# TaceoLabs/co-snarks

Hardware: AMD Instinct MI355X
Metric: BN254 G1 MSM points/sec (higher is better)
Workload: dtype i32x9 29-bit-limb lazy Montgomery, i64 accumulate (BN254 Fq 254-bit); 1 GPU; BN254 G1 Pippenger MSM, uniform scalars / known-dlog points, 2^20 points per GPU (BASELINE config 2); points_total=1048576, points_per_gpu=1048576, split=single GPU, exchange_mode=none, rccl_ranks_seen=0, spinup_steps=190

## Files before the change

### co-snarks_amd/csrc/host_fp64.hpp

```cpp
#pragma once
#include <stdint.h>
#include <string.h>

#include "field.hpp"

#if defined(__clang__)
#define CSH_HOST_UNROLL _Pragma("unroll")
#elif defined(__GNUC__)
#define CSH_HOST_UNROLL _Pragma("GCC unroll 16")
#else
#define CSH_HOST_UNROLL
#endif

namespace csh {

template <int N>
struct Fp64Consts {
  uint64_t mod[N], one[N], pm2[N];
  uint64_t inv;
};
template <class P>
constexpr Fp64Consts<P::N / 2> fp64_consts() {
  Fp64Consts<P::N / 2> k{};
  for (int i = 0; i < P::N / 2; ++i) {
    k.mod[i] = (uint64_t)P::MOD[2 * i] | ((uint64_t)P::MOD[2 * i + 1] << 32);
    k.one[i] = (uint64_t)P::R1[2 * i] | ((uint64_t)P::R1[2 * i + 1] << 32);
    k.pm2[i] = (uint64_t)P::PM2[2 * i] | ((uint64_t)P::PM2[2 * i + 1] << 32);
  }
  uint64_t y = k.mod[0];
  for (int i = 0; i < 6; ++i) y *= 2 - k.mod[0] * y;
  k.inv = (uint64_t)0 - y;
  return k;
}

template <class P>
struct Fp64 {
  static_assert(P::N % 2 == 0, "limb count must be even");
  static constexpr int N = P::N / 2;
  using Params = P;
  using u128 = unsigned __int128;
  uint64_t l[N];

  static constexpr Fp64Consts<N> K = fp64_consts<P>();
  static_assert((K.mod[N - 1] >> 63) == 0 && K.mod[N - 1] != 0x7fffffffffffffffull, "the modulus must leave its top bit free");
  static_assert((uint64_t)(K.mod[0] * K.inv) == ~(uint64_t)0, "inv must be -p^-1 mod 2^64");

  static uint64_t word(const uint32_t* w, int i) { return (uint64_t)w[2 * i] | ((uint64_t)w[2 * i + 1] << 32); }
  static constexpr uint64_t inv64() { return K.inv; }
  static Fp64 zero() {
    Fp64 r;
    for (int i = 0; i < N; ++i) r.l[i] = 0;
    return r;
  }
  static Fp64 one() {
    Fp64 r;
    for (int i = 0; i < N; ++i) r.l[i] = K.one[i];
    return r;
  }
  bool is_zero() const {
    uint64_t a = 0;
    for (int i = 0; i < N; ++i) a |= l[i];
    return a == 0;
  }
  bool operator==(const Fp64& b) const { return memcmp(l, b.l, sizeof l) == 0; }
  bool operator!=(const Fp64& b) const { return !(*this == b); }

  static bool geq_mod(const uint64_t* a) {
    CSH_HOST_UNROLL
    for (int i = N - 1; i >= 0; --i) {
      if (a[i] > K.mod[i]) return true;
      if (a[i] < K.mod[i]) return false;
    }
    return true;
  }
  static void sub_mod(uint64_t* a) {
    u128 br = 0;
    CSH_HOST_UNROLL
    for (int i = 0; i < N; ++i) {
      const u128 d = (u128)a[i] - K.mod[i] - (uint64_t)br;
      a[i] = (uint64_t)d;
      br = (d >> 64) & 1;
    }
  }
  static Fp64 add(const Fp64& a, const Fp64& b) {
    Fp64 r;
    u128 c = 0;
    CSH_HOST_UNROLL
    for (int i = 0; i < N; ++i) {
      c += (u128)a.l[i] + b.l[i];
      r.l[i] = (uint64_t)c;
      c >>= 64;
    }
    if (geq_mod(r.l)) sub_mod(r.l);
    return r;
  }
  static Fp64 sub(const Fp64& a, const Fp64& b) {
    Fp64 r;
    uint64_t br = 0;
    CSH_HOST_UNROLL
    for (int i = 0; i < N; ++i) {
      const u128 d = (u128)a.l[i] - b.l[i] - br;
      r.l[i] = (uint64_t)d;
      br = (uint64_t)(d >> 64) & 1;
    }
    if (br) {
      u128 c = 0;
      CSH_HOST_UNROLL
      for (int i = 0; i < N; ++i) {
        c += (u128)r.l[i] + K.mod[i];
        r.l[i] = (uint64_t)c;
        c >>= 64;
      }
    }
    return r;
  }
  static Fp64 neg(const Fp64& a) { return a.is_zero() ? a : sub(zero(), a); }

  static Fp64 mul(const Fp64& a, const Fp64& b) {
    uint64_t t[N];
    CSH_HOST_UNROLL
    for (int j = 0; j < N; ++j) t[j] = 0;
    CSH_HOST_UNROLL
    for (int i = 0; i < N; ++i) {
      u128 A = (u128)a.l[i] * b.l[0] + t[0];
      const uint64_t m = (uint64_t)A * K.inv;
      u128 C = (u128)m * K.mod[0] + (uint64_t)A;
      CSH_HOST_UNROLL
      for (int j = 1; j < N; ++j) {
        A = (u128)a.l[i] * b.l[j] + t[j] + (uint64_t)(A >> 64);
        C = (u128)m * K.mod[j] + (uint64_t)A + (uint64_t)(C >> 64);
        t[j - 1] = (uint64_t)C;
      }
      t[N - 1] = (uint64_t)(A >> 64) + (uint64_t)(C >> 64);
    }
    Fp64 r;
    CSH_HOST_UNROLL
    for (int i = 0; i < N; ++i) r.l[i] = t[i];
    if (geq_mod(r.l)) sub_mod(r.l);
    return r;
  }
  static Fp64 sqr(const Fp64& a) {
    uint64_t t[2 * N];
    CSH_HOST_UNROLL
    for (int j = 0; j < 2 * N; ++j) t[j] = 0;
    CSH_HOST_UNROLL
    for (int i = 0; i < N - 1; ++i) {
      uint64_t c = 0;
      CSH_HOST_UNROLL
      for (int j = i + 1; j < N; ++j) {
        const u128 v = (u128)a.l[i] * a.l[j] + t[i + j] + c;
        t[i + j] = (uint64_t)v;
        c = (uint64_t)(v >> 64);
      }
      t[i + N] = c;
    }
    CSH_HOST_UNROLL
    for (int j = 2 * N - 1; j > 0; --j) t[j] = (t[j] << 1) | (t[j - 1] >> 63);
    t[0] = 0;
    {
      uint64_t c = 0;
      CSH_HOST_UNROLL
      for (int i = 0; i < N; ++i) {
        const u128 d = (u128)a.l[i] * a.l[i];
        const u128 lo = (u128)t[2 * i] + (uint64_t)d + c;
        t[2 * i] = (uint64_t)lo;
        const u128 hi = (u128)t[2 * i + 1] + (uint64_t)(d >> 64) + (uint64_t)(lo >> 64);
        t[2 * i + 1] = (uint64_t)hi;
        c = (uint64_t)(hi >> 64);
      }
    }
    uint64_t top = 0;
    CSH_HOST_UNROLL
    for (int i = 0; i < N; ++i) {
      const uint64_t m = t[i] * K.inv;
      u128 C = (u128)m * K.mod[0] + t[i];
      CSH_HOST_UNROLL
      for (int j = 1; j < N; ++j) {
        C = (u128)m * K.mod[j] + t[i + j] + (uint64_t)(C >> 64);
        t[i + j] = (uint64_t)C;
      }
      const u128 s = (u128)t[i + N] + (uint64_t)(C >> 64) + top;
      t[i + N] = (uint64_t)s;
      top = (uint64_t)(s >> 64);
    }
    Fp64 r;
    CSH_HOST_UNROLL
    for (int i = 0; i < N; ++i) r.l[i] = t[i + N];
    if (geq_mod(r.l)) sub_mod(r.l);
    return r;
  }
  static Fp64 mul2(const Fp64& a) { return add(a, a); }
  static Fp64 mul3(const Fp64& a) { return add(add(a, a), a); }
  static Fp64 mul4(const Fp64& a) { return mul2(mul2(a)); }
  static Fp64 mul8(const Fp64& a) { return mul2(mul4(a)); }
  static Fp64 inv(const Fp64& a) {
    Fp64 pw[16];
    pw[0] = one();
    pw[1] = a;
    for (int i = 2; i < 16; ++i) pw[i] = (i & 1) ? mul(pw[i - 1], a) : sqr(pw[i / 2]);
    Fp64 r = one();
    bool started = false;
    for (int i = 16 * N - 1; i >= 0; --i) {
      const unsigned d = (unsigned)(K.pm2[i >> 4] >> (4 * (i & 15))) & 15u;
      if (started) r = sqr(sqr(sqr(sqr(r))));
      if (d) {
        r = started ? mul(r, pw[d]) : pw[d];
        started = true;
      }
    }
    return r;
  }

  static Fp64 mul_looped(const Fp64& a, const Fp64& b) {
    uint64_t t[N + 2];
    for (int i = 0; i < N + 2; ++i) t[i] = 0;
    const uint64_t inv = K.inv;
    for (int i = 0; i < N; ++i) {
      u128 c = 0;
      for (int j = 0; j < N; ++j) {
        c += (u128)a.l[j] * b.l[i] + t[j];
        t[j] = (uint64_t)c;
        c >>= 64;
      }
      c += t[N];
      t[N] = (uint64_t)c;
      t[N + 1] = (uint64_t)(c >> 64);
      const uint64_t m = t[0] * inv;
      c = (u128)m * K.mod[0] + t[0];
      c >>= 64;
      for (int j = 1; j < N; ++j) {
        c += (u128)m * K.mod[j] + t[j];
        t[j - 1] = (uint64_t)c;
        c >>= 64;
      }
      c += t[N];
      t[N - 1] = (uint64_t)c;
      t[N] = t[N + 1] + (uint64_t)(c >> 64);
    }
    Fp64 r;
    for (int i = 0; i < N; ++i) r.l[i] = t[i];
    if (t[N] || geq_mod(r.l)) sub_mod(r.l);
    return r;
  }
  static Fp64 inv_looped(const Fp64& a) {
    Fp64 r = one();
    for (int i = P::N * 32 - 1; i >= 0; --i) {
      r = mul_looped(r, r);
      if ((P::PM2[i >> 5] >> (i & 31)) & 1) r = mul_looped(r, a);
    }
    return r;
  }
};

template <class F>
struct Host64;
template <class P>
struct Host64<Fp<P>> {
  using type = Fp64<P>;
};
template <class P, int NR>
struct Host64<Fp2T<Fp<P>, NR>> {
  using type = Fp2T<Fp64<P>, NR>;
};

}
```

### co-snarks_amd/csrc/msm.hip

```cpp
#include <algorithm>
#include <condition_variable>
#include <memory>
#include <mutex>
#include <string>
#include <vector>

#include "msm_impl.hpp"

namespace csh {

thread_local float tl_msm_timing[6] = {0, 0, 0, 0, 0, 0};
thread_local uint32_t tl_msm_params[4] = {0, 0, 0, 0};

CSH_MSM_INSTANTIATE(extern, Bn254G1Cfg)
CSH_MSM_INSTANTIATE(extern, Bn254G2Cfg)
CSH_MSM_INSTANTIATE(extern, Bls381G1Cfg)
CSH_MSM_INSTANTIATE(extern, Bls381G2Cfg)
CSH_MSM_INSTANTIATE(extern, GrumpkinG1Cfg)
CSH_MSM_INSTANTIATE(extern, Bls377G1Cfg)
CSH_MSM_INSTANTIATE(extern, Bls377G2Cfg)
CSH_MSM_ACCUM_INSTANTIATE(extern, Bn254G1Cfg)
CSH_MSM_ACCUM_INSTANTIATE(extern, Bn254G2Cfg)
CSH_MSM_ACCUM_INSTANTIATE(extern, Bls381G1Cfg)
CSH_MSM_ACCUM_INSTANTIATE(extern, Bls381G2Cfg)
CSH_MSM_ACCUM_INSTANTIATE(extern, GrumpkinG1Cfg)
CSH_MSM_ACCUM_INSTANTIATE(extern, Bls377G1Cfg)
CSH_MSM_ACCUM_INSTANTIATE(extern, Bls377G2Cfg)
CSH_MSM_ACCUM_PAIR_INSTANTIATE(extern, Bn254G2Cfg)
CSH_MSM_ACCUM_PAIR_INSTANTIATE(extern, Bls381G2Cfg)
CSH_MSM_ACCUM_PAIR_INSTANTIATE(extern, Bls377G2Cfg)

static int repack_bases(Bases* B, hipStream_t st);

template <class Cfg>
static GroupOps group_ops_of(csh_curve_t curve, csh_group_t group) {
  using Fq = typename Cfg::Fq;
  return GroupOps{curve, group, Cfg::Fr::Params::BITS, sizeof(Affine<Fq>), sizeof(XYZZ<Fq>), msm_sort_stage<typename Cfg::Fr>,
                  msm_bucket_bytes<Cfg>, msm_bucket_stage<Cfg>, fold_windows_erased<Cfg>, accum_occupancy<Cfg>};
}
const GroupOps* group_ops(csh_curve_t curve, csh_group_t group) {
  static const GroupOps table[] = {
      group_ops_of<Bn254G1Cfg>(CSH_BN254, CSH_G1),       group_ops_of<Bn254G2Cfg>(CSH_BN254, CSH_G2),       group_ops_of<Bls381G1Cfg>(CSH_BLS12_381, CSH_G1),
      group_ops_of<Bls381G2Cfg>(CSH_BLS12_381, CSH_G2),  group_ops_of<GrumpkinG1Cfg>(CSH_GRUMPKIN, CSH_G1), group_ops_of<Bls377G1Cfg>(CSH_BLS12_377, CSH_G1),
      group_ops_of<Bls377G2Cfg>(CSH_BLS12_377, CSH_G2)};
  for (const GroupOps& o : table)
    if (o.curve == curve && o.group == group) return &o;
  set_error("unknown curve/group %d/%d", (int)curve, (int)group);
  return nullptr;
}

struct BasesFree {
  void operator()(Bases* B) const {
    if (B->points) (void)hipFree(B->points);
    if (B->table) (void)hipFree(B->table);
    delete B;
  }
};
using BasesPtr = std::unique_ptr<Bases, BasesFree>;

static int on_callers_device(const Bases* B) {
  int cur = -1;
  if (hipGetDevice(&cur) == hipSuccess && cur != B->device) {
    set_error("bases were uploaded on device %d but the calling thread is bound to device %d (csh_init): upload a copy per device", B->device, cur);
    return CSH_ERR_INVALID;
  }
  return CSH_OK;
}

}

using namespace csh;

namespace {
struct SharedUpload {
  int device = 0;
  const void* host = nullptr;
  size_t bytes = 0, cap = 0;
  void* dev = nullptr;
  hipEvent_t ready = nullptr;
  int refs = 0;
  std::mutex m;
  std::condition_variable cv;
  int state = 0;
  struct Req {
    csh_bases_t bases = nullptr;
    size_t offset = 0;
    void* out = nullptr;
    int rc = CSH_OK;
    std::string err;
  };
  std::vector<Req*> batch;
  bool sealed = false;
  bool batch_done = false;
  int curve = -1, mont = -1;
};
std::mutex g_up_mu;
std::vector<SharedUpload*> g_up_live;
struct PooledBuffer {
  int device;
  size_t cap;
  void* dev;
};
std::vector<PooledBuffer> g_up_pool;
constexpr size_t UP_POOL_MAX = 8;
constexpr size_t UP_POOL_MAX_BYTES = size_t(1) << 30;

struct SharedUploadRef {
  SharedUpload* e = nullptr;
  hipStream_t stream = nullptr;
  const void* dev() const { return e->dev; }
  bool is_owner = false;
  int acquire(int device, const void* host, size_t bytes, hipStream_t st, SharedUpload::Req* req = nullptr, int curve = -1, int mont = -1, bool* joined = nullptr) {
    stream = st;
    bool owner = false;
    {
      std::lock_guard<std::mutex> g(g_up_mu);
      for (SharedUpload* x : g_up_live)
        if (x->device == device && x->host == host && x->bytes == bytes) {
          bool failed;
          {
            std::lock_guard<std::mutex> gs(x->m);
            failed = x->state < 0;
          }
          if (failed) continue;
          e = x;
          break;
        }
      if (e) {
        ++e->refs;
      } else {
        e = new SharedUpload();
        e->device = device, e->host = host, e->bytes = bytes, e->refs = 1;
        e->curve = curve, e->mont = mont;
        size_t best = (size_t)-1;
        for (size_t i = 0; i < g_up_pool.size(); ++i)
          if (g_up_pool[i].device == device && g_up_pool[i].cap >= bytes && (best == (size_t)-1 || g_up_pool[i].cap < g_up_pool[best].cap)) best = i;
        if (best != (size_t)-1) {
          e->cap = g_up_pool[best].cap;
          e->dev = g_up_pool[best].dev;
          g_up_pool.erase(g_up_pool.begin() + (ptrdiff_t)best);
        }
        g_up_live.push_back(e);
        owner = true;
      }
    }
    is_owner = owner;
    if (owner) {
      hipError_t rc = hipSuccess;
      if (!e->dev) {
        e->cap = (bytes + (size_t(1) << 20) - 1) & ~((size_t(1) << 20) - 1);
        rc = hipMalloc(&e->dev, e->cap);
        if (rc != hipSuccess) e->dev = nullptr;
      }
      if (rc == hipSuccess) rc = hipEventCreateWithFlags(&e->ready, hipEventDisableTiming);
      if (rc == hipSuccess && upload_h2d(e->dev, host, bytes, st, 3) != CSH_OK) rc = hipErrorUnknown;
      if (rc == hipSuccess) rc = hipEventRecord(e->ready, st);
      {
        std::lock_guard<std::mutex> g(e->m);
        e->state = rc == hipSuccess ? 1 : -1;
      }
      e->cv.notify_all();
      if (rc != hipSuccess) {
        set_error("csh_msm: uploading the scalars failed: %s", hipGetErrorString(rc));
        return rc == hipErrorOutOfMemory ? CSH_ERR_OOM : CSH_ERR_HIP;
      }
      return CSH_OK;
    }
    {
      std::unique_lock<std::mutex> g(e->m);
      if (req && joined && !e->sealed && e->curve == curve && e->mont == mont && curve >= 0 && e->batch.size() < 15) {
        e->batch.push_back(req);
        *joined = true;
        e->cv.wait(g, [&] { return e->batch_done || e->state < 0; });
        if (!e->batch_done) {
          e->batch.erase(std::find(e->batch.begin(), e->batch.end(), req));
          set_error("csh_msm: the concurrent call that was uploading this scalar slice failed");
          return CSH_ERR_HIP;
        }
        tune().stat_uploads_shared.fetch_add(1, std::memory_order_relaxed);
        return CSH_OK;
      }
      e->cv.wait(g, [&] { return e->state != 0; });
      if (e->state < 0) {
        set_error("csh_msm: the concurrent call that was uploading this scalar slice failed");
        return CSH_ERR_HIP;
      }
    }
    CSH_HIP(hipStreamWaitEvent(st, e->ready, 0));
    tune().stat_uploads_shared.fetch_add(1, std::memory_order_relaxed);
    return CSH_OK;
  }
  std::vector<SharedUpload::Req*> seal() {
    std::lock_guard<std::mutex> g(e->m);
    e->sealed = true;
    return e->batch;
  }
  void finish_batch() {
    {
      std::lock_guard<std::mutex> g(e->m);
      e->batch_done = true;
    }
    e->cv.notify_all();
  }
  ~SharedUploadRef() {
    if (!e) return;
    if (is_owner) {
      bool wake = false;
      {
        std::lock_guard<std::mutex> g(e->m);
        if (!e->batch_done) {
          e->sealed = true;
          for (SharedUpload::Req* r : e->batch)
            if (r->rc == CSH_OK && r->err.empty()) {
              r->rc = CSH_ERR_HIP;
              r->err = "csh_msm: the concurrent call that ran this batch failed before it reached this request";
            }
          e->batch_done = true;
          wake = true;
        }
      }
      if (wake) e->cv.notify_all();
    }
    (void)hipStreamSynchronize(stream);
    SharedUpload* dead = nullptr;
    {
      std::lock_guard<std::mutex> g(g_up_mu);
      if (--e->refs == 0) {
        g_up_live.erase(std::find(g_up_live.begin(), g_up_live.end(), e));
        dead = e;
        size_t pooled = 0;
        for (const PooledBuffer& b : g_up_pool) pooled += b.cap;
        if (dead->dev && g_up_pool.size() < UP_POOL_MAX && pooled + dead->cap <= UP_POOL_MAX_BYTES) {
          g_up_pool.push_back({dead->device, dead->cap, dead->dev});
          dead->dev = nullptr;
        }
      }
    }
    if (dead) {
      if (dead->ready) (void)hipEventDestroy(dead->ready);
      if (dead->dev) (void)hipFree(dead->dev);
      delete dead;
    }
  }
};
}

static int csh::repack_bases(Bases* B, hipStream_t st) {
  CURVE_DISPATCH(B->curve, B->group, (repack_bases_t<Cfg>(B, st)));
}

extern "C" {

static int bases_upload_common(csh_curve_t curve, csh_group_t group, const void* pts, size_t n, size_t stride, bool src_dev, void* stream,
                               csh_bases_t* out) {
  CSH_REQUIRE(out, "out is NULL");
  const GroupOps* G = group_ops(curve, group);
  if (!G) return CSH_ERR_INVALID;
  CSH_REQUIRE(n < (size_t(1) << 31), "at most 2^31-1 bases per handle");
  CSH_REQUIRE(pts || n == 0, "points is NULL");
  CSH_TRY(ensure_device());
  const size_t pb = G->point_bytes;
  if (stride == 0) stride = pb;
  CSH_REQUIRE(stride >= pb, "stride_bytes smaller than a packed affine point");
  BasesPtr B(new Bases());
  B->curve = curve;
  B->group = group;
  B->n = n;
  B->point_bytes = pb;
  B->points = nullptr;
  if (hipGetDevice(&B->device) != hipSuccess) B->device = 0;
  hipError_t e = hipMalloc(&B->points, n ? n * pb : 1);
  if (e != hipSuccess) {
    B->points = nullptr;
    set_error("hipMalloc(%zu bytes) for bases failed: %s", n * pb, hipGetErrorString(e));
    return CSH_ERR_OOM;
  }
  if (n) {
    hipStream_t st = resolve_stream(stream);
    const hipMemcpyKind kind = src_dev ? hipMemcpyDeviceToDevice : hipMemcpyHostToDevice;
    if (!src_dev && stride == pb) {
      if (upload_h2d(B->points, pts, n * pb, st, 0) != CSH_OK) e = hipErrorUnknown;
    } else {
      e = stride == pb ? hipMemcpyAsync(B->points, pts, n * pb, kind, st) : hipMemcpy2DAsync(B->points, pb, pts, stride, pb, n, kind, st);
    }
    if (e == hipSuccess) e = hipStreamSynchronize(st);
    if (e != hipSuccess) {
      set_error("bases upload failed: %s", hipGetErrorString(e));
      return CSH_ERR_HIP;
    }
    CSH_TRY(repack_bases(B.get(), st));
  }
  *out = reinterpret_cast<csh_bases_t>(B.release());
  return CSH_OK;
}

int csh_bases_upload(csh_curve_t curve, csh_group_t group, const void* pts, size_t n, size_t stride, csh_bases_t* out) {
  return bases_upload_common(curve, group, pts, n, stride, false, nullptr, out);
}
int csh_bases_upload_dev(csh_curve_t curve, csh_group_t group, const void* pts, size_t n, size_t stride, void* stream, csh_bases_t* out) {
  return bases_upload_common(curve, group, pts, n, stride, true, stream, out);
}
int csh_bases_len(csh_bases_t bases, size_t* n) {
  CSH_REQUIRE(bases && n, "NULL argument");
  *n = reinterpret_cast<Bases*>(bases)->n;
  return CSH_OK;
}
int csh_bases_clone_range(csh_bases_t src, size_t offset, size_t n, int device, csh_bases_t* out) {
  CSH_REQUIRE(src && out, "NULL argument");
  const Bases* S = reinterpret_cast<const Bases*>(src);
  CSH_REQUIRE(offset <= S->n && n <= S->n - offset, "csh_bases_clone_range: offset + n exceeds the number of bases");
  int ndev = 0, cur = 0;
  CSH_HIP(hipGetDeviceCount(&ndev));
  CSH_REQUIRE(device >= 0 && device < ndev, "device out of range");
  CSH_HIP(hipGetDevice(&cur));
  BasesPtr B(new Bases(*S));
  B->points = nullptr;
  B->table = nullptr;
  B->device = device;
  B->n = n;
  const size_t pb = S->point_bytes, pbytes = n * pb, rows = S->table ? (size_t)S->table_W : 0;
  if (!rows) B->table_c = B->table_W = 0;
  hipError_t e = hipSetDevice(device);
  if (e == hipSuccess && pbytes) e = hipMalloc(&B->points, pbytes);
  if (e == hipSuccess && pbytes && rows) e = hipMalloc(&B->table, pbytes * rows);
  if (e == hipSuccess && pbytes) e = hipMemcpyPeer(B->points, device, static_cast<const char*>(S->points) + offset * pb, S->device, pbytes);
  for (size_t k = 0; e == hipSuccess && pbytes && k < rows; ++k)
    e = hipMemcpyPeer(static_cast<char*>(B->table) + k * pbytes, device, static_cast<const char*>(S->table) + (k * S->n + offset) * pb, S->device, pbytes);
  if (e == hipSuccess) e = hipDeviceSynchronize();
  if (e == hipSuccess && S->device != device) {
    e = hipSetDevice(S->device);
    if (e == hipSuccess) e = hipDeviceSynchronize();
  }
  (void)hipSetDevice(cur);
  if (e != hipSuccess) {
    set_error("csh_bases_clone_range to device %d failed: %s", device, hipGetErrorString(e));
    return e == hipErrorOutOfMemory ? CSH_ERR_OOM : CSH_ERR_HIP;
  }
  *out = reinterpret_cast<csh_bases_t>(B.release());
  return CSH_OK;
}
int csh_bases_clone(csh_bases_t src, int device, csh_bases_t* out) {
  CSH_REQUIRE(src && out, "NULL argument");
  return csh_bases_clone_range(src, 0, reinterpret_cast<const Bases*>(src)->n, device, out);
}
int csh_bases_free(csh_bases_t bases) {
  const BasesPtr freed(reinterpret_cast<Bases*>(bases));
  return CSH_OK;
}

static int bases_precompute(csh_bases_t bases, int c, int groups);
int csh_bases_table_policy(size_t key_points, int* c_out, int* rows_out) {
  CSH_REQUIRE(c_out && rows_out, "c_out / rows_out is NULL");
  *c_out = 0;
  *rows_out = 0;
  if (key_points < (size_t(1) << 14) || key_points > (size_t(1) << 26)) return CSH_OK;
  if (key_points < (size_t(1) << 15)) {
    int c = 16;
    while (c > 10 && (size_t(1) << (c + 1)) > key_points) --c;
    *c_out = c;
    *rows_out = 16;
    return CSH_OK;
  }
  if (key_points <= (size_t(3) << 20)) {
    *c_out = 17;
    *rows_out = 16;
  } else {
    *c_out = 20;
    *rows_out = 13;
  }
  return CSH_OK;
}
int csh_bases_drop_tables(csh_bases_t bases) {
  CSH_REQUIRE(bases, "bases is NULL");
  Bases* B = reinterpret_cast<Bases*>(bases);
  if (B->table) {
    (void)hipFree(B->table);
    B->table = nullptr;
    B->table_c = B->table_W = 0;
  }
  return CSH_OK;
}
int csh_bases_precompute(csh_bases_t bases, int c) { return bases_precompute(bases, c, 0); }
int csh_bases_precompute_grouped(csh_bases_t bases, int c, int groups) {
  CSH_REQUIRE(groups >= 2 && groups <= MAX_WINDOWS, "groups must be in [2, 128]");
  return bases_precompute(bases, c, groups);
}
static int bases_precompute(csh_bases_t bases, int c, int groups) {
  CSH_REQUIRE(bases, "bases is NULL");
  CSH_TRY(ensure_device());
  Bases* B = reinterpret_cast<Bases*>(bases);
  CSH_REQUIRE(c == 0 || (c >= 4 && c <= 22), "window width must be 0 (auto) or in [4, 22]");
  if (B->table) {
    (void)hipFree(B->table);
    B->table = nullptr;
  }
  if (B->n < 1024) return CSH_OK;
  if (c == 0) {
    c = 16;
    while (c > 10 && (size_t(1) << (c + 1)) > B->n) --c;
  }
  CSH_TRY(on_callers_device(B));
  hipStream_t st = resolve_stream(nullptr);
  CURVE_DISPATCH(B->curve, B->group, (precompute_table_t<Cfg>(B, c, groups, st)));
}

static int msm_args(csh_bases_t bases, size_t offset, size_t n, const void* scalars, const void* out) {
  CSH_REQUIRE(bases, "bases is NULL");
  CSH_REQUIRE(out, "out is NULL");
  Bases* B = reinterpret_cast<Bases*>(bases);
  CSH_REQUIRE(offset <= B->n && n <= B->n - offset, "offset + n exceeds the uploaded bases");
  CSH_REQUIRE(scalars || n == 0, "scalars is NULL");
  return on_callers_device(B);
}

int csh_msm_dev(csh_bases_t bases, size_t offset, size_t n, const uint64_t* scalars_dev, int mont, void* out_host, void* stream) {
  CSH_TRY(msm_args(bases, offset, n, scalars_dev, out_host));
  CSH_TRY(ensure_device());
  Bases* B = reinterpret_cast<Bases*>(bases);
  hipStream_t st = resolve_stream(stream);
  CURVE_DISPATCH(B->curve, B->group, (msm_t<Cfg>(B, offset, n, scalars_dev, mont, out_host, st)));
}

static int run_owned_batch(SharedUploadRef& up, SharedUpload::Req& own, size_t n, const uint64_t* dsc, int mont, hipStream_t st) {
  const std::vector<SharedUpload::Req*> others = up.seal();
  if (others.empty()) {
    up.finish_batch();
    return csh_msm_dev(own.bases, own.offset, n, dsc, mont, own.out, st);
  }
  std::vector<SharedUpload::Req*> all;
  all.push_back(&own);
  for (SharedUpload::Req* r : others) all.push_back(r);
  std::stable_sort(all.begin(), all.end(), [](const SharedUpload::Req* a, const SharedUpload::Req* b) {
    return reinterpret_cast<const Bases*>(a->bases)->group > reinterpret_cast<const Bases*>(b->bases)->group;
  });
  std::vector<csh_bases_t> hs;
  std::vector<size_t> offs;
  std::vector<void*> outs;
  for (SharedUpload::Req* r : all) hs.push_back(r->bases), offs.push_back(r->offset), outs.push_back(r->out);
  const int rc = csh_msm_multi_dev(hs.data(), offs.data(), all.size(), n, dsc, mont, outs.data(), st);
  const std::string err = rc == CSH_OK ? std::string() : std::string(csh_last_error());
  for (SharedUpload::Req* r : others) r->rc = rc, r->err = err;
  up.finish_batch();
  return rc;
}

int csh_msm(csh_bases_t bases, size_t offset, size_t n, const uint64_t* scalars, int mont, void* out) {
  CSH_TRY(msm_args(bases, offset, n, scalars, out));
  const size_t bytes = 32 * n;
  if (bytes >= (size_t(1) << 20) && tune().msm_share_uploads.load(std::memory_order_relaxed) != 0) {
    CSH_TRY(ensure_device());
    hipStream_t st = resolve_stream(nullptr);
    int device = 0;
    (void)hipGetDevice(&device);
    const bool batching = tune().msm_share_uploads.load(std::memory_order_relaxed) >= 2;
    const Bases* B = reinterpret_cast<const Bases*>(bases);
    SharedUpload::Req req;
    req.bases = bases, req.offset = offset, req.out = out;
    bool joined = false;
    SharedUploadRef up;
    CSH_TRY(up.acquire(device, scalars, bytes, st, batching ? &req : nullptr, batching ? (int)B->curve : -1, mont != 0, &joined));
    if (joined) {
      if (req.rc != CSH_OK) set_error("%s", req.err.c_str());
      return req.rc;
    }
    const uint64_t* dsc = reinterpret_cast<const uint64_t*>(up.dev());
    if (!up.is_owner || !batching) return csh_msm_dev(bases, offset, n, dsc, mont, out, st);
    return run_owned_batch(up, req, n, dsc, mont, st);
  }
  HostStage h;
  CSH_TRY(h.begin(Arena::padded(bytes)));
  uint64_t* ds;
  CSH_TRY(h.up(ds, scalars, bytes));
  return csh_msm_dev(bases, offset, n, ds, mont, out, h.st);
}

int csh_msm_shares(csh_bases_t bases, size_t offset, size_t n, const uint64_t* shares, uint32_t ncomp, int mont, void* const* outs) {
  CSH_REQUIRE(ncomp >= 1 && ncomp <= 2 && outs, "msm_shares: ncomp must be 1 or 2 and outs non-NULL");
  for (uint32_t c = 0; c < ncomp; ++c) CSH_REQUIRE(outs[c], "msm_shares: NULL output");
  CSH_TRY(msm_args(bases, offset, n, shares, outs[0]));
  if (ncomp == 1) return csh_msm(bases, offset, n, shares, mont, outs[0]);
  HostStage h;
  CSH_TRY(h.begin(Arena::padded(32 * (size_t)ncomp * n) + Arena::padded(32 * n)));
  uint64_t *dsh, *dcomp;
  CSH_TRY(h.up(dsh, shares, 32 * (size_t)ncomp * n));
  CSH_TRY(h.up(dcomp, nullptr, 32 * n));
  for (uint32_t c = 0; c < ncomp; ++c) {
    CSH_TRY(csh_extract_component_dev(dsh, ncomp, c, n, dcomp, h.st));
    CSH_TRY(csh_msm_dev(bases, offset, n, dcomp, mont, outs[c], h.st));
  }
  return CSH_OK;
}

int csh_msm_partial_bytes(csh_curve_t curve, csh_group_t group, size_t* bytes) {
  CSH_REQUIRE(bytes, "bytes is NULL");
  if (!group_ops(curve, group)) return CSH_ERR_INVALID;
  *bytes = partial_bytes_of(curve, group);
  return CSH_OK;
}

int csh_msm_partial_dev(csh_bases_t bases, size_t offset, size_t n, const uint64_t* scalars_dev, int mont, void* out_dev, void* stream) {
  CSH_TRY(msm_args(bases, offset, n, scalars_dev, out_dev));
  CSH_TRY(ensure_device());
  Bases* B = reinterpret_cast<Bases*>(bases);
  hipStream_t st = resolve_stream(stream);
  CURVE_DISPATCH(B->curve, B->group, (msm_partial_t<Cfg>(B, offset, n, scalars_dev, mont, out_dev, st, true)));
}

int csh_msm_fold_partials(csh_curve_t curve, csh_group_t group, const void* partials_host, size_t nparts, void* out_jacobian) {
  CSH_REQUIRE(partials_host && out_jacobian, "NULL argument");
  CURVE_DISPATCH(curve, group, (fold_partials_t<Cfg>(partials_host, nparts, out_jacobian)));
}

int csh_msm_multi_dev(const csh_bases_t* bases, const size_t* offsets, size_t k, size_t n, const uint64_t* scalars_dev, int mont,
                      void* const* outs_host, void* stream) {
  CSH_REQUIRE(bases && offsets && outs_host && k >= 1 && k <= 16, "msm_multi: bad arguments");
  CSH_REQUIRE(scalars_dev || n == 0, "scalars is NULL");
  CSH_REQUIRE(n < (size_t(1) << 31), "n too large");
  CSH_TRY(ensure_device());
  const auto handle = [&](size_t i) { return reinterpret_cast<const Bases*>(bases[i]); };
  const Bases* B0 = handle(0);
  CSH_REQUIRE(B0, "bases[0] is NULL");
  for (size_t i = 0; i < k; ++i) {
    const Bases* B = handle(i);
    CSH_REQUIRE(B && outs_host[i], "msm_multi: NULL handle or output");
    CSH_REQUIRE(B->curve == B0->curve, "msm_multi: all bases must belong to one curve");
    CSH_REQUIRE(offsets[i] <= B->n && n <= B->n - offsets[i], "msm_multi: offset + n exceeds the number of bases");
    CSH_REQUIRE(B->device == B0->device, "msm_multi: bases live on different devices");
  }
  CSH_TRY(on_callers_device(B0));
  hipStream_t st = resolve_stream(stream);
  std::vector<const GroupOps*> ops(k);
  for (size_t i = 0; i < k; ++i)
    if (!(ops[i] = group_ops(handle(i)->curve, handle(i)->group))) return CSH_ERR_INVALID;
  if (n == 0) {
    for (size_t i = 0; i < k; ++i) ops[i]->fold(nullptr, 0, 2, 0, outs_host[i]);
    return CSH_OK;
  }
  bool merged = true;
  for (size_t i = 0; i < k; ++i) merged = merged && msm_use_table(handle(i), n) && handle(i)->table_c == B0->table_c && handle(i)->table_W == B0->table_W;
  int occ = 8;
  for (const GroupOps* o : ops) occ = std::min(occ, o->occ());
  const MsmTable table{B0->table_c, B0->table_W, B0->n, 0};
  MsmPlan plan = msm_plan(n, ops[0]->scalar_bits, mont, occ, merged ? &table : nullptr);
  msm_record_params(plan.srt);
  const MsmParams& pdig = plan.dig;
  MsmParams& p = plan.srt;
  size_t bucket_max = 0, win_bytes = 0, slice = 0;
  for (const GroupOps* o : ops) {
    bucket_max = std::max(bucket_max, o->bucket_bytes(&p));
    win_bytes += Arena::padded(o->xyzz_bytes * MAX_WINDOWS);
    slice = std::max(slice, Arena::padded(o->xyzz_bytes * MAX_WINDOWS));
  }
  Arena& ar = arena_for(st);
  CSH_TRY(ar.reserve(msm_sort_bytes(p, pdig) + 2 * Arena::padded(bucket_max)));
  Arena& wa = arena_for((hipStream_t)((uintptr_t)st ^ 0x2));
  CSH_TRY(wa.reserve(win_bytes));
  hipStream_t aux = nullptr;
  if (tune().msm_multi_overlap.load(std::memory_order_relaxed) != 0 && k > 1) aux = resolve_aux_stream();
  const bool two = aux != nullptr;
  Events evs;
  CSH_TRY(evs.create(k + (two ? 2 : 0), hipEventDisableTiming));
  const hipEvent_t sorted_ev = two ? evs[k] : nullptr, aux_done = two ? evs[k + 1] : nullptr;
  auto body = [&]() -> int {
    SortOut so;
    std::vector<char*> win_dev(k);
    std::vector<hipStream_t> stage_stream(k, st);
    size_t mark = 0, sorted_stride = (size_t)-1, sorted_off = (size_t)-1;
    bool aux_used = false;
    for (size_t i = 0; i < k; ++i) {
      const Bases* B = handle(i);
      const bool resort = merged ? (B->n != sorted_stride || offsets[i] != sorted_off) : i == 0;
      if (resort) {
        if (two && aux_used) {
          CSH_HIP(hipEventRecord(aux_done, aux));
          CSH_HIP(hipStreamWaitEvent(st, aux_done, 0));
        }
        ar.off = 0;
        if (merged) {
          p.remap_stride = (uint32_t)(sorted_stride = B->n);
          p.remap_off = (uint32_t)(sorted_off = offsets[i]);
        }
        CSH_TRY(ops[0]->sort(p, pdig, scalars_dev, st, ar, &so, nullptr));
        mark = ar.off;
        if (two) {
          CSH_HIP(hipEventRecord(sorted_ev, st));
          CSH_HIP(hipStreamWaitEvent(aux, sorted_ev, 0));
        }
      }
      const bool on_aux = two && (i & 1);
      stage_stream[i] = on_aux ? aux : st;
      aux_used = aux_used || on_aux;
      ar.off = mark + (on_aux ? Arena::padded(bucket_max) : 0);
      win_dev[i] = wa.take<char>(ops[i]->xyzz_bytes * MAX_WINDOWS);
      const void* src = merged ? B->table : static_cast<const char*>(B->points) + offsets[i] * B->point_bytes;
      CSH_TRY(ops[i]->bucket(src, &p, &so, stage_stream[i], &ar, win_dev[i], nullptr));
    }
    void *pin_host = nullptr, *pin_dev = nullptr;
    std::vector<char> pageable;
    char* wins = nullptr;
    if (pinned_for((hipStream_t)((uintptr_t)st ^ 0x4), slice * k, &pin_host, &pin_dev)) {
      wins = static_cast<char*>(pin_host);
    } else {
      pageable.resize(slice * k);
      wins = pageable.data();
    }
    for (size_t i = 0; i < k; ++i) {
      hipError_t e = hipMemcpyAsync(wins + slice * i, win_dev[i], ops[i]->xyzz_bytes * p.W, hipMemcpyDeviceToHost, stage_stream[i]);
      if (e == hipSuccess) e = hipEventRecord(evs[i], stage_stream[i]);
      if (e != hipSuccess) {
        set_error("msm_multi: queuing the window sums of result %zu failed: %s", i, hipGetErrorString(e));
        return CSH_ERR_HIP;
      }
    }
    for (size_t i = 0; i < k; ++i) {
      const hipError_t e = hipEventSynchronize(evs[i]);
      if (e != hipSuccess) {
        set_error("msm_multi: result %zu failed on the device: %s", i, hipGetErrorString(e));
        return CSH_ERR_HIP;
      }
      ops[i]->fold(wins + slice * i, p.W, p.c, p.wide, outs_host[i]);
    }
    CSH_HIP(hipStreamSynchronize(st));
    if (aux) CSH_HIP(hipStreamSynchronize(aux));
    return CSH_OK;
  };
  const int rc = body();
  if (rc != CSH_OK) {
    (void)hipStreamSynchronize(st);
    if (aux) (void)hipStreamSynchronize(aux);
  }
  return rc;
}

int csh_msm_plan(csh_curve_t curve, size_t n, uint32_t out[6]) {
  CSH_REQUIRE(out, "out is NULL");
  const GroupOps* G = group_ops(curve, CSH_G1);
  if (!G) return CSH_ERR_INVALID;
  CSH_REQUIRE(n >= 1 && n < (size_t(1) << 31), "n out of range");
  const MsmParams p = msm_plan(n, G->scalar_bits, 1, 1).srt;
  const uint64_t lanes = (n + p.L - 1) / p.L;
  out[0] = (uint32_t)p.c;
  out[1] = (uint32_t)p.W;
  out[2] = p.L;
  out[3] = p.S;
  out[4] = (uint32_t)((uint64_t)p.W * ((lanes + ACC_BLK - 1) / ACC_BLK) * (ACC_BLK / 64));
  out[5] = (uint32_t)device_simds();
  return CSH_OK;
}

int csh_msm_last_params(uint32_t out[4]) {
  CSH_REQUIRE(out, "out is NULL");
  for (int i = 0; i < 4; ++i) out[i] = tl_msm_params[i];
  return CSH_OK;
}

int csh_msm_last_timing(float out_ms[6]) {
  CSH_REQUIRE(out_ms, "out_ms is NULL");
  for (int i = 0; i < 6; ++i) out_ms[i] = tl_msm_timing[i];
  return CSH_OK;
}

}
```

### co-snarks_amd/csrc/msm_impl.hpp

```cpp
#pragma once
#include <stdlib.h>
#include <string.h>

#include <algorithm>
#include <type_traits>
#include <vector>

#include "common.hpp"
#include "curve.hpp"
#include "curve_lazy.hpp"
#include "curve_quad.hpp"
#include "curve_pair.hpp"
#include "host_fp64.hpp"
#include "msm_digits.hpp"
#include "msm_plan.hpp"
#include "msm_sort.hpp"
#include "msm_sort_wide.hpp"


namespace csh {

struct Bn254G1Cfg { using Fq = Bn254Fq;   using Fr = Bn254Fr; static constexpr bool LAZY = true;  using L = Fq29s; static constexpr bool INLINE_ADD = true; static constexpr bool PAIR = false; };
struct Bn254G2Cfg { using Fq = Bn254Fq2;  using Fr = Bn254Fr; static constexpr bool LAZY = true;  using L = Fq29s2; static constexpr bool INLINE_ADD = true; static constexpr bool PAIR = true; static constexpr bool PAIR_ACC_DEFAULT = false; using LP = Fp2Pair<Fq29s>; };
struct Bls381G1Cfg { using Fq = Bls381Fq;  using Fr = Bls381Fr; static constexpr bool LAZY = true;  using L = Fq28s; static constexpr bool INLINE_ADD = true; static constexpr bool PAIR = false; };
struct GrumpkinG1Cfg { using Fq = Bn254Fr;   using Fr = Bn254Fq; static constexpr bool LAZY = true;  using L = Fr29s; static constexpr bool INLINE_ADD = true; static constexpr bool PAIR = false; };
struct Bls377G1Cfg { using Fq = Bls377Fq;  using Fr = Bls377Fr; static constexpr bool LAZY = true;  using L = Fq28s377; static constexpr bool INLINE_ADD = true; static constexpr bool PAIR = false; };
struct Bls377G2Cfg { using Fq = Bls377Fq2; using Fr = Bls377Fr; static constexpr bool LAZY = true;  using L = Fq28s377x2; static constexpr bool INLINE_ADD = true; static constexpr bool PAIR = true; static constexpr bool PAIR_ACC_DEFAULT = true; using LP = Fp2Pair<Fq28s377, 5>; };
struct Bls381G2Cfg { using Fq = Bls381Fq2; using Fr = Bls381Fr; static constexpr bool LAZY = true;  using L = Fq28s2; static constexpr bool INLINE_ADD = true; static constexpr bool PAIR = true; static constexpr bool PAIR_ACC_DEFAULT = true; using LP = Fp2Pair<Fq28s>; };

struct Bases {
  csh_curve_t curve;
  csh_group_t group;
  int device;
  size_t n;
  size_t point_bytes;
  void* points;
  void* table = nullptr;
  int table_c = 0, table_W = 0;
};


constexpr int MSM_BLK = 256;

template <class Fr>
__device__ __forceinline__ void load_scalar(const Fr* __restrict__ scalars, size_t i, int mont, uint32_t* s) {
  Fr v = scalars[i];
  if (mont) v = v.from_mont();
#pragma unroll
  for (int k = 0; k < Fr::N; ++k) s[k] = v.l[k];
}


template <class Fr>
__global__ __launch_bounds__(MSM_BLK) void k_msm_digits(const Fr* __restrict__ scalars, MsmParams p, uint16_t* __restrict__ dig) {
  const uint32_t g = p.dig_g > 1 ? p.dig_g : 1u, wp = p.dig_g > 1 ? p.dig_wp : (uint32_t)p.W;
  const uint32_t rows = g * wp;
  const uint32_t W = (uint32_t)p.W, wide = (uint32_t)p.wide;
  for (size_t i = blockIdx.x * (size_t)MSM_BLK + threadIdx.x; i < p.n; i += (size_t)gridDim.x * MSM_BLK) {
    uint32_t s[Fr::N];
    load_scalar<Fr>(scalars, i, p.mont, s);
    uint32_t carry = 0, rq = 0, rr = 0;
    for (uint32_t w = 0; w < rows; ++w) {
      uint32_t code = DIG_ZERO;
      if (w < W) {
        const uint32_t c = (uint32_t)p.c - (w >= wide ? 1u : 0u);
        const uint32_t mask = (1u << c) - 1, half = 1u << (c - 1);
        const uint32_t v = (s[0] & mask) + carry;
#pragma unroll
        for (int k = 0; k + 1 < Fr::N; ++k) s[k] = (s[k] >> c) | (s[k + 1] << (32 - c));
        s[Fr::N - 1] >>= c;
        const uint32_t neg = v > half ? 1u : 0u;
        const uint32_t mag = neg ? (1u << c) - v : v;
        carry = neg;
        code = mag ? ((mag - 1) | (neg << 15)) : (uint32_t)DIG_ZERO;
      }
      dig[(size_t)(rr * g + rq) * p.n + i] = (uint16_t)code;
      if (++rr == wp) {
        rr = 0;
        ++rq;
      }
    }
  }
}

template <class P>
__device__ __forceinline__ uint32_t top_word(const Fp<P>& f) { return f.l[Fp<P>::N - 1]; }
template <class F, int NR>
__device__ __forceinline__ uint32_t top_word(const Fp2T<F, NR>& f) { return top_word(f.c0) | top_word(f.c1); }
template <class Fq>
__device__ __forceinline__ bool stored_is_inf(const Affine<Fq>& pt) {
  return (top_word(pt.x) | top_word(pt.y)) == 0 && pt.is_inf();
}

__device__ __forceinline__ uint32_t upper_bound_u32(const uint32_t* __restrict__ a, uint32_t lo, uint32_t hi, uint32_t v) {
  while (lo < hi) {
    const uint32_t mid = (lo + hi) >> 1;
    if (a[mid] > v) hi = mid; else lo = mid + 1;
  }
  return lo;
}

template <class Cfg>
using LazyPt = XYZZLazy<typename Cfg::L>;

template <class Cfg>
__global__ __launch_bounds__(ACC_BLK) void k_msm_accum(const Affine<typename Cfg::Fq>* __restrict__ bases, MsmParams p,
                                                       const uint32_t* __restrict__ start, const uint32_t* __restrict__ nlanes,
                                                       const uint32_t* __restrict__ sorted, LazyPt<Cfg>* partial, uint32_t* giant_count) {
  using Fq = typename Cfg::Fq;
  static_assert(Cfg::LAZY, "the bucket pipeline runs in the signed lazy field");
  const int w = blockIdx.y;
  const uint32_t k = blockIdx.x * blockDim.x + threadIdx.x;
  if (k == 0 && w == 0) {
    giant_count[0] = 0;
    giant_count[1] = 0;
  }
  if (k >= nlanes[w]) return;
  const uint32_t* st = start + (size_t)w * (p.NB + 2);
  const uint32_t total = st[p.NB + 1];
  const uint32_t Lw = lane_len(p, w);
  const uint32_t lo = k * Lw;
  uint32_t hi = lo + Lw;
  if (hi > total) hi = total;
  uint32_t b = upper_bound_u32(st, 1, p.NB + 1, lo) - 1;
  uint32_t next = st[b + 1];
  const uint32_t* so = sorted + (size_t)w * p.n;
  LazyPt<Cfg>* pw = partial + (size_t)w * p.tmax;
  {
    using L = typename Cfg::L;
    XYZZLazy<L> acc = XYZZLazy<L>::inf();
    uint32_t e_next = so[lo];
    Affine<Fq> pt_next = bases[e_next & 0x7fffffffu];
    constexpr bool INDEX_AHEAD = !Cfg::PAIR;
    uint32_t e_next2 = (INDEX_AHEAD && lo + 1 < hi) ? so[lo + 1] : 0;
    for (uint32_t pos = lo; pos < hi; ++pos) {
      const uint32_t e = e_next;
      const Affine<Fq> pt = pt_next;
      if (pos + 1 < hi) {
        if constexpr (INDEX_AHEAD) {
          e_next = e_next2;
          pt_next = bases[e_next & 0x7fffffffu];
          if (pos + 2 < hi) e_next2 = so[pos + 2];
        } else {
          e_next = so[pos + 1];
          pt_next = bases[e_next & 0x7fffffffu];
        }
      }
      const bool inf = stored_is_inf(pt);
      const L x = L::unpack(pt.x);
      const L y = L::unpack(pt.y).cneg_unpacked(e >> 31);
      if (pos == next) {
        pw[b + k] = acc;
        do { ++b; next = st[b + 1]; } while (next <= pos);
        acc.x = x;
        acc.y = y;
        acc.zz = L::one();
        acc.zzz = L::one();
        acc.empty = inf;
        continue;
      }
      if (inf) continue;
      lazy_madd<L, Affine<Fq>>(acc, x, y, bases + (e & 0x7fffffffu), e >> 31);
    }
    pw[b + k] = acc;
  }
}

template <class Cfg>
__global__ __launch_bounds__(ACC_BLK) void k_msm_accum_pair(const Affine<typename Cfg::Fq>* __restrict__ bases, MsmParams p,
                                                            const uint32_t* __restrict__ start, const uint32_t* __restrict__ nlanes,
                                                            const uint32_t* __restrict__ sorted, LazyPt<Cfg>* partial, uint32_t* giant_count) {
  using Fq = typename Cfg::Fq;
  using L = typename Cfg::LP;
  using LF = typename L::Base;
  using F32 = decltype(bases->x.c0);
  const int w = blockIdx.y;
  const int role = pair_role();
  const uint32_t k = (blockIdx.x * blockDim.x + threadIdx.x) >> 1;
  if (blockIdx.x == 0 && threadIdx.x == 0 && w == 0) {
    giant_count[0] = 0;
    giant_count[1] = 0;
  }
  if (k >= nlanes[w]) return;
  const uint32_t* st = start + (size_t)w * (p.NB + 2);
  const uint32_t total = st[p.NB + 1];
  const uint32_t Lw = lane_len(p, w);
  const uint32_t lo = k * Lw;
  uint32_t hi = lo + Lw;
  if (hi > total) hi = total;
  uint32_t b = upper_bound_u32(st, 1, p.NB + 1, lo) - 1;
  uint32_t next = st[b + 1];
  const uint32_t* so = sorted + (size_t)w * p.n;
  LazyPt<Cfg>* pw = partial + (size_t)w * p.tmax;
  const F32* half = reinterpret_cast<const F32*>(bases) + role;
  XYZZLazy<L> acc = XYZZLazy<L>::inf();
  uint32_t e_next = so[lo];
  F32 x_next = half[4 * (size_t)(e_next & 0x7fffffffu)], y_next = half[4 * (size_t)(e_next & 0x7fffffffu) + 2];
  for (uint32_t pos = lo; pos < hi; ++pos) {
    const uint32_t e = e_next;
    const F32 xs = x_next, ys = y_next;
    if (pos + 1 < hi) {
      e_next = so[pos + 1];
      x_next = half[4 * (size_t)(e_next & 0x7fffffffu)];
      y_next = half[4 * (size_t)(e_next & 0x7fffffffu) + 2];
    }
    const bool inf = pair_all((top_word(xs) | top_word(ys)) == 0 && xs.is_zero() && ys.is_zero());
    const L x{LF::unpack(xs)};
    const L y{LF::unpack(ys).cneg_unpacked(e >> 31)};
    if (pos == next) {
      pair_store(&pw[b + k], role, acc);
      do { ++b; next = st[b + 1]; } while (next <= pos);
      acc.x = x;
      acc.y = y;
      acc.zz = L::one();
      acc.zzz = L::one();
      acc.empty = inf;
      continue;
    }
    if (inf) continue;
    lazy_madd<L, Affine<Fq>>(acc, x, y, bases + (e & 0x7fffffffu), e >> 31);
  }
  pair_store(&pw[b + k], role, acc);
}

constexpr int MERGE_BLK = 256;
constexpr int MERGE_Q = MERGE_BLK / 4;

constexpr uint32_t MERGE_CAP = 16;
constexpr uint32_t GIANT_BIG = 256, GIANT_SLICES = 16, GIANT_BIG_CAP = 128, GIANT_ROWS = 32, GIANT_SLICED_FLAG = 0x80000000u;
__device__ __forceinline__ void giant_enqueue(uint32_t* giant_count, uint32_t* giant_list, uint32_t* big_list, uint32_t w, uint32_t b, uint32_t nparts) {
  uint32_t tag = w;
  if (nparts >= GIANT_BIG) {
    const uint32_t q = atomicAdd(giant_count + 1, 1u);
    if (q < GIANT_BIG_CAP) {
      big_list[2 * q] = w;
      big_list[2 * q + 1] = b;
      tag |= GIANT_SLICED_FLAG;
    }
  }
  const uint32_t g = atomicAdd(giant_count, 1u);
  giant_list[2 * g] = tag;
  giant_list[2 * g + 1] = b;
}
template <class Cfg>
__global__ __launch_bounds__(MERGE_BLK) void k_msm_merge(MsmParams p, const uint32_t* __restrict__ start,
                                                         const LazyPt<Cfg>* __restrict__ partial, LazyPt<Cfg>* dense,
                                                         uint32_t* giant_count, uint32_t* giant_list, uint32_t* big_list) {
  using L = typename Cfg::L;
  __shared__ uint32_t list_n;
  __shared__ uint32_t list[MERGE_Q];
  const int w = blockIdx.y;
  const int role = threadIdx.x & 3;
  const uint32_t q = threadIdx.x >> 2;
  const uint32_t b0 = blockIdx.x * MERGE_Q + 1;
  const uint32_t* st = start + (size_t)w * (p.NB + 2);
  const uint32_t Lw = lane_len(p, w);
  const LazyPt<Cfg>* pw = partial + (size_t)w * p.tmax;
  LazyPt<Cfg>* dw = dense + (size_t)w * (p.NB + 1);
  if (threadIdx.x == 0) list_n = 0;
  __syncthreads();
  if (const uint32_t b = b0 + q; b <= p.NB) {
    const uint32_t lo = st[b], hi = st[b + 1];
    QPt<L> acc = qpt_inf<L>();
    if (hi > lo) {
      const uint32_t k0 = lo / Lw, k1 = (hi - 1) / Lw;
      if (k1 - k0 >= MERGE_CAP) {
        if (role == 0) giant_enqueue(giant_count, giant_list, big_list, (uint32_t)w, b, k1 - k0 + 1);
      } else {
        acc = qpt_load<L>(&pw[b + k0], role);
        if (k1 > k0) qadd<L>(acc, qpt_load<L>(&pw[b + k0 + 1], role), role);
        if (k1 - k0 >= 2 && role == 0) list[atomicAdd(&list_n, 1u)] = q;
      }
    }
    qpt_store<L>(&dw[b], role, acc);
  }
  __syncthreads();
  if (q < list_n) {
    const uint32_t b = b0 + list[q];
    const uint32_t k0 = st[b] / Lw, k1 = (st[b + 1] - 1) / Lw;
    QPt<L> acc = qpt_load<L>(&dw[b], role);
    for (uint32_t k = k0 + 2; k <= k1; ++k) qadd<L>(acc, qpt_load<L>(&pw[b + k], role), role);
    qpt_store<L>(&dw[b], role, acc);
  }
}

template <class L>
__device__ __forceinline__ void quad_block_tree(QPt<L>& x, XYZZLazy<L>* sh, int q, int nq, int role) {
  for (int half = nq >> 1; half >= 1; half >>= 1) {
    if (q >= half && q < 2 * half) qpt_store<L>(&sh[q - half], role, x);
    __syncthreads();
    if (q < half) qadd<L>(x, qpt_load<L>(&sh[q], role), role);
    __syncthreads();
  }
}

template <class Cfg>
__global__ __launch_bounds__(256) void k_msm_giant_slices(MsmParams p, const uint32_t* __restrict__ start, const LazyPt<Cfg>* __restrict__ partial,
                                                          const uint32_t* __restrict__ giant_count, const uint32_t* __restrict__ big_list,
                                                          LazyPt<Cfg>* gscratch) {
  using L = typename Cfg::L;
  __shared__ XYZZLazy<L> sh[32];
  const uint32_t sl = blockIdx.x;
  const uint32_t nbig = giant_count[1] < GIANT_BIG_CAP ? giant_count[1] : GIANT_BIG_CAP;
  const int role = threadIdx.x & 3, qd = threadIdx.x >> 2;
  for (uint32_t q = blockIdx.y; q < nbig; q += gridDim.y) {
    const uint32_t w = big_list[2 * q], b = big_list[2 * q + 1];
    const uint32_t* st = start + (size_t)w * (p.NB + 2);
    const uint32_t Lw = lane_len(p, (int)w);
    const uint32_t k0 = st[b] / Lw, k1 = (st[b + 1] - 1) / Lw;
    const uint32_t per = (k1 - k0 + GIANT_SLICES) / GIANT_SLICES;
    const uint32_t a = k0 + sl * per;
    uint32_t e = a + per;
    if (e > k1 + 1) e = k1 + 1;
    const LazyPt<Cfg>* pw = partial + (size_t)w * p.tmax + b;
    QPt<L> acc = qpt_inf<L>();
    for (uint32_t k = a + qd; k < e; k += 64) qadd<L>(acc, qpt_load<L>(&pw[k], role), role);
    quad_block_tree<L>(acc, sh, qd, 64, role);
    if (qd == 0) qpt_store<L>(&gscratch[(size_t)q * GIANT_SLICES + sl], role, acc);
  }
}

template <class Cfg>
__global__ __launch_bounds__(256) void k_msm_merge_giant(MsmParams p, const uint32_t* __restrict__ start,
                                                         const LazyPt<Cfg>* __restrict__ partial, LazyPt<Cfg>* dense,
                                                         const uint32_t* __restrict__ giant_count, const uint32_t* __restrict__ giant_list,
                                                         const uint32_t* __restrict__ big_list, const LazyPt<Cfg>* __restrict__ gscratch) {
  using L = typename Cfg::L;
  __shared__ XYZZLazy<L> sh[32];
  __shared__ uint32_t slot;
  const uint32_t count = giant_count[0];
  const uint32_t nbig = giant_count[1] < GIANT_BIG_CAP ? giant_count[1] : GIANT_BIG_CAP;
  const int role = threadIdx.x & 3, q = threadIdx.x >> 2;
  for (uint32_t g = blockIdx.x; g < count; g += gridDim.x) {
    const uint32_t tag = giant_list[2 * g], w = tag & ~GIANT_SLICED_FLAG, b = giant_list[2 * g + 1];
    QPt<L> acc = qpt_inf<L>();
    if (tag & GIANT_SLICED_FLAG) {
      __syncthreads();
      if (threadIdx.x == 0) slot = GIANT_BIG_CAP;
      __syncthreads();
      if (threadIdx.x < nbig && big_list[2 * threadIdx.x] == w && big_list[2 * threadIdx.x + 1] == b) slot = threadIdx.x;
      __syncthreads();
      if (slot < GIANT_BIG_CAP) {
        if ((uint32_t)q < GIANT_SLICES) acc = qpt_load<L>(&gscratch[(size_t)slot * GIANT_SLICES + q], role);
      } else {
        const uint32_t* st = start + (size_t)w * (p.NB + 2);
        const uint32_t Lw = lane_len(p, (int)w);
        const uint32_t k0 = st[b] / Lw, k1 = (st[b + 1] - 1) / Lw;
        const LazyPt<Cfg>* pw = partial + (size_t)w * p.tmax + b;
        for (uint32_t k = k0 + q; k <= k1; k += 64) qadd<L>(acc, qpt_load<L>(&pw[k], role), role);
      }
    } else {
      const uint32_t* st = start + (size_t)w * (p.NB + 2);
      const uint32_t Lw = lane_len(p, (int)w);
      const uint32_t k0 = st[b] / Lw, k1 = (st[b + 1] - 1) / Lw;
      const LazyPt<Cfg>* pw = partial + (size_t)w * p.tmax + b;
      for (uint32_t k = k0 + q; k <= k1; k += 64) qadd<L>(acc, qpt_load<L>(&pw[k], role), role);
    }
    quad_block_tree<L>(acc, sh, q, 64, role);
    if (q == 0) qpt_store<L>(&dense[(size_t)w * (p.NB + 1) + b], role, acc);
  }
}

template <class Cfg>
__global__ __launch_bounds__(256) void k_msm_mark_giant(MsmParams p, const uint32_t* __restrict__ start, uint32_t* giant_count, uint32_t* giant_list,
                                                        uint32_t* big_list) {
  const int w = blockIdx.y;
  const uint32_t b = blockIdx.x * 256 + threadIdx.x + 1;
  if (b > p.NB) return;
  const uint32_t* st = start + (size_t)w * (p.NB + 2);
  const uint32_t lo = st[b], hi = st[b + 1];
  const uint32_t Lw = lane_len(p, w);
  if (hi > lo && (hi - 1) / Lw - lo / Lw >= MERGE_CAP) giant_enqueue(giant_count, giant_list, big_list, (uint32_t)w, b, (hi - 1) / Lw - lo / Lw + 1);
}
template <class Cfg>
__device__ __forceinline__ QPt<typename Cfg::L> qbucket_merged(uint32_t Lw, const uint32_t* __restrict__ st, const LazyPt<Cfg>* __restrict__ pw,
                                                               const LazyPt<Cfg>* __restrict__ dw, uint32_t t, int role) {
  using L = typename Cfg::L;
  const uint32_t lo = st[t], hi = st[t + 1];
  if (hi <= lo) return qpt_inf<L>();
  const uint32_t k0 = lo / Lw, k1 = (hi - 1) / Lw;
  if (k1 - k0 >= MERGE_CAP) return qpt_load<L>(&dw[t], role);
  QPt<L> acc = qpt_load<L>(&pw[t + k0], role);
  for (uint32_t k = k0 + 1; k <= k1; ++k) qadd<L>(acc, qpt_load<L>(&pw[t + k], role), role);
  return acc;
}
template <class Cfg>
__device__ __forceinline__ XYZZLazy<typename Cfg::LP> pbucket_merged(uint32_t Lw, const uint32_t* __restrict__ st, const LazyPt<Cfg>* __restrict__ pw,
                                                                     const LazyPt<Cfg>* __restrict__ dw, uint32_t t, int role) {
  using L = typename Cfg::LP;
  const uint32_t lo = st[t], hi = st[t + 1];
  if (hi <= lo) return XYZZLazy<L>::inf();
  const uint32_t k0 = lo / Lw, k1 = (hi - 1) / Lw;
  if (k1 - k0 >= MERGE_CAP) return dw[t].empty ? XYZZLazy<L>::inf() : pair_load(&dw[t], role);
  XYZZLazy<L> acc = pw[t + k0].empty ? XYZZLazy<L>::inf() : pair_load(&pw[t + k0], role);
  for (uint32_t k = k0 + 1; k <= k1; ++k) {
    if (pw[t + k].empty) continue;
    const XYZZLazy<L> q = pair_load(&pw[t + k], role);
    lazy_add_inl<L>(acc, q);
  }
  return acc;
}

template <class Cfg, bool FUSED>
__global__ __launch_bounds__(256) void k_msm_reduce(MsmParams p, const LazyPt<Cfg>* __restrict__ dense,
                                                    LazyPt<Cfg>* segres, const uint32_t* __restrict__ start, const LazyPt<Cfg>* __restrict__ partial) {
  using L = typename Cfg::L;
  const int w = blockIdx.y;
  const int role = threadIdx.x & 3;
  const uint32_t k = blockIdx.x * 64 + (threadIdx.x >> 2);
  if (k >= p.S) return;
  const uint32_t per = (p.NB + p.S - 1) / p.S;
  const uint32_t t0 = 1 + k * per;
  uint32_t t1 = t0 + per;
  if (t1 > p.NB + 1) t1 = p.NB + 1;
  QPt<L> running = qpt_inf<L>(), acc = qpt_inf<L>();
  uint32_t prev_b = 0;
  if (t0 < t1) {
    const LazyPt<Cfg>* dw = dense + (size_t)w * (p.NB + 1);
    const uint32_t* st = FUSED ? start + (size_t)w * (p.NB + 2) : nullptr;
    const LazyPt<Cfg>* pw = FUSED ? partial + (size_t)w * p.tmax : nullptr;
    for (uint32_t t = t1; t-- > t0;) {
      QPt<L> pt;
      if constexpr (FUSED) pt = qbucket_merged<Cfg>(lane_len(p, w), st, pw, dw, t, role);
      else pt = qpt_load<L>(&dw[t], role);
      if (pt.empty) continue;
      uint32_t gap = prev_b ? prev_b - t : 0;
      if (gap) {
        if (gap <= 4) {
          while (gap--) qadd<L>(acc, running, role);
        } else {
          const QPt<L> m = qmul_small_w2<L>(running, gap, role);
          qadd<L>(acc, m, role);
        }
      }
      qadd<L>(running, pt, role);
      prev_b = t;
    }
    if (prev_b) {
      const QPt<L> m = qmul_small_w2<L>(running, prev_b, role);
      qadd<L>(acc, m, role);
    }
  }
  qpt_store<L>(&segres[(size_t)w * p.S + k], role, acc);
}

constexpr int RED_BLK = 256;

template <class Cfg>
__global__ __launch_bounds__(RED_BLK) void k_msm_reduce_serial(MsmParams p, const LazyPt<Cfg>* __restrict__ dense, LazyPt<Cfg>* segres) {
  using L = typename Cfg::L;
  const int w = blockIdx.y;
  const uint32_t k = blockIdx.x * RED_BLK + threadIdx.x;
  if (k >= p.S) return;
  const uint32_t per = (p.NB + p.S - 1) / p.S;
  const uint32_t t0 = 1 + k * per;
  uint32_t t1 = t0 + per;
  if (t1 > p.NB + 1) t1 = p.NB + 1;
  LazyPt<Cfg> running = LazyPt<Cfg>::inf(), acc = LazyPt<Cfg>::inf();
  uint32_t prev_b = 0;
  if (t0 < t1) {
    const LazyPt<Cfg>* dw = dense + (size_t)w * (p.NB + 1);
    for (uint32_t t = t1; t-- > t0;) {
      const LazyPt<Cfg> pt = dw[t];
      if (pt.empty) continue;
      uint32_t gap = prev_b ? prev_b - t : 0;
      if (gap) {
        if (gap <= 4) {
          while (gap--) lazy_add_inl<L>(acc, running);
        } else {
          const LazyPt<Cfg> m = lazy_mul_small<L, true>(running, gap);
          lazy_add_inl<L>(acc, m);
        }
      }
      lazy_add_inl<L>(running, pt);
      prev_b = t;
    }
    if (prev_b) {
      const LazyPt<Cfg> m = lazy_mul_small<L, true>(running, prev_b);
      lazy_add_inl<L>(acc, m);
    }
  }
  segres[(size_t)w * p.S + k] = acc;
}

template <class Cfg, bool FUSED>
__global__ __launch_bounds__(RED_BLK) void k_msm_reduce_pair(MsmParams p, const LazyPt<Cfg>* __restrict__ dense, LazyPt<Cfg>* segres,
                                                             const uint32_t* __restrict__ start, const LazyPt<Cfg>* __restrict__ partial) {
  using L = typename Cfg::LP;
  const int w = blockIdx.y;
  const int role = pair_role();
  const uint32_t k = blockIdx.x * (RED_BLK / 2) + (threadIdx.x >> 1);
  if (k >= p.S) return;
  const uint32_t per = (p.NB + p.S - 1) / p.S;
  const uint32_t t0 = 1 + k * per;
  uint32_t t1 = t0 + per;
  if (t1 > p.NB + 1) t1 = p.NB + 1;
  XYZZLazy<L> running = XYZZLazy<L>::inf(), acc = XYZZLazy<L>::inf();
  uint32_t prev_b = 0;
  if (t0 < t1) {
    const LazyPt<Cfg>* dw = dense + (size_t)w * (p.NB + 1);
    const uint32_t* st = FUSED ? start + (size_t)w * (p.NB + 2) : nullptr;
    const LazyPt<Cfg>* pw = FUSED ? partial + (size_t)w * p.tmax : nullptr;
    for (uint32_t t = t1; t-- > t0;) {
      XYZZLazy<L> pt;
      if constexpr (FUSED) {
        pt = pbucket_merged<Cfg>(lane_len(p, w), st, pw, dw, t, role);
        if (pt.empty) continue;
      } else {
        if (dw[t].empty) continue;
        pt = pair_load(&dw[t], role);
      }
      uint32_t gap = prev_b ? prev_b - t : 0;
      if (gap) {
        if (gap <= 4) {
          while (gap--) lazy_add_inl<L>(acc, running);
        } else {
          const XYZZLazy<L> m = lazy_mul_small<L, true>(running, gap);
          lazy_add_inl<L>(acc, m);
        }
      }
      lazy_add_inl<L>(running, pt);
      prev_b = t;
    }
    if (prev_b) {
      const XYZZLazy<L> m = lazy_mul_small<L, true>(running, prev_b);
      lazy_add_inl<L>(acc, m);
    }
  }
  pair_store(&segres[(size_t)w * p.S + k], role, acc);
}

template <class Cfg>
__global__ __launch_bounds__(256) void k_msm_fold_tree(const LazyPt<Cfg>* __restrict__ in, uint32_t stride_in, uint32_t count,
                                                       LazyPt<Cfg>* out, uint32_t stride_out, XYZZ<typename Cfg::Fq>* win_out) {
  using L = typename Cfg::L;
  using Fq = typename Cfg::Fq;
  __shared__ XYZZLazy<L> sh[32];
  const int w = blockIdx.y;
  const int role = threadIdx.x & 3, q = threadIdx.x >> 2;
  const LazyPt<Cfg>* a = in + (size_t)w * stride_in;
  const uint32_t i0 = blockIdx.x * 128 + q, i1 = i0 + 64;
  QPt<L> x = i0 < count ? qpt_load<L>(&a[i0], role) : qpt_inf<L>();
  if (i1 < count) qadd<L>(x, qpt_load<L>(&a[i1], role), role);
  quad_block_tree<L>(x, sh, q, 64, role);
  if (q == 0) {
    if (win_out) {
      static_assert(sizeof(XYZZ<Fq>) == 4 * sizeof(Fq), "XYZZ members must be contiguous");
      (&win_out[w].x)[role] = x.empty ? Fq::zero() : x.v.to_fp();
    } else {
      qpt_store<L>(&out[(size_t)w * stride_out + blockIdx.x], role, x);
    }
  }
}

template <class Cfg>
__global__ __launch_bounds__(256) void k_bases_repack(Affine<typename Cfg::Fq>* pts, size_t n) {
  if constexpr (Cfg::LAZY) {
    using L = typename Cfg::L;
    for (size_t i = blockIdx.x * (size_t)256 + threadIdx.x; i < n; i += (size_t)gridDim.x * 256) {
      Affine<typename Cfg::Fq> p = pts[i];
      if (p.is_inf()) continue;
      p.x = L::repack_for_storage(p.x);
      p.y = L::repack_for_storage(p.y);
      pts[i] = p;
    }
  }
}

template <class Cfg>
__global__ void k_msm_gather_windows(const LazyPt<Cfg>* segres, uint32_t stride, int W, XYZZ<typename Cfg::Fq>* out) {
  const int w = threadIdx.x;
  if (w < W) out[w] = lazy_to_xyzz<typename Cfg::L, typename Cfg::Fq>(segres[(size_t)w * stride]);
}

extern thread_local float tl_msm_timing[6];
extern thread_local uint32_t tl_msm_params[4];
inline void msm_record_params(const MsmParams& srt) {
  tl_msm_params[0] = (uint32_t)srt.c;
  tl_msm_params[1] = (uint32_t)srt.W;
  tl_msm_params[2] = srt.L;
  tl_msm_params[3] = srt.S;
}

struct Events {
  std::vector<hipEvent_t> ev;
  Events() = default;
  Events(const Events&) = delete;
  Events& operator=(const Events&) = delete;
  ~Events() {
    for (hipEvent_t e : ev) (void)hipEventDestroy(e);
  }
  int create(size_t count, unsigned flags) {
    ev.reserve(ev.size() + count);
    for (size_t i = 0; i < count; ++i) {
      hipEvent_t e;
      CSH_HIP(hipEventCreateWithFlags(&e, flags));
      ev.push_back(e);
    }
    return CSH_OK;
  }
  hipEvent_t operator[](size_t i) const { return ev[i]; }
};

struct PartialHeader {
  uint32_t magic, c, W, wide;
  uint32_t pad[4];
};
constexpr uint32_t PARTIAL_MAGIC = 0x4d534d50u;


struct SortOut {
  uint32_t *start, *nlanes, *sorted;
};

inline bool msm_sort_is_wide(const MsmParams& p) { return p.c > 16 && p.W == 1 && p.remap_n != 0; }
template <class Fr>
constexpr int fr_id_of() {
  return std::is_same<Fr, Bls381Fr>::value ? 1 : (std::is_same<Fr, Bn254Fq>::value ? 2 : (std::is_same<Fr, Bls377Fr>::value ? 3 : 0));
}

struct SortStageBufs {
  SortBuffers sb;
  bool two_level;
};
inline SortBuffers sort_group_view(const MsmParams& p, const SortBuffers& b, int w0) {
  const size_t len = (size_t)p.NB + 2, n = p.n;
  SortBuffers g = b;
  g.hist += len * w0;
  g.start += len * w0;
  g.nlanes += w0;
  g.sorted += n * w0;
  g.dig += n * w0;
  g.blkcnt += (size_t)p.NB * p.CH * w0;
  if (g.inter) g.inter += n * w0;
  if (g.part_cnt) g.part_cnt += (size_t)(p.NB / 256) * p.CH * w0;
  return g;
}
inline SortStageBufs sort_take(const MsmParams& p, Arena& ar) {
  const size_t len = (size_t)p.NB + 2, n = p.n;
  SortStageBufs s;
  s.sb.hist = ar.take<uint32_t>(len * p.W);
  s.sb.start = ar.take<uint32_t>(len * p.W);
  s.sb.nlanes = ar.take<uint32_t>(MAX_WINDOWS);
  s.sb.sorted = ar.take<uint32_t>(n * p.W);
  s.sb.dig = ar.take<uint16_t>(n * p.W);
  s.sb.blkcnt = ar.take<uint32_t>((size_t)p.NB * p.CH * p.W);
  s.two_level = msm_sort_two_level(p);
  s.sb.inter = s.two_level ? ar.take<uint64_t>(n * p.W) : nullptr;
  s.sb.part_cnt = s.two_level ? ar.take<uint32_t>((size_t)(p.NB / 256) * p.CH * p.W) : nullptr;
  return s;
}
inline size_t msm_sort_bytes(const MsmParams& p, const MsmParams& pdig) {
  if (msm_sort_is_wide(p)) return msm_sort_wide_bytes(p, pdig);
  Arena sizing;
  sort_take(p, sizing);
  return sizing.off;
}
template <class Fr>
int msm_sort_prepare(const MsmParams& p, const MsmParams& pdig, const uint64_t* scalars_dev, hipStream_t st, Arena& ar, SortStageBufs* out) {
  *out = sort_take(p, ar);
  const int g1 = grid_for(pdig.n, MSM_BLK, 65536);
  hipLaunchKernelGGL(k_msm_digits<Fr>, dim3(g1), dim3(MSM_BLK), 0, st, reinterpret_cast<const Fr*>(scalars_dev), pdig, const_cast<uint16_t*>(out->sb.dig));
  return CSH_OK;
}
template <class Fr>
int msm_sort_stage(const MsmParams& p, const MsmParams& pdig, const uint64_t* scalars_dev, hipStream_t st, Arena& ar, SortOut* out, hipEvent_t* ev) {
  if (msm_sort_is_wide(p)) return msm_sort_wide_launch(fr_id_of<Fr>(), p, pdig, scalars_dev, st, ar, &out->start, &out->nlanes, &out->sorted, ev);
  SortStageBufs ss;
  CSH_TRY(msm_sort_prepare<Fr>(p, pdig, scalars_dev, st, ar, &ss));
  CSH_TRY(msm_sort_launch(p, ss.sb, st, ev));
  *out = SortOut{ss.sb.start, ss.sb.nlanes, ss.sb.sorted};
  return CSH_OK;
}

template <class Cfg>
struct BucketBufs {
  LazyPt<Cfg>*partial, *segres, *dense, *fold_a, *fold_b;
  uint32_t* giant;
  uint32_t* big;
  LazyPt<Cfg>* gscratch;
  uint32_t fold_n1, max_lanes, max_giant, giant_blocks;
};
constexpr int MAX_GROUPS = 8;
template <class Cfg>
BucketBufs<Cfg> bucket_take(const MsmParams& p, Arena& ar) {
  BucketBufs<Cfg> b;
  b.max_lanes = (uint32_t)(((size_t)p.n + p.L - 1) / p.L);
  b.max_giant = (uint32_t)(((uint64_t)b.max_lanes * p.W) / MERGE_CAP + 1);
  b.giant_blocks = b.max_giant < 1024 ? b.max_giant : 1024;
  b.partial = ar.take<LazyPt<Cfg>>((size_t)p.tmax * p.W);
  b.segres = ar.take<LazyPt<Cfg>>((size_t)p.S * p.W);
  b.dense = ar.take<LazyPt<Cfg>>((size_t)(p.NB + 1) * p.W);
  b.giant = ar.take<uint32_t>((2 * (size_t)b.max_giant + 2) * MAX_GROUPS);
  b.big = ar.take<uint32_t>((size_t)2 * GIANT_BIG_CAP * MAX_GROUPS);
  b.gscratch = ar.take<LazyPt<Cfg>>((size_t)GIANT_BIG_CAP * GIANT_SLICES * MAX_GROUPS);
  b.fold_n1 = (p.S + 127) / 128;
  b.fold_a = ar.take<LazyPt<Cfg>>((size_t)b.fold_n1 * p.W);
  b.fold_b = ar.take<LazyPt<Cfg>>((size_t)b.fold_n1 * p.W);
  return b;
}
template <class Cfg>
size_t msm_bucket_bytes(const MsmParams* pp) {
  Arena sizing;
  bucket_take<Cfg>(*pp, sizing);
  return sizing.off;
}

template <class Cfg>
int bucket_group(const void* points, const MsmParams& p_all, const SortOut& so, const BucketBufs<Cfg>& bb, int w0, int nw, int group, hipStream_t st,
                 void* win_out_dev, hipEvent_t* ev) {
  using Fq = typename Cfg::Fq;
  MsmParams p = p_all;
  p.wide = p_all.wide > w0 ? p_all.wide - w0 : 0;
  const size_t len = (size_t)p.NB + 2;
  const uint32_t* start = so.start + len * w0;
  const uint32_t* nlanes = so.nlanes + w0;
  const uint32_t* sorted = so.sorted + (size_t)p.n * w0;
  LazyPt<Cfg>* partial = bb.partial + (size_t)p.tmax * w0;
  LazyPt<Cfg>* segres = bb.segres + (size_t)p.S * w0;
  LazyPt<Cfg>* dense = bb.dense + (size_t)(p.NB + 1) * w0;
  LazyPt<Cfg>* fold_a = bb.fold_a + (size_t)bb.fold_n1 * w0;
  LazyPt<Cfg>* fold_b = bb.fold_b + (size_t)bb.fold_n1 * w0;
  uint32_t* giant = bb.giant + (2 * (size_t)bb.max_giant + 2) * group;
  uint32_t* big = bb.big + (size_t)2 * GIANT_BIG_CAP * group;
  LazyPt<Cfg>* gscratch = bb.gscratch + (size_t)GIANT_BIG_CAP * GIANT_SLICES * group;
  const Affine<Fq>* bases = reinterpret_cast<const Affine<Fq>*>(points);
  {
    const int tb = tune().acc_blk.load(std::memory_order_relaxed);
    const int blk = (tb == 64 || tb == 128) ? tb : ACC_BLK;
    bool pair = false;
    if constexpr (Cfg::PAIR) pair = Cfg::PAIR_ACC_DEFAULT != ((tune().msm_variant.load(std::memory_order_relaxed) & 2) != 0);
    if constexpr (Cfg::PAIR) {
      if (pair) {
        const dim3 ag((2 * bb.max_lanes + blk - 1) / blk, nw), ab(blk);
        hipLaunchKernelGGL(k_msm_accum_pair<Cfg>, ag, ab, 0, st, bases, p, start, nlanes, sorted, partial, giant);
      }
    }
    if (!pair) {
      const dim3 ag((bb.max_lanes + blk - 1) / blk, nw), ab(blk);
      hipLaunchKernelGGL(k_msm_accum<Cfg>, ag, ab, 0, st, bases, p, start, nlanes, sorted, partial, giant);
    }
  }
  if (ev) CSH_HIP(hipEventRecord(ev[4], st));
  const int variant = tune().msm_variant.load(std::memory_order_relaxed);
  int form;
  if constexpr (Cfg::PAIR) form = (variant & 1) ? 1 : ((variant & 4) ? 0 : 2);
  else form = (variant & 1) ? 0 : 1;
  const bool fused = form != 0 && (variant & 16) != 0;
  if (fused)
    hipLaunchKernelGGL(k_msm_mark_giant<Cfg>, dim3((p.NB + 255) / 256, nw), dim3(256), 0, st, p, start, giant, giant + 2, big);
  else
    hipLaunchKernelGGL(k_msm_merge<Cfg>, dim3((p.NB + MERGE_Q - 1) / MERGE_Q, nw), dim3(MERGE_BLK), 0, st, p, start, partial, dense, giant, giant + 2, big);
  hipLaunchKernelGGL(k_msm_giant_slices<Cfg>, dim3(GIANT_SLICES, GIANT_ROWS), dim3(256), 0, st, p, start, partial, giant, big, gscratch);
  hipLaunchKernelGGL(k_msm_merge_giant<Cfg>, dim3(bb.giant_blocks), dim3(256), 0, st, p, start, partial, dense, giant, giant + 2, big, gscratch);
  MsmParams pr = p;
  if (form == 1) {
    pr.S = std::min(p.S, reduce_segments(p.NB, p.W, 4));
    if (fused) hipLaunchKernelGGL((k_msm_reduce<Cfg, true>), dim3((pr.S + 63) / 64, nw), dim3(256), 0, st, pr, dense, segres, start, partial);
    else hipLaunchKernelGGL((k_msm_reduce<Cfg, false>), dim3((pr.S + 63) / 64, nw), dim3(256), 0, st, pr, dense, segres, start, partial);
  } else if (form == 2) {
    pr.S = std::min(p.S, reduce_segments(p.NB, p.W, 2));
    if constexpr (Cfg::PAIR) {
      if (fused) hipLaunchKernelGGL((k_msm_reduce_pair<Cfg, true>), dim3((pr.S + RED_BLK / 2 - 1) / (RED_BLK / 2), nw), dim3(RED_BLK), 0, st, pr, dense, segres, start, partial);
      else hipLaunchKernelGGL((k_msm_reduce_pair<Cfg, false>), dim3((pr.S + RED_BLK / 2 - 1) / (RED_BLK / 2), nw), dim3(RED_BLK), 0, st, pr, dense, segres, start, partial);
    }
  } else {
    hipLaunchKernelGGL(k_msm_reduce_serial<Cfg>, dim3((pr.S + RED_BLK - 1) / RED_BLK, nw), dim3(RED_BLK), 0, st, pr, dense, segres);
  }
  const LazyPt<Cfg>* cur = segres;
  uint32_t cur_n = pr.S, cur_stride = pr.S;
  LazyPt<Cfg>* nxt = fold_a;
  XYZZ<Fq>* win_out = reinterpret_cast<XYZZ<Fq>*>(win_out_dev) + w0;
  bool exported = false;
  while (cur_n > 1) {
    const uint32_t out_n = (cur_n + 127) / 128;
    exported = out_n == 1;
    hipLaunchKernelGGL(k_msm_fold_tree<Cfg>, dim3(out_n, nw), dim3(256), 0, st, cur, cur_stride, cur_n, nxt, bb.fold_n1,
                       exported ? win_out : (XYZZ<Fq>*)nullptr);
    cur = nxt;
    cur_n = out_n;
    cur_stride = bb.fold_n1;
    nxt = nxt == fold_a ? fold_b : fold_a;
  }
  if (!exported)
    hipLaunchKernelGGL(k_msm_gather_windows<Cfg>, dim3(1), dim3(MAX_WINDOWS), 0, st, cur, cur_stride, nw, win_out);
  CSH_HIP(hipGetLastError());
  return CSH_OK;
}

template <class Cfg>
int msm_bucket_stage(const void* points, const MsmParams* pp, const SortOut* so, hipStream_t st, Arena* arp, void* win_out_dev, hipEvent_t* ev) {
  const MsmParams& p = *pp;
  const BucketBufs<Cfg> bb = bucket_take<Cfg>(p, *arp);
  CSH_TRY((bucket_group<Cfg>(points, p, *so, bb, 0, p.W, 0, st, win_out_dev, ev)));
  if (ev) CSH_HIP(hipEventRecord(ev[5], st));
  return CSH_OK;
}


inline bool msm_use_table(const Bases* B, size_t n) {
  if (!B->table || n == 0 || tune().msm_no_table.load(std::memory_order_relaxed)) return false;
  if ((uint64_t)n * (uint64_t)B->table_W >= (uint64_t(1) << 31) || (uint64_t)B->n * (uint64_t)B->table_W >= (uint64_t(1) << 31)) return false;
  return n * 8 >= B->n;
}

template <class Cfg>
int accum_occupancy() {
  static std::atomic<int> cache{0};
  int v = cache.load(std::memory_order_relaxed);
  if (v) return v;
  v = 1;
  if constexpr (!Cfg::PAIR) {
    int blocks = 0;
    if (hipOccupancyMaxActiveBlocksPerMultiprocessor(&blocks, k_msm_accum<Cfg>, ACC_BLK, 0) == hipSuccess && blocks > 0) {
      v = blocks * (ACC_BLK / 64) / 4;
      v = v < 1 ? 1 : (v > 8 ? 8 : v);
    }
  }
  cache.store(v, std::memory_order_relaxed);
  return v;
}

template <class Cfg>
int msm_windows_dev(const Bases* B, size_t offset, size_t n, const uint64_t* scalars_dev, int mont, hipStream_t st,
                    XYZZ<typename Cfg::Fq>* win_out_dev , MsmParams* p_out) {
  using Fr = typename Cfg::Fr;
  using Fq = typename Cfg::Fq;
  const MsmTable table{B->table_c, B->table_W, B->n, offset};
  const MsmPlan plan = msm_plan(n, Fr::Params::BITS, mont, accum_occupancy<Cfg>(), msm_use_table(B, n) ? &table : nullptr);
  const MsmParams &p = plan.srt, &pdig = plan.dig;
  const void* points = plan.merged ? B->table : reinterpret_cast<const Affine<Fq>*>(B->points) + offset;
  msm_record_params(p);
  *p_out = p;
  Arena& ar = arena_for(st);
  CSH_TRY(ar.reserve(msm_sort_bytes(p, pdig) + msm_bucket_bytes<Cfg>(&p)));
  const bool timing = tune().msm_timing.load(std::memory_order_relaxed) != 0;
  Events timed;
  if (timing) {
    CSH_TRY(timed.create(7, hipEventDefault));
    CSH_HIP(hipEventRecord(timed[0], st));
  }
  hipEvent_t* ev = timing ? timed.ev.data() : nullptr;
  SortOut so;
  CSH_TRY(msm_sort_stage<Fr>(p, pdig, scalars_dev, st, ar, &so, ev));
  CSH_TRY(msm_bucket_stage<Cfg>(points, &p, &so, st, &ar, win_out_dev, ev));
  if (timing) {
    CSH_HIP(hipEventSynchronize(ev[5]));
    for (int i = 0; i < 5; ++i) CSH_HIP(hipEventElapsedTime(&tl_msm_timing[i], ev[i], ev[i + 1]));
    CSH_HIP(hipEventElapsedTime(&tl_msm_timing[5], ev[0], ev[5]));
  }
  return CSH_OK;
}

template <class Cfg>
__global__ __launch_bounds__(128) void k_bases_precompute(const Affine<typename Cfg::Fq>* __restrict__ pts, size_t n, int c, int W,
                                                          Affine<typename Cfg::Fq>* __restrict__ table) {
  using Fq = typename Cfg::Fq;
  using L = typename Cfg::L;
  const size_t i = blockIdx.x * (size_t)128 + threadIdx.x;
  if (i >= n) return;
  const Affine<Fq> stored = pts[i];
  table[i] = stored;
  if (stored.is_inf()) {
    for (int w = 1; w < W; ++w) table[(size_t)w * n + i] = stored;
    return;
  }
  Affine<Fq> q{L::unpack(stored.x).to_fp(), L::unpack(stored.y).to_fp()};
  for (int w = 1; w < W; ++w) {
    XYZZ<Fq> acc = XYZZ<Fq>::from_affine(q);
    for (int k = 0; k < c; ++k) acc = xyzz_dbl(acc);
    q = xyzz_to_affine(acc);
    Affine<Fq> out = q;
    if (!q.is_inf()) {
      out.x = L::repack_for_storage(q.x);
      out.y = L::repack_for_storage(q.y);
    }
    table[(size_t)w * n + i] = out;
  }
}

template <class Cfg>
int precompute_table_t(Bases* B, int c, int groups, hipStream_t st) {
  using Fq = typename Cfg::Fq;
  using Fr = typename Cfg::Fr;
  const int windows = windows_for(Fr::Params::BITS, c);
  const int asked = groups <= 0 || groups > windows ? windows : groups;
  CSH_REQUIRE(c <= 16 || asked == windows, "windows wider than 16 bits need one table row per window (groups = 0 or >= the window count)");
  const int wp = (windows + asked - 1) / asked;
  const int W = (windows + wp - 1) / wp;
  const int step = c * wp;
  void* t = nullptr;
  hipError_t e = hipMalloc(&t, sizeof(Affine<Fq>) * B->n * (size_t)W);
  if (e != hipSuccess) {
    set_error("hipMalloc(%zu bytes) for the fixed-base tables failed: %s", sizeof(Affine<Fq>) * B->n * (size_t)W, hipGetErrorString(e));
    return CSH_ERR_OOM;
  }
  hipLaunchKernelGGL(k_bases_precompute<Cfg>, dim3((unsigned)((B->n + 127) / 128)), dim3(128), 0, st, reinterpret_cast<const Affine<Fq>*>(B->points),
                     B->n, step, W, reinterpret_cast<Affine<Fq>*>(t));
  e = hipGetLastError();
  if (e == hipSuccess) e = hipStreamSynchronize(st);
  if (e != hipSuccess) {
    (void)hipFree(t);
    set_error("fixed-base table kernel failed: %s", hipGetErrorString(e));
    return CSH_ERR_HIP;
  }
  B->table = t;
  B->table_c = c;
  B->table_W = W;
  return CSH_OK;
}

template <class Cfg>
void fold_windows_erased(const void* wins_host, int W, int c, int wide, void* out_jacobian);

template <class F>
XYZZ<F> horner_windows(const XYZZ<F>* wins, int W, int c, int wide);
template <class Fq>
void fold_windows_host(const XYZZ<Fq>* wins32, int W, int c, int wide, void* out_jacobian) {
  using F = typename Host64<Fq>::type;
  static_assert(sizeof(XYZZ<F>) == sizeof(XYZZ<Fq>) && sizeof(Jac<F>) == sizeof(Jac<Fq>), "64-bit view must alias the device encoding");
  std::vector<XYZZ<F>> wins(W);
  memcpy((void*)wins.data(), wins32, sizeof(XYZZ<F>) * W);
  Affine<F> a = xyzz_to_affine(horner_windows<F>(wins.data(), W, c, wide));
  Jac<F> j = a.is_inf() ? Jac<F>::inf() : Jac<F>{a.x, a.y, F::one()};
  memcpy(out_jacobian, &j, sizeof(j));
}

template <class Cfg>
void fold_windows_erased(const void* wins_host, int W, int c, int wide, void* out_jacobian) {
  fold_windows_host<typename Cfg::Fq>(reinterpret_cast<const XYZZ<typename Cfg::Fq>*>(wins_host), W, c, wide, out_jacobian);
}

template <class Cfg>
int msm_t(const Bases* B, size_t offset, size_t n, const uint64_t* scalars_dev, int mont, void* out_host, hipStream_t st) {
  using Fq = typename Cfg::Fq;
  if (n == 0) {
    Jac<Fq> j = Jac<Fq>::inf();
    memcpy(out_host, &j, sizeof(j));
    return CSH_OK;
  }
  Arena& wa = arena_for((hipStream_t)((uintptr_t)st ^ 0x2));
  CSH_TRY(wa.reserve(sizeof(XYZZ<Fq>) * MAX_WINDOWS));
  XYZZ<Fq>* win_dev = wa.take<XYZZ<Fq>>(MAX_WINDOWS);
  MsmParams p;
  CSH_TRY((msm_windows_dev<Cfg>(B, offset, n, scalars_dev, mont, st, win_dev, &p)));
  void *pin_host = nullptr, *pin_dev = nullptr;
  std::vector<XYZZ<Fq>> pageable;
  XYZZ<Fq>* wins = nullptr;
  if (pinned_for(st, sizeof(XYZZ<Fq>) * MAX_WINDOWS, &pin_host, &pin_dev)) {
    wins = reinterpret_cast<XYZZ<Fq>*>(pin_host);
  } else {
    pageable.resize(p.W);
    wins = pageable.data();
  }
  CSH_HIP(hipMemcpyAsync(wins, win_dev, sizeof(XYZZ<Fq>) * p.W, hipMemcpyDeviceToHost, st));
  CSH_HIP(hipStreamSynchronize(st));
  fold_windows_host<Fq>(wins, p.W, p.c, p.wide, out_host);
  return CSH_OK;
}

template <int UNUSED = 0>
__global__ void k_msm_partial_header(PartialHeader* out, uint32_t c, uint32_t W, uint32_t wide) {
  PartialHeader h;
  h.magic = PARTIAL_MAGIC;
  h.c = c;
  h.W = W;
  h.wide = wide;
  for (int i = 0; i < 4; ++i) h.pad[i] = 0;
  *out = h;
}

template <class Cfg>
int msm_partial_t(const Bases* B, size_t offset, size_t n, const uint64_t* scalars_dev, int mont, void* out_dev, hipStream_t st, bool sync) {
  using Fq = typename Cfg::Fq;
  XYZZ<Fq>* wins = reinterpret_cast<XYZZ<Fq>*>(static_cast<char*>(out_dev) + sizeof(PartialHeader));
  CSH_HIP(hipMemsetAsync(out_dev, 0, sizeof(PartialHeader) + sizeof(XYZZ<Fq>) * MAX_WINDOWS, st));
  uint32_t c = 0, W = 0, wide = 0;
  if (n > 0) {
    MsmParams p;
    CSH_TRY((msm_windows_dev<Cfg>(B, offset, n, scalars_dev, mont, st, wins, &p)));
    c = (uint32_t)p.c;
    W = (uint32_t)p.W;
    wide = (uint32_t)p.wide;
  }
  hipLaunchKernelGGL(k_msm_partial_header<0>, dim3(1), dim3(1), 0, st, reinterpret_cast<PartialHeader*>(out_dev), c, W, wide);
  CSH_HIP(hipGetLastError());
  if (sync) CSH_HIP(hipStreamSynchronize(st));
  return CSH_OK;
}

template <class F>
XYZZ<F> xyzz_dbl_many_host(const XYZZ<F>& p, int c) {
  if (p.is_inf() || c <= 0) return p;
  const F zz2 = F::sqr(p.zz);
  F X = F::mul(p.x, zz2), Y = F::mul(p.y, F::mul(zz2, p.zz)), Z = p.zzz;
  for (int k = 0; k < c; ++k) {
    if (Y.is_zero()) return XYZZ<F>::inf();
    const F A = F::sqr(X), B = F::sqr(Y), C = F::sqr(B);
    const F t = F::add(X, B);
    const F D = F::mul2(F::sub(F::sub(F::sqr(t), A), C));
    const F E = F::mul3(A);
    const F X3 = F::sub(F::sqr(E), F::mul2(D));
    const F Y3 = F::sub(F::mul(E, F::sub(D, X3)), F::mul8(C));
    Z = F::mul2(F::mul(Y, Z));
    X = X3;
    Y = Y3;
  }
  const F ZZ = F::sqr(Z);
  return {X, Y, ZZ, F::mul(Z, ZZ)};
}

template <class F>
XYZZ<F> horner_windows(const XYZZ<F>* wins, int W, int c, int wide) {
  XYZZ<F> acc = XYZZ<F>::inf();
  for (int w = W - 1; w >= 0; --w) {
    acc = xyzz_dbl_many_host(acc, window_bits(c, wide, w));
    acc = xyzz_add_inl(acc, wins[w]);
  }
  return acc;
}

template <class Cfg>
int fold_partials_t(const void* partials_host, size_t nparts, void* out_jacobian) {
  using Fq = typename Cfg::Fq;
  using F = typename Host64<Fq>::type;
  const size_t stride = sizeof(PartialHeader) + sizeof(XYZZ<Fq>) * MAX_WINDOWS;
  XYZZ<F> total = XYZZ<F>::inf();
  std::vector<XYZZ<F>> sum;
  uint32_t sum_c = 0, sum_W = 0, sum_wide = 0;
  for (size_t k = 0; k < nparts; ++k) {
    const char* base = static_cast<const char*>(partials_host) + k * stride;
    PartialHeader h;
    memcpy(&h, base, sizeof h);
    CSH_REQUIRE(h.magic == PARTIAL_MAGIC, "fold_partials: bad partial header");
    if (h.W == 0) continue;
    CSH_REQUIRE(h.W <= (uint32_t)MAX_WINDOWS && h.c >= 2 && h.c <= 22 && h.wide <= h.W, "fold_partials: bad window parameters");
    const uint32_t wide = h.wide ? h.wide : h.W;
    std::vector<XYZZ<F>> wins(h.W);
    memcpy((void*)wins.data(), base + sizeof h, sizeof(XYZZ<F>) * h.W);
    if (sum.empty()) {
      sum.swap(wins);
      sum_c = h.c;
      sum_W = h.W;
      sum_wide = wide;
    } else if (h.c == sum_c && h.W == sum_W && wide == sum_wide) {
      for (uint32_t w = 0; w < h.W; ++w) sum[w] = xyzz_add_inl(sum[w], wins[w]);
    } else {
      total = xyzz_add_inl(total, horner_windows<F>(wins.data(), (int)h.W, (int)h.c, (int)wide));
    }
  }
  if (!sum.empty()) total = xyzz_add_inl(total, horner_windows<F>(sum.data(), (int)sum_W, (int)sum_c, (int)sum_wide));
  Affine<F> a = xyzz_to_affine(total);
  Jac<F> j = a.is_inf() ? Jac<F>::inf() : Jac<F>{a.x, a.y, F::one()};
  memcpy(out_jacobian, &j, sizeof(j));
  return CSH_OK;
}

template <class Cfg>
int repack_bases_t(Bases* B, hipStream_t st) {
  if constexpr (Cfg::LAZY) {
    if (B->n) {
      hipLaunchKernelGGL(k_bases_repack<Cfg>, dim3(grid_for(B->n, 256)), dim3(256), 0, st, (Affine<typename Cfg::Fq>*)B->points, B->n);
      CSH_HIP(hipGetLastError());
      CSH_HIP(hipStreamSynchronize(st));
    }
  }
  return CSH_OK;
}

template <class Cfg>
int msm_tail_selftest_t(const void* dense_host, uint32_t NB, uint32_t S, int form, void* win_out_host) {
  using Fq = typename Cfg::Fq;
  CSH_REQUIRE(dense_host && win_out_host && NB >= 1 && S >= 1 && NB <= (1u << 21) && S <= (1u << 16), "msm_tail_selftest: bad arguments");
  CSH_REQUIRE(form == 0 || form == 1 || (form == 2 && Cfg::PAIR), "msm_tail_selftest: unknown form");
  CSH_TRY(ensure_device());
  MsmParams p{};
  p.NB = NB;
  p.S = S;
  p.W = 1;
  p.wide = 1;
  const uint32_t fold_n1 = (S + 127) / 128;
  struct Mem {
    void* p = nullptr;
    ~Mem() {
      if (p) (void)hipFree(p);
    }
  } m_dense, m_seg, m_fa, m_fb, m_win;
  CSH_HIP(hipMalloc(&m_dense.p, ((size_t)NB + 1) * sizeof(LazyPt<Cfg>)));
  CSH_HIP(hipMalloc(&m_seg.p, (size_t)S * sizeof(LazyPt<Cfg>)));
  CSH_HIP(hipMalloc(&m_fa.p, (size_t)fold_n1 * sizeof(LazyPt<Cfg>)));
  CSH_HIP(hipMalloc(&m_fb.p, (size_t)fold_n1 * sizeof(LazyPt<Cfg>)));
  CSH_HIP(hipMalloc(&m_win.p, sizeof(XYZZ<Fq>)));
  CSH_HIP(hipMemcpy(m_dense.p, dense_host, ((size_t)NB + 1) * sizeof(LazyPt<Cfg>), hipMemcpyHostToDevice));
  const LazyPt<Cfg>* dense = reinterpret_cast<const LazyPt<Cfg>*>(m_dense.p);
  LazyPt<Cfg>* segres = reinterpret_cast<LazyPt<Cfg>*>(m_seg.p);
  LazyPt<Cfg>* fold_a = reinterpret_cast<LazyPt<Cfg>*>(m_fa.p);
  LazyPt<Cfg>* fold_b = reinterpret_cast<LazyPt<Cfg>*>(m_fb.p);
  XYZZ<Fq>* win_out = reinterpret_cast<XYZZ<Fq>*>(m_win.p);
  const hipStream_t st = nullptr;
  const uint32_t* no_start = nullptr;
  const LazyPt<Cfg>* no_partial = nullptr;
  if (form == 1) {
    hipLaunchKernelGGL((k_msm_reduce<Cfg, false>), dim3((S + 63) / 64, 1), dim3(256), 0, st, p, dense, segres, no_start, no_partial);
  } else if (form == 2) {
    if constexpr (Cfg::PAIR)
      hipLaunchKernelGGL((k_msm_reduce_pair<Cfg, false>), dim3((S + RED_BLK / 2 - 1) / (RED_BLK / 2), 1), dim3(RED_BLK), 0, st, p, dense, segres, no_start, no_partial);
  } else {
    hipLaunchKernelGGL(k_msm_reduce_serial<Cfg>, dim3((S + RED_BLK - 1) / RED_BLK, 1), dim3(RED_BLK), 0, st, p, dense, segres);
  }
  CSH_HIP(hipGetLastError());
  const LazyPt<Cfg>* cur = segres;
  uint32_t cur_n = S, cur_stride = S;
  LazyPt<Cfg>* nxt = fold_a;
  bool exported = false;
  while (cur_n > 1) {
    const uint32_t out_n = (cur_n + 127) / 128;
    exported = out_n == 1;
    hipLaunchKernelGGL(k_msm_fold_tree<Cfg>, dim3(out_n, 1), dim3(256), 0, st, cur, cur_stride, cur_n, nxt, fold_n1, exported ? win_out : (XYZZ<Fq>*)nullptr);
    cur = nxt;
    cur_n = out_n;
    cur_stride = fold_n1;
    nxt = nxt == fold_a ? fold_b : fold_a;
  }
  if (!exported) hipLaunchKernelGGL(k_msm_gather_windows<Cfg>, dim3(1), dim3(MAX_WINDOWS), 0, st, cur, cur_stride, 1, win_out);
  CSH_HIP(hipGetLastError());
  CSH_HIP(hipDeviceSynchronize());
  CSH_HIP(hipMemcpy(win_out_host, win_out, sizeof(XYZZ<Fq>), hipMemcpyDeviceToHost));
  return CSH_OK;
}

#define CSH_MSM_ACCUM_INSTANTIATE(KW, CFG)                                                                                               \
  KW template __global__ void k_msm_accum<CFG>(const Affine<typename CFG::Fq>* __restrict__, MsmParams, const uint32_t* __restrict__,  \
                                               const uint32_t* __restrict__, const uint32_t* __restrict__, LazyPt<CFG>*, uint32_t*);
#define CSH_MSM_ACCUM_PAIR_INSTANTIATE(KW, CFG)                                                                                               \
  KW template __global__ void k_msm_accum_pair<CFG>(const Affine<typename CFG::Fq>* __restrict__, MsmParams, const uint32_t* __restrict__,  \
                                                    const uint32_t* __restrict__, const uint32_t* __restrict__, LazyPt<CFG>*, uint32_t*);

#define CSH_MSM_INSTANTIATE(KW, CFG)                                                                                            \
  KW template int msm_t<CFG>(const Bases*, size_t, size_t, const uint64_t*, int, void*, hipStream_t);                           \
  KW template int msm_partial_t<CFG>(const Bases*, size_t, size_t, const uint64_t*, int, void*, hipStream_t, bool);                 \
  KW template int fold_partials_t<CFG>(const void*, size_t, void*);                                                             \
  KW template int repack_bases_t<CFG>(Bases*, hipStream_t);                                                                     \
  KW template int msm_tail_selftest_t<CFG>(const void*, uint32_t, uint32_t, int, void*);                                        \
  KW template size_t msm_bucket_bytes<CFG>(const MsmParams*);                                                                   \
  KW template int msm_bucket_stage<CFG>(const void*, const MsmParams*, const SortOut*, hipStream_t, Arena*, void*, hipEvent_t*);          \
  KW template int precompute_table_t<CFG>(Bases*, int, int, hipStream_t);                                                            \
  KW template void fold_windows_erased<CFG>(const void*, int, int, int, void*);

#define CURVE_DISPATCH(curve, group, CALL)                                                      \
  do {                                                                                          \
    if ((curve) == CSH_BN254 && (group) == CSH_G1) { using Cfg = csh::Bn254G1Cfg; return CALL; }     \
    if ((curve) == CSH_BN254 && (group) == CSH_G2) { using Cfg = csh::Bn254G2Cfg; return CALL; }     \
    if ((curve) == CSH_BLS12_381 && (group) == CSH_G1) { using Cfg = csh::Bls381G1Cfg; return CALL; } \
    if ((curve) == CSH_BLS12_381 && (group) == CSH_G2) { using Cfg = csh::Bls381G2Cfg; return CALL; } \
    if ((curve) == CSH_GRUMPKIN && (group) == CSH_G1) { using Cfg = csh::GrumpkinG1Cfg; return CALL; }  \
    if ((curve) == CSH_BLS12_377 && (group) == CSH_G1) { using Cfg = csh::Bls377G1Cfg; return CALL; } \
    if ((curve) == CSH_BLS12_377 && (group) == CSH_G2) { using Cfg = csh::Bls377G2Cfg; return CALL; } \
    (void)csh::group_ops(curve, group);               \
    return CSH_ERR_INVALID;                                                                     \
  } while (0)

struct GroupOps {
  csh_curve_t curve;
  csh_group_t group;
  int scalar_bits;
  size_t point_bytes;
  size_t xyzz_bytes;
  int (*sort)(const MsmParams&, const MsmParams&, const uint64_t*, hipStream_t, Arena&, SortOut*, hipEvent_t*);
  size_t (*bucket_bytes)(const MsmParams*);
  int (*bucket)(const void*, const MsmParams*, const SortOut*, hipStream_t, Arena*, void*, hipEvent_t*);
  void (*fold)(const void*, int, int, int, void*);
  int (*occ)();
};
const GroupOps* group_ops(csh_curve_t curve, csh_group_t group);
inline size_t partial_bytes_of(csh_curve_t c, csh_group_t g) { return sizeof(PartialHeader) + 2 * group_ops(c, g)->point_bytes * MAX_WINDOWS; }

}
```

### co-snarks_amd/csrc/msm_sort.hip

```cpp
#include <stdlib.h>

#include "msm_sort.hpp"

namespace csh {

__device__ __forceinline__ uint32_t entry_id(const MsmParams& p, size_t i) {
  if (p.remap_n == 0) return (uint32_t)i;
  const uint32_t f = (uint32_t)i;
  const uint32_t w = f / p.remap_n;
  return w * p.remap_stride + p.remap_off + (f - w * p.remap_n);
}

__global__ __launch_bounds__(SORT_BLK) void k_msm_hist_lds(MsmParams p, const uint16_t* __restrict__ dig, uint32_t* __restrict__ blkcnt,
                                                            uint32_t* __restrict__ part_cnt ) {
  extern __shared__ uint32_t lds_cnt[];
  const uint32_t ch = blockIdx.x, w = blockIdx.y;
  for (uint32_t b = threadIdx.x; b < p.NB; b += SORT_BLK) lds_cnt[b] = 0;
  __syncthreads();
  const size_t lo = (size_t)ch * p.chunk_len;
  size_t hi = lo + p.chunk_len;
  if (hi > p.n) hi = p.n;
  const uint16_t* d = dig + (size_t)w * p.n;
  for (size_t i0 = lo; i0 < hi; i0 += 4 * SORT_BLK) {
    uint32_t code[4];
#pragma unroll
    for (int k = 0; k < 4; ++k) {
      const size_t i = i0 + (size_t)k * SORT_BLK + threadIdx.x;
      code[k] = i < hi ? (uint32_t)d[i] : DIG_ZERO;
    }
#pragma unroll
    for (int k = 0; k < 4; ++k) (void)lds_slot(lds_cnt, code[k] & 0x7fffu, code[k] != DIG_ZERO);
  }
  __syncthreads();
  uint32_t* out = blkcnt + ((size_t)w * p.CH + ch) * p.NB;
  for (uint32_t b = threadIdx.x; b < p.NB; b += SORT_BLK) out[b] = lds_cnt[b];
  if (part_cnt) {
    const uint32_t P = p.NB / 256;
    const int lane = threadIdx.x & 63;
    for (uint32_t part = threadIdx.x >> 6; part < P; part += SORT_BLK / 64) {
      const uint32_t* c = lds_cnt + part * 256;
      uint32_t v = c[lane] + c[lane + 64] + c[lane + 128] + c[lane + 192];
#pragma unroll
      for (int d = 32; d >= 1; d >>= 1) v += (uint32_t)__shfl_xor((int)v, d);
      if (lane == 0) part_cnt[((size_t)w * p.CH + ch) * P + part] = v;
    }
  }
}

__global__ __launch_bounds__(256) void k_msm_colscan(MsmParams p, uint32_t* __restrict__ blkcnt, uint32_t* __restrict__ hist) {
  const uint32_t w = blockIdx.y;
  const uint32_t b = blockIdx.x * 256 + threadIdx.x;
  if (b >= p.NB) return;
  uint32_t acc = 0;
  uint32_t* col = blkcnt + (size_t)w * p.CH * p.NB + b;
  for (uint32_t ch0 = 0; ch0 < p.CH; ch0 += 8) {
    uint32_t t[8];
#pragma unroll
    for (uint32_t j = 0; j < 8; ++j) t[j] = ch0 + j < p.CH ? col[(size_t)(ch0 + j) * p.NB] : 0u;
#pragma unroll
    for (uint32_t j = 0; j < 8; ++j) {
      if (ch0 + j < p.CH) col[(size_t)(ch0 + j) * p.NB] = acc;
      acc += t[j];
    }
  }
  hist[(size_t)w * (p.NB + 2) + b + 1] = acc;
  if (b == 0) {
    hist[(size_t)w * (p.NB + 2)] = 0;
    hist[(size_t)w * (p.NB + 2) + p.NB + 1] = 0;
  }
}

__global__ __launch_bounds__(1024) void k_msm_scan(MsmParams p, uint32_t* hist, uint32_t* start, uint32_t* nlanes) {
  extern __shared__ uint32_t sc_lds[];
  const int w = blockIdx.x;
  const uint32_t len = p.NB + 2;
  uint32_t* h = hist + (size_t)w * len;
  uint32_t* st = start + (size_t)w * len;
  uint32_t* wave_tot = sc_lds + len;
  for (uint32_t b = threadIdx.x; b < len; b += 1024) sc_lds[b] = h[b];
  __syncthreads();
  const uint32_t per = (len + 1023) / 1024;
  const uint32_t b0 = threadIdx.x * per;
  uint32_t cnt = 0;
  for (uint32_t k = 0; k < per; ++k) {
    const uint32_t b = b0 + k;
    if (b < len) cnt += sc_lds[b];
  }
  uint32_t total;
  uint32_t run_c = block_excl_scan<16>(cnt, wave_tot, &total);
  for (uint32_t k = 0; k < per; ++k) {
    const uint32_t b = b0 + k;
    if (b < len) {
      const uint32_t cv = sc_lds[b];
      sc_lds[b] = run_c;
      run_c += cv;
    }
  }
  __syncthreads();
  for (uint32_t b = threadIdx.x; b < len; b += 1024) {
    st[b] = sc_lds[b];
    h[b] = sc_lds[b];
  }
  if (threadIdx.x == 0) nlanes[w] = (total + lane_len(p, w) - 1) / lane_len(p, w);
}

__global__ __launch_bounds__(SORT_BLK) void k_msm_scatter_lds(MsmParams p, const uint16_t* __restrict__ dig,
                                                               const uint32_t* __restrict__ start, const uint32_t* __restrict__ blkcnt,
                                                               uint32_t* __restrict__ sorted) {
  extern __shared__ uint32_t lds_cur[];
  const uint32_t ch = blockIdx.x, w = blockIdx.y;
  const uint32_t* st = start + (size_t)w * (p.NB + 2) + 1;
  const uint32_t* pre = blkcnt + ((size_t)w * p.CH + ch) * p.NB;
  for (uint32_t b = threadIdx.x; b < p.NB; b += SORT_BLK) lds_cur[b] = st[b] + pre[b];
  __syncthreads();
  const size_t lo = (size_t)ch * p.chunk_len;
  size_t hi = lo + p.chunk_len;
  if (hi > p.n) hi = p.n;
  const uint16_t* d = dig + (size_t)w * p.n;
  uint32_t* so = sorted + (size_t)w * p.n;
  for (size_t i0 = lo; i0 < hi; i0 += SORT_BLK) {
    const size_t i = i0 + threadIdx.x;
    uint32_t code = DIG_ZERO;
    if (i < hi) code = d[i];
    const bool valid = code != DIG_ZERO;
    const uint32_t pos = lds_slot(lds_cur, code & 0x7fffu, valid);
    if (valid) so[pos] = entry_id(p, i) | ((code >> 15) << 31);
  }
}


constexpr uint32_t PART_BUCKETS = 256;
constexpr uint32_t PART_LB = 8;
static_assert(PART_BUCKETS == 1u << PART_LB, "the record format's low key must hold a partition's bucket index");

__global__ __launch_bounds__(256) void k_msm_part_offsets(MsmParams p, const uint32_t* __restrict__ start, uint32_t* part_cnt) {
  const uint32_t P = p.NB / PART_BUCKETS;
  const uint32_t part = blockIdx.x * 256 + threadIdx.x, w = blockIdx.y;
  if (part >= P) return;
  uint32_t run = start[(size_t)w * (p.NB + 2) + (size_t)part * PART_BUCKETS + 1];
  uint32_t* col = part_cnt + (size_t)w * p.CH * P + part;
  for (uint32_t ch0 = 0; ch0 < p.CH; ch0 += 8) {
    uint32_t c[8];
#pragma unroll
    for (uint32_t j = 0; j < 8; ++j) c[j] = ch0 + j < p.CH ? col[(size_t)(ch0 + j) * P] : 0u;
#pragma unroll
    for (uint32_t j = 0; j < 8; ++j) {
      if (ch0 + j < p.CH) col[(size_t)(ch0 + j) * P] = run;
      run += c[j];
    }
  }
}

#ifndef CSH_L1_WPE
#define CSH_L1_WPE 8
#endif
#if CSH_L1_WPE > 0
#define CSH_L1_OCC __attribute__((amdgpu_waves_per_eu(CSH_L1_WPE)))
#else
#define CSH_L1_OCC
#endif
constexpr int L1_EPT = 8;
constexpr int L1_TILE = L1_EPT * SORT_BLK;
constexpr uint32_t MAXP = 128;
template <int REC>
__global__ __launch_bounds__(SORT_BLK) CSH_L1_OCC void k_msm_scatter_l1(MsmParams p, const uint16_t* __restrict__ dig, const uint32_t* __restrict__ part_off,
                                                             void* __restrict__ inter) {
  __shared__ uint32_t gcur[MAXP];
  __shared__ uint32_t cnt[MAXP];
  __shared__ uint32_t toff[MAXP];
  __shared__ uint32_t wsum[2];
  __shared__ uint32_t pay[L1_TILE];
  __shared__ uint8_t slo[L1_TILE];
  __shared__ uint8_t sbin[L1_TILE];
  const uint32_t ch = blockIdx.x, w = blockIdx.y, tid = threadIdx.x;
  const uint32_t P = p.NB / PART_BUCKETS;
  if (tid < MAXP) {
    gcur[tid] = tid < P ? part_off[((size_t)w * p.CH + ch) * P + tid] : 0;
    cnt[tid] = 0;
  }
  __syncthreads();
  const size_t lo = (size_t)ch * p.chunk_len;
  size_t hi = lo + p.chunk_len;
  if (hi > p.n) hi = p.n;
  const uint16_t* d = dig + (size_t)w * p.n;
  SortRec<REC>* out = reinterpret_cast<SortRec<REC>*>(inter) + (size_t)w * p.n;
  for (size_t t0 = lo; t0 < hi; t0 += L1_TILE) {
    uint32_t code[L1_EPT], rank[L1_EPT];
#pragma unroll
    for (int k = 0; k < L1_EPT; ++k) {
      const size_t i = t0 + (size_t)k * SORT_BLK + tid;
      code[k] = i < hi ? (uint32_t)__builtin_nontemporal_load(d + i) : DIG_ZERO;
    }
#pragma unroll
    for (int k = 0; k < L1_EPT; ++k) rank[k] = lds_slot(cnt, (code[k] & 0x7fffu) / PART_BUCKETS, code[k] != DIG_ZERO);
    __syncthreads();
    const uint32_t v = tid < MAXP ? cnt[tid] : 0;
    uint32_t tile_n;
    const uint32_t excl = block_excl_scan<MAXP / 64, SORT_BLK / 64>(v, wsum, &tile_n);
    if (tid < MAXP) toff[tid] = excl;
    __syncthreads();
#pragma unroll
    for (int k = 0; k < L1_EPT; ++k) {
      if (code[k] != DIG_ZERO) {
        const uint32_t b0 = code[k] & 0x7fffu;
        const uint32_t slot = toff[b0 / PART_BUCKETS] + rank[k];
        pay[slot] = entry_id(p, t0 + (size_t)k * SORT_BLK + tid) | ((code[k] >> 15) << 31);
        slo[slot] = (uint8_t)(b0 % PART_BUCKETS);
        sbin[slot] = (uint8_t)(b0 / PART_BUCKETS);
      }
    }
    __syncthreads();
#pragma unroll
    for (int k = 0; k < L1_EPT; ++k) {
      const uint32_t sl = k * SORT_BLK + tid;
      if (sl < tile_n) {
        const uint32_t bin = sbin[sl];
        out[gcur[bin] + (sl - toff[bin])] = rec_pack<REC>(pay[sl], slo[sl], PART_LB);
      }
    }
    __syncthreads();
    if (tid < MAXP) {
      gcur[tid] += v;
      cnt[tid] = 0;
    }
    __syncthreads();
  }
}

struct L2Lds {
  uint32_t obase[PART_BUCKETS];
  uint32_t cnt[PART_BUCKETS];
  uint32_t toff[PART_BUCKETS];
  uint32_t wsum[4];
  uint32_t pay[L2_TILE];
  uint8_t sbin[L2_TILE];
};
struct L2OwnRuns {
  __device__ void reserve(uint32_t*, uint32_t, uint32_t) const {}
  __device__ void advance(uint32_t* obase, uint32_t b, uint32_t v) const { obase[b] += v; }
};
struct L2SharedRuns {
  uint32_t* cur;
  __device__ void reserve(uint32_t* obase, uint32_t b, uint32_t v) const { obase[b] = v ? atomicAdd(&cur[b], v) : 0u; }
  __device__ void advance(uint32_t*, uint32_t, uint32_t) const {}
};
template <int REC, class Runs>
__device__ __forceinline__ void l2_sort_slice(L2Lds& s, const Runs runs, const SortRec<REC>* __restrict__ in, uint32_t lo, uint32_t hi,
                                              uint32_t* __restrict__ so) {
  const uint32_t tid = threadIdx.x;
  for (uint32_t t0 = lo; t0 < hi; t0 += L2_TILE) {
    SortRec<REC> e[L2_EPT];
    uint32_t rank[L2_EPT];
    l2_load_rank<REC>(in, t0, hi, PART_LB, s.cnt, e, rank);
    __syncthreads();
    uint32_t v = 0, total;
    if (tid < PART_BUCKETS) {
      v = s.cnt[tid];
      runs.reserve(s.obase, tid, v);
    }
    const uint32_t excl = block_excl_scan<PART_BUCKETS / 64, SORT_BLK / 64>(v, s.wsum, &total);
    if (tid < PART_BUCKETS) s.toff[tid] = excl;
    __syncthreads();
#pragma unroll
    for (int k = 0; k < L2_EPT; ++k) {
      if (t0 + k * SORT_BLK + tid < hi) {
        const uint32_t bin = rec_low<REC>(e[k], PART_LB);
        const uint32_t slot = s.toff[bin] + rank[k];
        s.pay[slot] = rec_entry<REC>(e[k], PART_LB);
        s.sbin[slot] = (uint8_t)bin;
      }
    }
    __syncthreads();
    const uint32_t tile_n = hi - t0 < (uint32_t)L2_TILE ? hi - t0 : (uint32_t)L2_TILE;
#pragma unroll
    for (int k = 0; k < L2_EPT; ++k) {
      const uint32_t sl = k * SORT_BLK + tid;
      if (sl < tile_n) {
        const uint32_t bin = s.sbin[sl];
        so[s.obase[bin] + (sl - s.toff[bin])] = s.pay[sl];
      }
    }
    __syncthreads();
    if (tid < PART_BUCKETS) {
      runs.advance(s.obase, tid, v);
      s.cnt[tid] = 0;
    }
    __syncthreads();
  }
}

template <int REC>
__global__ __launch_bounds__(SORT_BLK) void k_msm_scatter_l2(MsmParams p, const uint32_t* __restrict__ start, const void* __restrict__ inter,
                                                             uint32_t* __restrict__ sorted) {
  __shared__ L2Lds s;
  const uint32_t part = blockIdx.x, w = blockIdx.y, tid = threadIdx.x;
  const uint32_t* st = start + (size_t)w * (p.NB + 2) + (size_t)part * PART_BUCKETS + 1;
  if (tid < PART_BUCKETS) {
    s.obase[tid] = st[tid];
    s.cnt[tid] = 0;
  }
  __syncthreads();
  l2_sort_slice<REC>(s, L2OwnRuns{}, reinterpret_cast<const SortRec<REC>*>(inter) + (size_t)w * p.n, st[0], st[PART_BUCKETS],
                     sorted + (size_t)w * p.n);
}

template <int REC>
__global__ __launch_bounds__(SORT_BLK) void k_msm_scatter_l2t(MsmParams p, const uint32_t* __restrict__ start, uint32_t* __restrict__ cursor,
                                                              const void* __restrict__ inter, uint32_t* __restrict__ sorted) {
  __shared__ L2Lds s;
  __shared__ uint32_t job[3];
  const uint32_t x = blockIdx.x, w = blockIdx.y, tid = threadIdx.x;
  const uint32_t P = p.NB / PART_BUCKETS;
  const uint32_t* stw = start + (size_t)w * (p.NB + 2);
  {
    uint32_t lo_p = 0, hi_p = 0, nb = 0, total;
    if (tid < P) {
      lo_p = stw[(size_t)tid * PART_BUCKETS + 1];
      hi_p = stw[(size_t)(tid + 1) * PART_BUCKETS + 1];
      const uint32_t c = hi_p - lo_p;
      nb = c ? (c + L2_TILE / 2) / L2_TILE : 0;
      if (c && nb == 0) nb = 1;
    }
    if (tid == 0) job[0] = 0xffffffffu;
    const uint32_t pre = block_excl_scan<MAXP / 64, SORT_BLK / 64>(nb, s.wsum, &total);
    if (nb && x >= pre && x < pre + nb) {
      const uint32_t c = hi_p - lo_p, slice = (c + nb - 1) / nb, j = x - pre;
      uint32_t a = lo_p + j * slice, b = a + slice;
      if (b > hi_p) b = hi_p;
      if (a > hi_p) a = hi_p;
      job[0] = tid;
      job[1] = a;
      job[2] = b;
    }
    __syncthreads();
  }
  const uint32_t part = job[0];
  if (part == 0xffffffffu) return;
  if (tid < PART_BUCKETS) s.cnt[tid] = 0;
  __syncthreads();
  l2_sort_slice<REC>(s, L2SharedRuns{cursor + (size_t)w * (p.NB + 2) + (size_t)part * PART_BUCKETS + 1},
                     reinterpret_cast<const SortRec<REC>*>(inter) + (size_t)w * p.n, job[1], job[2], sorted + (size_t)w * p.n);
}

bool msm_sort_two_level(const MsmParams& p) {
  if (p.NB < 4 * PART_BUCKETS) return false;
  if (const int f = tune().sort_two_level.load(std::memory_order_relaxed); f >= 0) return f != 0;
  return p.n >= (1u << 20);
}

SortPath msm_sort_path(const MsmParams& p) {
  SortPath s{msm_sort_two_level(p), false, false};
  if (!s.two_level) return s;
  const uint64_t max_id = p.remap_n ? (uint64_t)(p.n / p.remap_n) * p.remap_stride : (uint64_t)p.n;
  const int variant = tune().msm_variant.load(std::memory_order_relaxed);
  s.rec4 = (variant & 8) == 0 && max_id <= (1u << (31 - PART_LB));
  s.per_partition = (variant & 32) != 0;
  return s;
}

template <int REC>
static void launch_two_level(const MsmParams& p, const SortBuffers& b, bool per_partition, hipStream_t st) {
  const uint32_t nparts = p.NB / PART_BUCKETS;
  hipLaunchKernelGGL(k_msm_scatter_l1<REC>, dim3(p.CH, p.W), dim3(SORT_BLK), 0, st, p, b.dig, b.part_cnt, (void*)b.inter);
  if (per_partition) {
    hipLaunchKernelGGL(k_msm_scatter_l2<REC>, dim3(nparts, p.W), dim3(SORT_BLK), 0, st, p, b.start, (const void*)b.inter, b.sorted);
  } else {
    const uint32_t l2_blocks = (uint32_t)(p.n / L2_TILE) + nparts + 1;
    hipLaunchKernelGGL(k_msm_scatter_l2t<REC>, dim3(l2_blocks, p.W), dim3(SORT_BLK), 0, st, p, b.start, b.hist, (const void*)b.inter, b.sorted);
  }
}

int msm_sort_launch(const MsmParams& p, const SortBuffers& b, hipStream_t st, hipEvent_t* ev) {
  const SortPath path = msm_sort_path(p);
  const bool two_level = path.two_level;
  const size_t sort_lds = sizeof(uint32_t) * p.NB;
  if (sort_lds > 48 * 1024) {
    CSH_TRY(raise_lds_limit((const void*)k_msm_hist_lds, 128 * 1024));
    CSH_TRY(raise_lds_limit((const void*)k_msm_scatter_lds, 128 * 1024));
  }
  hipLaunchKernelGGL(k_msm_hist_lds, dim3(p.CH, p.W), dim3(SORT_BLK), sort_lds, st, p, b.dig, b.blkcnt, two_level ? b.part_cnt : nullptr);
  hipLaunchKernelGGL(k_msm_colscan, dim3((p.NB + 255) / 256, p.W), dim3(256), 0, st, p, b.blkcnt, b.hist);
  if (ev) CSH_HIP(hipEventRecord(ev[1], st));
  {
    const size_t scan_lds = sizeof(uint32_t) * ((size_t)p.NB + 2 + 16);
    if (scan_lds > 48 * 1024) CSH_TRY(raise_lds_limit((const void*)k_msm_scan, 136 * 1024));
    hipLaunchKernelGGL(k_msm_scan, dim3(p.W), dim3(1024), scan_lds, st, p, b.hist, b.start, b.nlanes);
  }
  if (ev) CSH_HIP(hipEventRecord(ev[2], st));
  if (two_level) {
    hipLaunchKernelGGL(k_msm_part_offsets, dim3((p.NB / PART_BUCKETS + 255) / 256, p.W), dim3(256), 0, st, p, b.start, b.part_cnt);
    path.rec4 ? launch_two_level<1>(p, b, path.per_partition, st) : launch_two_level<0>(p, b, path.per_partition, st);
  } else {
    hipLaunchKernelGGL(k_msm_scatter_lds, dim3(p.CH, p.W), dim3(SORT_BLK), sort_lds, st, p, b.dig, b.start, b.blkcnt, b.sorted);
  }
  if (ev) CSH_HIP(hipEventRecord(ev[3], st));
  return CSH_OK;
}

}
```

### co-snarks_amd/csrc/msm_sort.hpp

```cpp
#pragma once
#include <type_traits>

#include "common.hpp"

namespace csh {

struct MsmParams {
  uint32_t n;
  int c;
  int W;
  uint32_t NB;
  uint32_t L;
  uint32_t tmax;
  uint32_t S;
  int mont;
  uint32_t CH;
  uint32_t chunk_len;
  uint32_t remap_n, remap_stride, remap_off;
  uint32_t dig_g, dig_wp;
  int wide;
  uint32_t Ln;
};
__host__ __device__ inline uint32_t lane_len(const MsmParams& p, int w) { return w >= p.wide ? p.Ln : p.L; }

constexpr uint32_t DIG_ZERO = 0xFFFFu;
constexpr int MAX_WINDOWS = 128;

struct SortBuffers {
  uint32_t* hist;
  uint32_t* start;
  uint32_t* nlanes;
  uint32_t* sorted;
  const uint16_t* dig;
  uint32_t* blkcnt;
  uint64_t* inter;
  uint32_t* part_cnt;
};

#if defined(__HIPCC__)
__device__ __forceinline__ uint32_t lds_slot(uint32_t* counter, uint32_t b, bool valid) {
  uint32_t slot = 0;
  bool todo = valid;
  for (int round = 0; round < 4; ++round) {
    const unsigned long long act = __ballot(todo);
    if (!act) return slot;
    const int leader = __ffsll((long long)act) - 1;
    const uint32_t lb = (uint32_t)__shfl((int)b, leader);
    const unsigned long long grp = __ballot(todo && b == lb);
    const int cnt = __popcll(grp);
    if (cnt < 8) break;
    uint32_t base = 0;
    const int lane = threadIdx.x & 63;
    if (lane == leader) base = atomicAdd(&counter[lb], (uint32_t)cnt);
    base = (uint32_t)__shfl((int)base, leader);
    if (todo && b == lb) {
      slot = base + (uint32_t)__popcll(grp & ((1ull << lane) - 1ull));
      todo = false;
    }
  }
  if (todo) slot = atomicAdd(&counter[b], 1u);
  return slot;
}

__device__ __forceinline__ uint32_t wave_incl_scan(uint32_t v) {
  const int lane = threadIdx.x & 63;
#pragma unroll
  for (int d = 1; d < 64; d <<= 1) {
    const uint32_t up = (uint32_t)__shfl_up((int)v, d);
    if (lane >= d) v += up;
  }
  return v;
}

template <int NW, int BLOCK_WAVES = NW>
__device__ __forceinline__ uint32_t block_excl_scan(uint32_t v, uint32_t* wsum, uint32_t* total) {
  const int lane = threadIdx.x & 63, wv = threadIdx.x >> 6;
  uint32_t incl = 0;
  if (BLOCK_WAVES == NW || wv < NW) {
    incl = wave_incl_scan(v);
    if (lane == 63) wsum[wv] = incl;
  }
  __syncthreads();
  uint32_t base = 0, tot = 0;
#pragma unroll
  for (int i = 0; i < NW; ++i) {
    const uint32_t t = wsum[i];
    if (i < wv) base += t;
    tot += t;
  }
  *total = tot;
  return base + incl - v;
}

template <int REC>
using SortRec = typename std::conditional<REC != 0, uint32_t, uint64_t>::type;
template <int REC>
__device__ __forceinline__ SortRec<REC> rec_pack(uint32_t entry, uint32_t low, uint32_t lb) {
  if constexpr (REC == 1) {
    const uint32_t idb = 31 - lb;
    return (entry & ((1u << idb) - 1)) | ((entry >> 31) << idb) | (low << (idb + 1));
  } else {
    return (uint64_t)entry | ((uint64_t)low << 32);
  }
}
template <int REC>
__device__ __forceinline__ uint32_t rec_low(SortRec<REC> e, uint32_t lb) {
  if constexpr (REC == 1) return e >> (32 - lb);
  else return (uint32_t)(e >> 32);
}
template <int REC>
__device__ __forceinline__ uint32_t rec_entry(SortRec<REC> e, uint32_t lb) {
  if constexpr (REC == 1) {
    const uint32_t idb = 31 - lb;
    return (e & ((1u << idb) - 1)) | (((e >> idb) & 1u) << 31);
  } else {
    return (uint32_t)e;
  }
}

constexpr int SORT_BLK = 1024;
constexpr int L2_EPT = 8;
constexpr int L2_TILE = L2_EPT * SORT_BLK;
template <int REC>
__device__ __forceinline__ void l2_load_rank(const SortRec<REC>* __restrict__ in, uint32_t t0, uint32_t hi, uint32_t lb, uint32_t* cnt,
                                             SortRec<REC>* e, uint32_t* rank) {
#pragma unroll
  for (int k = 0; k < L2_EPT; ++k) {
    const uint32_t i = t0 + k * SORT_BLK + threadIdx.x;
    e[k] = i < hi ? __builtin_nontemporal_load(in + i) : 0;
  }
#pragma unroll
  for (int k = 0; k < L2_EPT; ++k) rank[k] = lds_slot(cnt, rec_low<REC>(e[k], lb), t0 + k * SORT_BLK + threadIdx.x < hi);
}
#endif

bool msm_sort_two_level(const MsmParams& p);
struct SortPath {
  bool two_level;
  bool rec4;
  bool per_partition;
};
SortPath msm_sort_path(const MsmParams& p);
int msm_sort_launch(const MsmParams& p, const SortBuffers& b, hipStream_t st, hipEvent_t* ev);

}
```

### co-snarks_amd/csrc/selftest_dev.hip

```cpp
#define CSH_CHECK_BOUNDS_DEVICE 1
#include <string.h>

#include <vector>

#include "msm_impl.hpp"

using namespace csh;

namespace csh {
#define CSH_ST_TAIL_DECL(CFG) extern template int msm_tail_selftest_t<CFG>(const void*, uint32_t, uint32_t, int, void*);
CSH_ST_TAIL_DECL(Bn254G1Cfg)
CSH_ST_TAIL_DECL(Bn254G2Cfg)
CSH_ST_TAIL_DECL(Bls381G1Cfg)
CSH_ST_TAIL_DECL(Bls381G2Cfg)
CSH_ST_TAIL_DECL(GrumpkinG1Cfg)
CSH_ST_TAIL_DECL(Bls377G1Cfg)
CSH_ST_TAIL_DECL(Bls377G2Cfg)
}

namespace {

struct DevMem {
  void* p = nullptr;
  ~DevMem() {
    if (p) (void)hipFree(p);
  }
  int alloc(size_t bytes) {
    CSH_HIP(hipMalloc(&p, bytes ? bytes : 1));
    return CSH_OK;
  }
  template <class T>
  T* as() { return reinterpret_cast<T*>(p); }
};

int bound_record_clear() {
  const unsigned long long z[2] = {0, 0};
  CSH_HIP(hipMemcpyToSymbol(HIP_SYMBOL(g_bound_record), z, sizeof z));
  return CSH_OK;
}
int bound_record_take(uint64_t rec[3]) {
  unsigned long long r[2];
  CSH_HIP(hipDeviceSynchronize());
  CSH_HIP(hipMemcpyFromSymbol(r, HIP_SYMBOL(g_bound_record), sizeof r));
  rec[0] = r[0];
  rec[1] = r[1] >> 16;
  rec[2] = r[1] & 0xffff;
  return bound_record_clear();
}

template <class LF>
__global__ void k_st_bound_control(int64_t* sink) {
  LF a, b;
  for (int i = 0; i < LF::NL; ++i) {
    a.l[i] = (int32_t)(1u << (LF::B + 2));
    b.l[i] = 3;
  }
  const typename LF::Wide w = LF::mul_wide(a, b);
  int64_t s = 0;
  for (int k = 0; k < 2 * LF::NL; ++k) s += w.t[k];
  sink[threadIdx.x] = s;
}
template <class LF>
int bound_control_t(uint64_t rec[3]) {
  DevMem sink;
  CSH_TRY(sink.alloc(64 * sizeof(int64_t)));
  CSH_TRY(bound_record_clear());
  hipLaunchKernelGGL(k_st_bound_control<LF>, dim3(1), dim3(64), 0, 0, sink.as<int64_t>());
  CSH_HIP(hipGetLastError());
  return bound_record_take(rec);
}

template <class LP, class F32>
__global__ __launch_bounds__(256) void k_st_fp2pair_raw(int op, const int32_t* __restrict__ limbs, uint32_t npairs, F32* out) {
  constexpr int NL = LP::NL;
  const uint32_t t = blockIdx.x * 256 + threadIdx.x, j = t >> 1;
  const int role = pair_role();
  if (j >= npairs) return;
  LP v[4];
  for (int e = 0; e < 4; ++e)
    for (int i = 0; i < NL; ++i) v[e].v.l[i] = limbs[(((size_t)j * 4 + e) * 2 + role) * NL + i];
  LP r;
  if (op == 0) r = LP::mul(v[0], v[1]);
  else if (op == 1) r = LP::sqr(v[0]);
  else if (op == 2) r = LP::sqr_sub(v[0], v[1]);
  else r = LP::mul_sub(v[0], v[1], v[2], v[3]);
  out[2 * (size_t)j + role] = r.v.to_fp();
}
template <class LP, class F32>
int fp2pair_raw_t(int op, const int32_t* limbs, size_t npairs, uint64_t* out, uint64_t rec[3]) {
  const size_t in_bytes = npairs * 8 * LP::NL * sizeof(int32_t), out_bytes = npairs * 2 * sizeof(F32);
  DevMem din, dout;
  CSH_TRY(din.alloc(in_bytes));
  CSH_TRY(dout.alloc(out_bytes));
  CSH_HIP(hipMemcpy(din.p, limbs, in_bytes, hipMemcpyHostToDevice));
  CSH_TRY(bound_record_clear());
  hipLaunchKernelGGL((k_st_fp2pair_raw<LP, F32>), dim3((unsigned)((2 * npairs + 255) / 256)), dim3(256), 0, 0, op, din.as<int32_t>(), (uint32_t)npairs,
                     dout.as<F32>());
  CSH_HIP(hipGetLastError());
  CSH_TRY(bound_record_take(rec));
  CSH_HIP(hipMemcpy(out, dout.p, out_bytes, hipMemcpyDeviceToHost));
  return CSH_OK;
}

template <class LP>
__global__ __launch_bounds__(256) void k_st_fp2pair_zero(const int32_t* __restrict__ limbs, uint32_t npairs, uint8_t* flags) {
  constexpr int NL = LP::NL;
  const uint32_t t = blockIdx.x * 256 + threadIdx.x, j = t >> 1;
  const int role = pair_role();
  if (j >= npairs) return;
  LP v;
  for (int i = 0; i < NL; ++i) v.v.l[i] = limbs[((size_t)j * 2 + role) * NL + i];
  const bool m = v.maybe_zero(), s = v.is_zero_slow(), z = v.is_zero();
  if (role == 0) flags[j] = (uint8_t)((m ? 1 : 0) | (s ? 2 : 0) | (z ? 4 : 0));
}
template <class LP>
int fp2pair_zero_t(const int32_t* limbs, size_t npairs, uint8_t* flags, uint64_t rec[3]) {
  const size_t in_bytes = npairs * 2 * LP::NL * sizeof(int32_t);
  DevMem din, dout;
  CSH_TRY(din.alloc(in_bytes));
  CSH_TRY(dout.alloc(npairs));
  CSH_HIP(hipMemcpy(din.p, limbs, in_bytes, hipMemcpyHostToDevice));
  CSH_TRY(bound_record_clear());
  hipLaunchKernelGGL(k_st_fp2pair_zero<LP>, dim3((unsigned)((2 * npairs + 255) / 256)), dim3(256), 0, 0, din.as<int32_t>(), (uint32_t)npairs, dout.as<uint8_t>());
  CSH_HIP(hipGetLastError());
  CSH_TRY(bound_record_take(rec));
  CSH_HIP(hipMemcpy(flags, dout.p, npairs, hipMemcpyDeviceToHost));
  return CSH_OK;
}

template <class L, class Fq>
void build_slots(const Affine<Fq>* pts, const uint8_t* neg, const uint32_t* off, size_t nslots, XYZZLazy<L>* out) {
  for (size_t s = 0; s < nslots; ++s) {
    XYZZLazy<L> acc = XYZZLazy<L>::inf();
    for (uint32_t i = off[s]; i < off[s + 1]; ++i) {
      Affine<Fq> p;
      memcpy(&p, pts + i, sizeof p);
      if (p.is_inf()) continue;
      L x = L::unpack(L::repack_for_storage(p.x)), y = L::unpack(L::repack_for_storage(p.y));
      if (neg && neg[i]) y = y.neg_unpacked();
      lazy_madd(acc, x, y);
    }
    memset(&out[s], 0, sizeof out[s]);
    out[s].x = acc.x;
    out[s].y = acc.y;
    out[s].zz = acc.zz;
    out[s].zzz = acc.zzz;
    out[s].empty = acc.empty;
  }
}

struct StOp {
  uint32_t code, reg, arg, k;
};
enum : uint32_t {
  ST_LOAD = 0,
  ST_ADDP = 1,
  ST_ADDR = 2,
  ST_ADDS = 3,
  ST_DBL = 4,
  ST_MULK = 5,
  ST_MADD = 6,
  ST_ADDK = 7,
  ST_NOPS = 8
};

template <class T>
__device__ __forceinline__ void st_swap(T& a, T& b) {
  const T t = a;
  a = b;
  b = t;
}

template <class L>
__global__ __launch_bounds__(256) void k_st_quad_ops(const XYZZLazy<L>* __restrict__ slots, const StOp* __restrict__ ops, const uint32_t* __restrict__ unit_off,
                                                     uint32_t nunits, XYZZLazy<L>* out) {
  const int role = threadIdx.x & 3;
  const uint32_t u = (blockIdx.x * 256 + threadIdx.x) >> 2;
  if (u >= nunits) return;
  QPt<L> d = qpt_inf<L>(), o = qpt_inf<L>();
  for (uint32_t i = unit_off[u]; i < unit_off[u + 1]; ++i) {
    const StOp op = ops[i];
    if (op.reg & 1) st_swap(d, o);
    QPt<L> p = qpt_inf<L>();
    bool add = false;
    if (op.code == ST_LOAD || op.code == ST_ADDP) {
      p = qpt_load<L>(&slots[op.arg], role);
      if (op.code == ST_LOAD) d = p;
      else add = true;
    } else if (op.code == ST_ADDR) {
      p = o;
      add = true;
    } else if (op.code == ST_ADDS) {
      p = d;
      add = true;
    } else if (op.code == ST_MULK || op.code == ST_ADDK) {
      p = qmul_small<L>(op.code == ST_ADDK ? o : d, op.k, role);
      if (op.code == ST_MULK) d = p;
      else add = true;
    }
    if (add) qadd<L>(d, p, role);
    if (op.code == ST_DBL) qdbl<L>(d, role);
    if (op.reg & 1) st_swap(d, o);
  }
  qpt_store<L>(&out[2 * (size_t)u], role, d);
  qpt_store<L>(&out[2 * (size_t)u + 1], role, o);
}

template <class LS, class LP, class Fq>
__global__ __launch_bounds__(256) void k_st_pair_ops(const XYZZLazy<LS>* __restrict__ slots, const Affine<Fq>* __restrict__ aff, const StOp* __restrict__ ops,
                                                     const uint32_t* __restrict__ unit_off, uint32_t nunits, XYZZLazy<LS>* out) {
  const int role = pair_role();
  const uint32_t u = (blockIdx.x * 256 + threadIdx.x) >> 1;
  if (u >= nunits) return;
  XYZZLazy<LP> d = XYZZLazy<LP>::inf(), o = XYZZLazy<LP>::inf();
  for (uint32_t i = unit_off[u]; i < unit_off[u + 1]; ++i) {
    const StOp op = ops[i];
    if (op.reg & 1) st_swap(d, o);
    XYZZLazy<LP> p = XYZZLazy<LP>::inf();
    bool add = false;
    if (op.code == ST_LOAD || op.code == ST_ADDP) {
      p = pair_load(&slots[op.arg], role);
      if (op.code == ST_LOAD) d = p;
      else add = true;
    } else if (op.code == ST_ADDR) {
      p = o;
      add = true;
    } else if (op.code == ST_ADDS) {
      p = d;
      add = true;
    } else if (op.code == ST_MULK || op.code == ST_ADDK) {
      p = lazy_mul_small<LP, true>(op.code == ST_ADDK ? o : d, op.k);
      if (op.code == ST_MULK) d = p;
      else add = true;
    } else if (op.code == ST_MADD) {
      LP x, y;
      pair_unpack_affine<LP, Affine<Fq>>(aff + op.arg, &x, &y);
      y = y.cneg_unpacked(op.k & 1u);
      lazy_madd<LP, Affine<Fq>>(d, x, y, aff + op.arg, op.k & 1u);
    }
    if (add) lazy_add_inl<LP>(d, p);
    if (op.code == ST_DBL) d = lazy_dbl_inl<LP>(d);
    if (op.reg & 1) st_swap(d, o);
  }
  pair_store(&out[2 * (size_t)u], role, d);
  pair_store(&out[2 * (size_t)u + 1], role, o);
}

template <class L, class Fq>
__global__ __launch_bounds__(128) void k_st_export(const XYZZLazy<L>* __restrict__ in, uint32_t n, XYZZ<Fq>* out) {
  const uint32_t i = blockIdx.x * 128 + threadIdx.x;
  if (i < n) out[i] = lazy_to_xyzz<L, Fq>(in[i]);
}

template <class L, class LP, class Fq>
int point_ops_t(int form, const void* affine_pts, const uint8_t* neg, size_t npts, const uint32_t* slot_off, size_t nslots, const uint32_t* ops_words,
                const uint32_t* unit_off, size_t nunits, void* out_xyzz, uint64_t rec[3]) {
  constexpr bool HAS_PAIR = !std::is_void<LP>::value;
  if (form != 1 && !(form == 2 && HAS_PAIR)) return CSH_ERR_INVALID;
  if (!nunits || !nslots || nunits > (1u << 20) || nslots > (1u << 20)) return CSH_ERR_INVALID;
  const Affine<Fq>* pts = reinterpret_cast<const Affine<Fq>*>(affine_pts);
  for (size_t s = 0; s < nslots; ++s)
    if (slot_off[s] > slot_off[s + 1] || slot_off[s + 1] > npts) return CSH_ERR_INVALID;
  const size_t nops = unit_off[nunits];
  const StOp* ops = reinterpret_cast<const StOp*>(ops_words);
  for (size_t u = 0; u < nunits; ++u)
    if (unit_off[u] > unit_off[u + 1]) return CSH_ERR_INVALID;
  for (size_t i = 0; i < nops; ++i) {
    const StOp& o = ops[i];
    if (o.code >= ST_NOPS || o.reg > 1) return CSH_ERR_INVALID;
    if ((o.code == ST_LOAD || o.code == ST_ADDP) && o.arg >= nslots) return CSH_ERR_INVALID;
    if (o.code == ST_MADD) {
      if (form != 2 || o.arg >= npts) return CSH_ERR_INVALID;
      Affine<Fq> p;
      memcpy(&p, pts + o.arg, sizeof p);
      if (p.is_inf()) return CSH_ERR_INVALID;
    }
  }
  std::vector<XYZZLazy<L>> slots(nslots);
  build_slots<L, Fq>(pts, neg, slot_off, nslots, slots.data());
  std::vector<Affine<Fq>> stored(npts ? npts : 1);
  for (size_t i = 0; i < npts; ++i) {
    memcpy(&stored[i], pts + i, sizeof(Affine<Fq>));
    if (!stored[i].is_inf()) stored[i] = {L::repack_for_storage(stored[i].x), L::repack_for_storage(stored[i].y)};
  }
  DevMem dslots, daff, dops, doff, dout, dx;
  CSH_TRY(dslots.alloc(nslots * sizeof(XYZZLazy<L>)));
  CSH_TRY(daff.alloc(stored.size() * sizeof(Affine<Fq>)));
  CSH_TRY(dops.alloc(nops * sizeof(StOp)));
  CSH_TRY(doff.alloc((nunits + 1) * sizeof(uint32_t)));
  CSH_TRY(dout.alloc(2 * nunits * sizeof(XYZZLazy<L>)));
  CSH_TRY(dx.alloc(2 * nunits * sizeof(XYZZ<Fq>)));
  CSH_HIP(hipMemcpy(dslots.p, slots.data(), nslots * sizeof(XYZZLazy<L>), hipMemcpyHostToDevice));
  CSH_HIP(hipMemcpy(daff.p, stored.data(), stored.size() * sizeof(Affine<Fq>), hipMemcpyHostToDevice));
  if (nops) CSH_HIP(hipMemcpy(dops.p, ops, nops * sizeof(StOp), hipMemcpyHostToDevice));
  CSH_HIP(hipMemcpy(doff.p, unit_off, (nunits + 1) * sizeof(uint32_t), hipMemcpyHostToDevice));
  CSH_HIP(hipMemset(dout.p, 0, 2 * nunits * sizeof(XYZZLazy<L>)));
  CSH_TRY(bound_record_clear());
  if (form == 1) {
    hipLaunchKernelGGL(k_st_quad_ops<L>, dim3((unsigned)((4 * nunits + 255) / 256)), dim3(256), 0, 0, dslots.as<XYZZLazy<L>>(), dops.as<StOp>(),
                       doff.as<uint32_t>(), (uint32_t)nunits, dout.as<XYZZLazy<L>>());
  } else {
    if constexpr (HAS_PAIR)
      hipLaunchKernelGGL((k_st_pair_ops<L, LP, Fq>), dim3((unsigned)((2 * nunits + 255) / 256)), dim3(256), 0, 0, dslots.as<XYZZLazy<L>>(),
                         daff.as<Affine<Fq>>(), dops.as<StOp>(), doff.as<uint32_t>(), (uint32_t)nunits, dout.as<XYZZLazy<L>>());
  }
  CSH_HIP(hipGetLastError());
  hipLaunchKernelGGL((k_st_export<L, Fq>), dim3((unsigned)((2 * nunits + 127) / 128)), dim3(128), 0, 0, dout.as<XYZZLazy<L>>(), (uint32_t)(2 * nunits),
                     dx.as<XYZZ<Fq>>());
  CSH_HIP(hipGetLastError());
  CSH_TRY(bound_record_take(rec));
  CSH_HIP(hipMemcpy(out_xyzz, dx.p, 2 * nunits * sizeof(XYZZ<Fq>), hipMemcpyDeviceToHost));
  return CSH_OK;
}

template <class Cfg>
int msm_tail_t(int form, const void* affine_pts, const uint8_t* neg, size_t npts, const uint32_t* ids, const uint32_t* off, size_t nocc, uint32_t NB, uint32_t S,
               void* out_xyzz) {
  using L = typename Cfg::L;
  using Fq = typename Cfg::Fq;
  if (NB < 1 || NB > (1u << 16) || S < 1 || S > (1u << 16) || nocc > NB) return CSH_ERR_INVALID;
  for (size_t i = 0; i < nocc; ++i)
    if (ids[i] < 1 || ids[i] > NB || off[i] > off[i + 1] || off[i + 1] > npts) return CSH_ERR_INVALID;
  std::vector<XYZZLazy<L>> occ(nocc ? nocc : 1);
  build_slots<L, Fq>(reinterpret_cast<const Affine<Fq>*>(affine_pts), neg, off, nocc, occ.data());
  std::vector<XYZZLazy<L>> dense((size_t)NB + 1);
  memset((void*)dense.data(), 0, dense.size() * sizeof(XYZZLazy<L>));
  for (auto& d : dense) d.empty = true;
  for (size_t i = 0; i < nocc; ++i) dense[ids[i]] = occ[i];
  return msm_tail_selftest_t<Cfg>(dense.data(), NB, S, form, out_xyzz);
}

enum : int {
  SI_C = 0, SI_W, SI_WIDE, SI_NB, SI_L, SI_LN, SI_DIG_G, SI_DIG_WP, SI_REMAP_N, SI_REMAP_STRIDE, SI_REMAP_OFF,
  SI_SRT_N, SI_SRT_W, SI_SRT_WIDE,
  SI_PATH,
  SI_REC_BYTES,
  SI_PER_PARTITION,
  SI_WIDE_LB,
  SI_CH, SI_CHUNK_LEN,
  SI_WORDS = 24
};
int msm_sort_selftest(csh_curve_t curve, const uint64_t* scalars, size_t n, int mont, const uint64_t* table, uint32_t* info, uint32_t* start, size_t start_words,
                      uint32_t* nlanes, uint32_t* sorted, size_t sorted_words) {
  const GroupOps* G = group_ops(curve, CSH_G1);
  if (!G) return CSH_ERR_INVALID;
  CSH_REQUIRE(scalars && info, "selftest_msm_sort: NULL argument");
  CSH_REQUIRE(n >= 1 && n <= (size_t(1) << 24), "selftest_msm_sort: n out of range");
  CSH_TRY(ensure_device());
  MsmTable tb{};
  if (table) {
    CSH_REQUIRE(table[0] >= 2 && table[0] <= 22 && table[1] >= 1, "selftest_msm_sort: table window width or rows out of range");
    tb = MsmTable{(int)table[0], 0, (size_t)table[2], (size_t)table[3]};
    CSH_REQUIRE(table[1] <= (uint64_t)windows_for(G->scalar_bits, tb.c), "selftest_msm_sort: more table rows than windows");
    tb.rows = (int)table[1];
    CSH_REQUIRE(table[3] <= table[2] && n <= table[2] - table[3], "selftest_msm_sort: offset + n exceeds the table's stride");
    CSH_REQUIRE((uint64_t)tb.stride * tb.rows < (uint64_t(1) << 31) && (uint64_t)n * tb.rows < (uint64_t(1) << 31), "selftest_msm_sort: table ids exceed 31 bits");
  }
  const MsmPlan plan = msm_plan(n, G->scalar_bits, mont ? 1 : 0, 1, table ? &tb : nullptr);
  const MsmParams &p = plan.srt, &pd = plan.dig;
  const bool wide = msm_sort_is_wide(p);
  CSH_REQUIRE(p.c <= 16 || wide, "selftest_msm_sort: windows wider than 16 bits need one table row per window");
  memset(info, 0, SI_WORDS * sizeof(uint32_t));
  info[SI_C] = (uint32_t)pd.c, info[SI_W] = (uint32_t)pd.W, info[SI_WIDE] = (uint32_t)pd.wide, info[SI_NB] = p.NB, info[SI_L] = p.L, info[SI_LN] = p.Ln;
  info[SI_DIG_G] = pd.dig_g, info[SI_DIG_WP] = pd.dig_wp, info[SI_REMAP_N] = p.remap_n, info[SI_REMAP_STRIDE] = p.remap_stride, info[SI_REMAP_OFF] = p.remap_off;
  info[SI_SRT_N] = p.n, info[SI_SRT_W] = (uint32_t)p.W, info[SI_SRT_WIDE] = (uint32_t)p.wide;
  if (wide) {
    const WidePlan wp = msm_wide_plan(p, pd);
    info[SI_PATH] = 2, info[SI_REC_BYTES] = wp.rec4 ? 4 : 8, info[SI_WIDE_LB] = wp.lb, info[SI_CH] = wp.CH, info[SI_CHUNK_LEN] = wp.chunk_tiles * 512;
  } else {
    const SortPath sp = msm_sort_path(p);
    info[SI_PATH] = sp.two_level ? 1 : 0, info[SI_REC_BYTES] = sp.two_level ? (sp.rec4 ? 4 : 8) : 0, info[SI_PER_PARTITION] = sp.per_partition ? 1 : 0;
    info[SI_CH] = p.CH, info[SI_CHUNK_LEN] = p.chunk_len;
  }
  if (!start && !nlanes && !sorted) return CSH_OK;
  const size_t nstart = ((size_t)p.NB + 2) * p.W, nsorted = (size_t)p.n * p.W;
  CSH_REQUIRE(start && nlanes && sorted && start_words >= nstart && sorted_words >= nsorted, "selftest_msm_sort: output buffers too small");
  DevMem dsc;
  CSH_TRY(dsc.alloc(32 * n));
  CSH_HIP(hipMemcpy(dsc.p, scalars, 32 * n, hipMemcpyHostToDevice));
  hipStream_t st = resolve_stream(nullptr);
  Arena& ar = arena_for(st);
  const size_t bytes = msm_sort_bytes(p, pd);
  CSH_TRY(ar.reserve(bytes));
  CSH_HIP(hipMemset(ar.base, 0xFF, bytes));
  CSH_HIP(hipDeviceSynchronize());
  SortOut so{};
  CSH_TRY(G->sort(p, pd, dsc.as<uint64_t>(), st, ar, &so, nullptr));
  CSH_HIP(hipGetLastError());
  CSH_HIP(hipStreamSynchronize(st));
  CSH_HIP(hipMemcpy(start, so.start, nstart * sizeof(uint32_t), hipMemcpyDeviceToHost));
  CSH_HIP(hipMemcpy(nlanes, so.nlanes, (size_t)p.W * sizeof(uint32_t), hipMemcpyDeviceToHost));
  CSH_HIP(hipMemcpy(sorted, so.sorted, nsorted * sizeof(uint32_t), hipMemcpyDeviceToHost));
  return CSH_OK;
}

template <class Launch>
int fused_form(const uint64_t* subtrahend, uint64_t* out, size_t n, int alias, Launch launch) {
  if (n == 0) return CSH_OK;
  const size_t eb = 32 * n;
  DevMem dsub, dout;
  CSH_TRY(dout.alloc(eb));
  if (alias) {
    CSH_HIP(hipMemcpy(dout.p, subtrahend, eb, hipMemcpyHostToDevice));
  } else {
    CSH_HIP(hipMemset(dout.p, 0xFF, eb));
    if (subtrahend) {
      CSH_TRY(dsub.alloc(eb));
      CSH_HIP(hipMemcpy(dsub.p, subtrahend, eb, hipMemcpyHostToDevice));
    }
  }
  CSH_HIP(hipDeviceSynchronize());
  hipStream_t st = resolve_stream(nullptr);
  CSH_TRY(launch(alias ? dout.as<uint64_t>() : dsub.as<uint64_t>(), dout.as<uint64_t>(), st));
  CSH_HIP(hipStreamSynchronize(st));
  CSH_HIP(hipMemcpy(out, dout.p, eb, hipMemcpyDeviceToHost));
  return CSH_OK;
}
int upload_operand(DevMem& d, const uint64_t* host, size_t bytes) {
  CSH_TRY(d.alloc(bytes));
  CSH_HIP(hipMemcpy(d.p, host, bytes, hipMemcpyHostToDevice));
  return CSH_OK;
}

}

#define ST_GROUP_DISPATCH(curve, group, CALL)                                                                                                   \
  do {                                                                                                                                          \
    if ((curve) == CSH_BN254 && (group) == CSH_G1) { using Cfg = Bn254G1Cfg; using L = Fq29s; using LP = void; using Fq = Bn254Fq; return CALL; }           \
    if ((curve) == CSH_BN254 && (group) == CSH_G2) { using Cfg = Bn254G2Cfg; using L = Fq29s2; using LP = Bn254G2Cfg::LP; using Fq = Bn254Fq2; return CALL; } \
    if ((curve) == CSH_BLS12_381 && (group) == CSH_G1) { using Cfg = Bls381G1Cfg; using L = Fq28s; using LP = void; using Fq = Bls381Fq; return CALL; }     \
    if ((curve) == CSH_BLS12_381 && (group) == CSH_G2) { using Cfg = Bls381G2Cfg; using L = Fq28s2; using LP = Bls381G2Cfg::LP; using Fq = Bls381Fq2; return CALL; } \
    if ((curve) == CSH_GRUMPKIN && (group) == CSH_G1) { using Cfg = GrumpkinG1Cfg; using L = Fr29s; using LP = void; using Fq = Bn254Fr; return CALL; }      \
    if ((curve) == CSH_BLS12_377 && (group) == CSH_G1) { using Cfg = Bls377G1Cfg; using L = Fq28s377; using LP = void; using Fq = Bls377Fq; return CALL; }  \
    if ((curve) == CSH_BLS12_377 && (group) == CSH_G2) { using Cfg = Bls377G2Cfg; using L = Fq28s377x2; using LP = Bls377G2Cfg::LP; using Fq = Bls377Fq2; return CALL; } \
    return CSH_ERR_INVALID;                                                                                                                     \
  } while (0)

extern "C" {

int csh_selftest_bound_control_dev(int type, uint64_t rec[3]) {
  CSH_TRY(ensure_device());
  switch (type) {
    case 0: return bound_control_t<Fq29s>(rec);
    case 1: return bound_control_t<Fq28s>(rec);
    case 2: return bound_control_t<Fr29s>(rec);
    case 3: return bound_control_t<Fq28s377>(rec);
    default: return CSH_ERR_INVALID;
  }
}

int csh_selftest_fp2pair_raw_dev(int curve, int op, const int32_t* limbs, size_t npairs, uint64_t* out, uint64_t rec[3]) {
  CSH_TRY(ensure_device());
  if (op < 0 || op > 3 || !npairs || npairs > (1u << 20)) return CSH_ERR_INVALID;
  if (curve == CSH_BN254) return fp2pair_raw_t<Bn254G2Cfg::LP, Bn254Fq>(op, limbs, npairs, out, rec);
  if (curve == CSH_BLS12_381) return fp2pair_raw_t<Bls381G2Cfg::LP, Bls381Fq>(op, limbs, npairs, out, rec);
  if (curve == CSH_BLS12_377) return fp2pair_raw_t<Bls377G2Cfg::LP, Bls377Fq>(op, limbs, npairs, out, rec);
  return CSH_ERR_INVALID;
}

int csh_selftest_fp2pair_zero_dev(int curve, const int32_t* limbs, size_t npairs, uint8_t* flags, uint64_t rec[3]) {
  CSH_TRY(ensure_device());
  if (!npairs || npairs > (1u << 20)) return CSH_ERR_INVALID;
  if (curve == CSH_BN254) return fp2pair_zero_t<Bn254G2Cfg::LP>(limbs, npairs, flags, rec);
  if (curve == CSH_BLS12_381) return fp2pair_zero_t<Bls381G2Cfg::LP>(limbs, npairs, flags, rec);
  if (curve == CSH_BLS12_377) return fp2pair_zero_t<Bls377G2Cfg::LP>(limbs, npairs, flags, rec);
  return CSH_ERR_INVALID;
}

int csh_selftest_point_ops_dev(int curve, int group, int form, const void* affine_pts, const uint8_t* neg, size_t npts, const uint32_t* slot_off, size_t nslots,
                               const uint32_t* ops, const uint32_t* unit_off, size_t nunits, void* out_xyzz, uint64_t rec[3]) {
  CSH_TRY(ensure_device());
  ST_GROUP_DISPATCH(curve, group, (point_ops_t<L, LP, Fq>(form, affine_pts, neg, npts, slot_off, nslots, ops, unit_off, nunits, out_xyzz, rec)));
}

int csh_selftest_msm_tail_dev(int curve, int group, int form, const void* affine_pts, const uint8_t* neg, size_t npts, const uint32_t* bucket_ids,
                              const uint32_t* bucket_off, size_t nocc, uint32_t NB, uint32_t S, void* out_xyzz) {
  CSH_TRY(ensure_device());
  ST_GROUP_DISPATCH(curve, group, (msm_tail_t<Cfg>(form, affine_pts, neg, npts, bucket_ids, bucket_off, nocc, NB, S, out_xyzz)));
}

int csh_selftest_msm_sort_dev(int curve, const uint64_t* scalars, size_t n, int mont, const uint64_t* table, uint32_t* info, uint32_t* start, size_t start_words,
                              uint32_t* nlanes, uint32_t* sorted, size_t sorted_words) {
  return msm_sort_selftest((csh_curve_t)curve, scalars, n, mont, table, info, start, start_words, nlanes, sorted, sorted_words);
}

int csh_selftest_vec_mul_sub_dev(int curve, const uint64_t* a, const uint64_t* b, const uint64_t* c, uint64_t* out, size_t n, int c_aliases_out) {
  CSH_REQUIRE((a && b && c && out) || n == 0, "selftest_vec_mul_sub: NULL argument");
  CSH_TRY(ensure_device());
  DevMem da, db;
  if (n) {
    CSH_TRY(upload_operand(da, a, 32 * n));
    CSH_TRY(upload_operand(db, b, 32 * n));
  }
  return fused_form(c, out, n, c_aliases_out, [&](const uint64_t* dc, uint64_t* dout, hipStream_t st) {
    return vec_mul_sub_dev((csh_curve_t)curve, da.as<uint64_t>(), db.as<uint64_t>(), dc, dout, n, st);
  });
}

int csh_selftest_rep3_local_mul_sub_dev(int curve, const uint64_t* lhs, const uint64_t* rhs, const uint64_t* mask, const uint64_t* sub, uint64_t* out, size_t n,
                                        int sub_aliases_out) {
  CSH_REQUIRE((lhs && rhs && out) || n == 0, "selftest_rep3_local_mul_sub: NULL argument");
  CSH_REQUIRE(sub || !sub_aliases_out, "selftest_rep3_local_mul_sub: no sub operand to put into the output buffer");
  CSH_TRY(ensure_device());
  DevMem dl, dr, dm;
  if (n) {
    CSH_TRY(upload_operand(dl, lhs, 64 * n));
    CSH_TRY(upload_operand(dr, rhs, 64 * n));
    if (mask) CSH_TRY(upload_operand(dm, mask, 32 * n));
  }
  return fused_form(sub, out, n, sub_aliases_out, [&](const uint64_t* ds, uint64_t* dout, hipStream_t st) {
    return rep3_local_mul_sub_dev((csh_curve_t)curve, dl.as<uint64_t>(), dr.as<uint64_t>(), dm.as<uint64_t>(), ds, dout, n, st);
  });
}

}
```

Baseline: 658.9 million points/s.

## Fork bucket scans onto aux stream, gate giant kernels, use binary-GCD host inverse

The two-level sort now runs the column scan and bucket-start scan on an auxiliary stream, concurrently with the partition-offset and level-1 scatter kernels, and joins before level 2. Partition offsets are computed independently with a block scan, and colscan can skip its write-back. A small kernel counts oversized buckets into pinned memory so the host can skip the giant slice/merge kernels when none exist, at the cost of a host sync mid-pipeline. The host field inverse switches from exponentiation to binary extended GCD.

```diff
diff --git a/co-snarks_amd/csrc/host_fp64.hpp b/co-snarks_amd/csrc/host_fp64.hpp
--- a/co-snarks_amd/csrc/host_fp64.hpp
+++ b/co-snarks_amd/csrc/host_fp64.hpp
@@ -16,7 +16,7 @@
 
 template <int N>
 struct Fp64Consts {
-  uint64_t mod[N], one[N], pm2[N];
+  uint64_t mod[N], one[N], pm2[N], r2[N];
   uint64_t inv;
 };
 template <class P>
@@ -26,6 +26,7 @@
     k.mod[i] = (uint64_t)P::MOD[2 * i] | ((uint64_t)P::MOD[2 * i + 1] << 32);
     k.one[i] = (uint64_t)P::R1[2 * i] | ((uint64_t)P::R1[2 * i + 1] << 32);
     k.pm2[i] = (uint64_t)P::PM2[2 * i] | ((uint64_t)P::PM2[2 * i + 1] << 32);
+    k.r2[i] = (uint64_t)P::R2[2 * i] | ((uint64_t)P::R2[2 * i + 1] << 32);
   }
   uint64_t y = k.mod[0];
   for (int i = 0; i < 6; ++i) y *= 2 - k.mod[0] * y;
@@ -193,22 +194,92 @@
   static Fp64 mul3(const Fp64& a) { return add(add(a, a), a); }
   static Fp64 mul4(const Fp64& a) { return mul2(mul2(a)); }
   static Fp64 mul8(const Fp64& a) { return mul2(mul4(a)); }
+  static void shr1(uint64_t* x) {
+    CSH_HOST_UNROLL
+    for (int i = 0; i + 1 < N; ++i) x[i] = (x[i] >> 1) | (x[i + 1] << 63);
+    x[N - 1] >>= 1;
+  }
+  static void halve_mod(uint64_t* x) {
+    if (x[0] & 1) {
+      u128 c = 0;
+      CSH_HOST_UNROLL
+      for (int i = 0; i < N; ++i) {
+        c += (u128)x[i] + K.mod[i];
+        x[i] = (uint64_t)c;
+        c >>= 64;
+      }
+    }
+    shr1(x);
+  }
+  static bool sub_words(uint64_t* x, const uint64_t* y) {
+    uint64_t br = 0;
+    CSH_HOST_UNROLL
+    for (int i = 0; i < N; ++i) {
+      const u128 d = (u128)x[i] - y[i] - br;
+      x[i] = (uint64_t)d;
+      br = (uint64_t)(d >> 64) & 1;
+    }
+    return br != 0;
+  }
+  static void sub_mod_words(uint64_t* x, const uint64_t* y) {
+    if (sub_words(x, y)) {
+      u128 c = 0;
+      CSH_HOST_UNROLL
+      for (int i = 0; i < N; ++i) {
+        c += (u128)x[i] + K.mod[i];
+        x[i] = (uint64_t)c;
+        c >>= 64;
+      }
+    }
+  }
+  static bool geq_words(const uint64_t* x, const uint64_t* y) {
+    CSH_HOST_UNROLL
+    for (int i = N - 1; i >= 0; --i) {
+      if (x[i] > y[i]) return true;
+      if (x[i] < y[i]) return false;
+    }
+    return true;
+  }
+  static bool is_one_words(const uint64_t* x) {
+    uint64_t hi = 0;
+    CSH_HOST_UNROLL
+    for (int i = 1; i < N; ++i) hi |= x[i];
+    return x[0] == 1 && hi == 0;
+  }
   static Fp64 inv(const Fp64& a) {
-    Fp64 pw[16];
-    pw[0] = one();
-    pw[1] = a;
-    for (int i = 2; i < 16; ++i) pw[i] = (i & 1) ? mul(pw[i - 1], a) : sqr(pw[i / 2]);
-    Fp64 r = one();
-    bool started = false;
-    for (int i = 16 * N - 1; i >= 0; --i) {
-      const unsigned d = (unsigned)(K.pm2[i >> 4] >> (4 * (i & 15))) & 15u;
-      if (started) r = sqr(sqr(sqr(sqr(r))));
-      if (d) {
-        r = started ? mul(r, pw[d]) : pw[d];
-        started = true;
-      }
-    }
-    return r;
+    if (a.is_zero()) return a;
+    uint64_t u[N], v[N];
+    Fp64 b, c = zero();
+    CSH_HOST_UNROLL
+    for (int i = 0; i < N; ++i) {
+      u[i] = a.l[i];
+      v[i] = K.mod[i];
+      b.l[i] = K.r2[i];
+    }
+    if (geq_words(u, v)) sub_words(u, v);
+    for (;;) {
+      uint64_t z = 0;
+      CSH_HOST_UNROLL
+      for (int i = 0; i < N; ++i) z |= u[i];
+      if (z == 0) return zero();
+      while (!(u[0] & 1)) {
+        shr1(u);
+        halve_mod(b.l);
+      }
+      if (is_one_words(u)) return b;
+      while (!(v[0] & 1)) {
+        shr1(v);
+        halve_mod(c.l);
+      }
+      if (is_one_words(v)) return c;
+      if (geq_words(u, v)) {
+        sub_words(u, v);
+        sub_mod_words(b.l, c.l);
+      } else {
+        sub_words(v, u);
+        sub_mod_words(c.l, b.l);
+      }
+    }
   }
 
   static Fp64 mul_looped(const Fp64& a, const Fp64& b) {
diff --git a/co-snarks_amd/csrc/msm.hip b/co-snarks_amd/csrc/msm.hip
--- a/co-snarks_amd/csrc/msm.hip
+++ b/co-snarks_amd/csrc/msm.hip
@@ -559,8 +559,10 @@
   if (tune().msm_multi_overlap.load(std::memory_order_relaxed) != 0 && k > 1) aux = resolve_aux_stream();
   const bool two = aux != nullptr;
   Events evs;
-  CSH_TRY(evs.create(k + (two ? 2 : 0), hipEventDisableTiming));
+  CSH_TRY(evs.create(k + (two ? 4 : 0), hipEventDisableTiming));
   const hipEvent_t sorted_ev = two ? evs[k] : nullptr, aux_done = two ? evs[k + 1] : nullptr;
+  const SortFork fork{aux, two ? evs[k + 2] : nullptr, two ? evs[k + 3] : nullptr};
+  const bool forking = two && (tune().msm_variant.load(std::memory_order_relaxed) & 128) == 0;
   auto body = [&]() -> int {
     SortOut so;
     std::vector<char*> win_dev(k);
@@ -580,7 +582,7 @@
           p.remap_stride = (uint32_t)(sorted_stride = B->n);
           p.remap_off = (uint32_t)(sorted_off = offsets[i]);
         }
-        CSH_TRY(ops[0]->sort(p, pdig, scalars_dev, st, ar, &so, nullptr));
+        CSH_TRY(ops[0]->sort(p, pdig, scalars_dev, st, ar, &so, nullptr, forking ? &fork : nullptr));
         mark = ar.off;
         if (two) {
           CSH_HIP(hipEventRecord(sorted_ev, st));
@@ -593,7 +595,7 @@
       ar.off = mark + (on_aux ? Arena::padded(bucket_max) : 0);
       win_dev[i] = wa.take<char>(ops[i]->xyzz_bytes * MAX_WINDOWS);
       const void* src = merged ? B->table : static_cast<const char*>(B->points) + offsets[i] * B->point_bytes;
-      CSH_TRY(ops[i]->bucket(src, &p, &so, stage_stream[i], &ar, win_dev[i], nullptr));
+      CSH_TRY(ops[i]->bucket(src, &p, &so, stage_stream[i], &ar, win_dev[i], nullptr, nullptr));
     }
     void *pin_host = nullptr, *pin_dev = nullptr;
     std::vector<char> pageable;
diff --git a/co-snarks_amd/csrc/msm_impl.hpp b/co-snarks_amd/csrc/msm_impl.hpp
--- a/co-snarks_amd/csrc/msm_impl.hpp
+++ b/co-snarks_amd/csrc/msm_impl.hpp
@@ -227,6 +227,9 @@
 constexpr int MERGE_Q = MERGE_BLK / 4;
 
 constexpr uint32_t MERGE_CAP = 16;
+__device__ __forceinline__ bool bucket_oversized(uint32_t lo, uint32_t hi, uint32_t Lw) {
+  return hi > lo && (hi - 1) / Lw - lo / Lw >= MERGE_CAP;
+}
 constexpr uint32_t GIANT_BIG = 256, GIANT_SLICES = 16, GIANT_BIG_CAP = 128, GIANT_ROWS = 32, GIANT_SLICED_FLAG = 0x80000000u;
 __device__ __forceinline__ void giant_enqueue(uint32_t* giant_count, uint32_t* giant_list, uint32_t* big_list, uint32_t w, uint32_t b, uint32_t nparts) {
   uint32_t tag = w;
@@ -264,7 +267,7 @@
     QPt<L> acc = qpt_inf<L>();
     if (hi > lo) {
       const uint32_t k0 = lo / Lw, k1 = (hi - 1) / Lw;
-      if (k1 - k0 >= MERGE_CAP) {
+      if (bucket_oversized(lo, hi, Lw)) {
         if (role == 0) giant_enqueue(giant_count, giant_list, big_list, (uint32_t)w, b, k1 - k0 + 1);
       } else {
         acc = qpt_load<L>(&pw[b + k0], role);
@@ -370,7 +373,27 @@
   const uint32_t* st = start + (size_t)w * (p.NB + 2);
   const uint32_t lo = st[b], hi = st[b + 1];
   const uint32_t Lw = lane_len(p, w);
-  if (hi > lo && (hi - 1) / Lw - lo / Lw >= MERGE_CAP) giant_enqueue(giant_count, giant_list, big_list, (uint32_t)w, b, (hi - 1) / Lw - lo / Lw + 1);
+  if (bucket_oversized(lo, hi, Lw)) giant_enqueue(giant_count, giant_list, big_list, (uint32_t)w, b, (hi - 1) / Lw - lo / Lw + 1);
+}
+template <class Cfg>
+__global__ __launch_bounds__(1024) void k_msm_count_giant(MsmParams p, const uint32_t* __restrict__ start, uint32_t* out) {
+  __shared__ uint32_t wave_cnt[16];
+  const int w = blockIdx.x;
+  const uint32_t* st = start + (size_t)w * (p.NB + 2);
+  const uint32_t Lw = lane_len(p, w);
+  uint32_t cnt = 0;
+#pragma unroll 4
+  for (uint32_t b = threadIdx.x + 1; b <= p.NB; b += 1024) cnt += bucket_oversized(st[b], st[b + 1], Lw) ? 1u : 0u;
+#pragma unroll
+  for (int d = 32; d >= 1; d >>= 1) cnt += (uint32_t)__shfl_xor((int)cnt, d);
+  if ((threadIdx.x & 63) == 0) wave_cnt[threadIdx.x >> 6] = cnt;
+  __syncthreads();
+  if (threadIdx.x == 0) {
+    uint32_t total = 0;
+#pragma unroll
+    for (int i = 0; i < 16; ++i) total += wave_cnt[i];
+    __hip_atomic_store(out + w, total, __ATOMIC_RELAXED, __HIP_MEMORY_SCOPE_SYSTEM);
+  }
 }
 template <class Cfg>
 __device__ __forceinline__ QPt<typename Cfg::L> qbucket_merged(uint32_t Lw, const uint32_t* __restrict__ st, const LazyPt<Cfg>* __restrict__ pw,
@@ -602,6 +625,12 @@
   hipEvent_t operator[](size_t i) const { return ev[i]; }
 };
 
+struct GiantGate {
+  hipEvent_t counted;
+  const volatile uint32_t* counts;
+  uint32_t* counts_dev;
+};
+
 struct PartialHeader {
   uint32_t magic, c, W, wide;
   uint32_t pad[4];
@@ -664,11 +693,12 @@
   return CSH_OK;
 }
 template <class Fr>
-int msm_sort_stage(const MsmParams& p, const MsmParams& pdig, const uint64_t* scalars_dev, hipStream_t st, Arena& ar, SortOut* out, hipEvent_t* ev) {
+int msm_sort_stage(const MsmParams& p, const MsmParams& pdig, const uint64_t* scalars_dev, hipStream_t st, Arena& ar, SortOut* out, hipEvent_t* ev,
+                   const SortFork* fork) {
   if (msm_sort_is_wide(p)) return msm_sort_wide_launch(fr_id_of<Fr>(), p, pdig, scalars_dev, st, ar, &out->start, &out->nlanes, &out->sorted, ev);
   SortStageBufs ss;
   CSH_TRY(msm_sort_prepare<Fr>(p, pdig, scalars_dev, st, ar, &ss));
-  CSH_TRY(msm_sort_launch(p, ss.sb, st, ev));
+  CSH_TRY(msm_sort_launch(p, ss.sb, st, ev, fork));
   *out = SortOut{ss.sb.start, ss.sb.nlanes, ss.sb.sorted};
   return CSH_OK;
 }
@@ -708,7 +738,7 @@
 
 template <class Cfg>
 int bucket_group(const void* points, const MsmParams& p_all, const SortOut& so, const BucketBufs<Cfg>& bb, int w0, int nw, int group, hipStream_t st,
-                 void* win_out_dev, hipEvent_t* ev) {
+                 void* win_out_dev, hipEvent_t* ev, const GiantGate* gate) {
   using Fq = typename Cfg::Fq;
   MsmParams p = p_all;
   p.wide = p_all.wide > w0 ? p_all.wide - w0 : 0;
@@ -725,6 +755,10 @@
   uint32_t* big = bb.big + (size_t)2 * GIANT_BIG_CAP * group;
   LazyPt<Cfg>* gscratch = bb.gscratch + (size_t)GIANT_BIG_CAP * GIANT_SLICES * group;
   const Affine<Fq>* bases = reinterpret_cast<const Affine<Fq>*>(points);
+  if (gate) {
+    hipLaunchKernelGGL(k_msm_count_giant<Cfg>, dim3(nw), dim3(1024), 0, st, p, start, gate->counts_dev + w0);
+    CSH_HIP(hipEventRecord(gate->counted, st));
+  }
   {
     const int tb = tune().acc_blk.load(std::memory_order_relaxed);
     const int blk = (tb == 64 || tb == 128) ? tb : ACC_BLK;
@@ -751,8 +785,17 @@
     hipLaunchKernelGGL(k_msm_mark_giant<Cfg>, dim3((p.NB + 255) / 256, nw), dim3(256), 0, st, p, start, giant, giant + 2, big);
   else
     hipLaunchKernelGGL(k_msm_merge<Cfg>, dim3((p.NB + MERGE_Q - 1) / MERGE_Q, nw), dim3(MERGE_BLK), 0, st, p, start, partial, dense, giant, giant + 2, big);
-  hipLaunchKernelGGL(k_msm_giant_slices<Cfg>, dim3(GIANT_SLICES, GIANT_ROWS), dim3(256), 0, st, p, start, partial, giant, big, gscratch);
-  hipLaunchKernelGGL(k_msm_merge_giant<Cfg>, dim3(bb.giant_blocks), dim3(256), 0, st, p, start, partial, dense, giant, giant + 2, big, gscratch);
+  bool oversized = true;
+  if (gate) {
+    CSH_HIP(hipEventSynchronize(gate->counted));
+    uint32_t queued = 0;
+    for (int w = 0; w < nw; ++w) queued |= gate->counts[w0 + w];
+    oversized = queued != 0;
+  }
+  if (oversized) {
+    hipLaunchKernelGGL(k_msm_giant_slices<Cfg>, dim3(GIANT_SLICES, GIANT_ROWS), dim3(256), 0, st, p, start, partial, giant, big, gscratch);
+    hipLaunchKernelGGL(k_msm_merge_giant<Cfg>, dim3(bb.giant_blocks), dim3(256), 0, st, p, start, partial, dense, giant, giant + 2, big, gscratch);
+  }
   MsmParams pr = p;
   if (form == 1) {
     pr.S = std::min(p.S, reduce_segments(p.NB, p.W, 4));
@@ -789,10 +832,11 @@
 }
 
 template <class Cfg>
-int msm_bucket_stage(const void* points, const MsmParams* pp, const SortOut* so, hipStream_t st, Arena* arp, void* win_out_dev, hipEvent_t* ev) {
+int msm_bucket_stage(const void* points, const MsmParams* pp, const SortOut* so, hipStream_t st, Arena* arp, void* win_out_dev, hipEvent_t* ev,
+                     const GiantGate* gate) {
   const MsmParams& p = *pp;
   const BucketBufs<Cfg> bb = bucket_take<Cfg>(p, *arp);
-  CSH_TRY((bucket_group<Cfg>(points, p, *so, bb, 0, p.W, 0, st, win_out_dev, ev)));
+  CSH_TRY((bucket_group<Cfg>(points, p, *so, bb, 0, p.W, 0, st, win_out_dev, ev, gate)));
   if (ev) CSH_HIP(hipEventRecord(ev[5], st));
   return CSH_OK;
 }
@@ -821,9 +865,15 @@
   return v;
 }
 
+inline hipStream_t msm_fork_stream(const MsmParams& p, hipStream_t st, bool syncs) {
+  if (!syncs || st != resolve_stream(nullptr) || msm_sort_is_wide(p) || !msm_sort_two_level(p)) return nullptr;
+  if (tune().msm_multi_overlap.load(std::memory_order_relaxed) == 0 || (tune().msm_variant.load(std::memory_order_relaxed) & 128) != 0) return nullptr;
+  return resolve_aux_stream();
+}
+
 template <class Cfg>
 int msm_windows_dev(const Bases* B, size_t offset, size_t n, const uint64_t* scalars_dev, int mont, hipStream_t st,
-                    XYZZ<typename Cfg::Fq>* win_out_dev , MsmParams* p_out) {
+                    XYZZ<typename Cfg::Fq>* win_out_dev , MsmParams* p_out, const GiantGate* gate, bool syncs) {
   using Fr = typename Cfg::Fr;
   using Fq = typename Cfg::Fq;
   const MsmTable table{B->table_c, B->table_W, B->n, offset};
@@ -841,15 +891,27 @@
     CSH_HIP(hipEventRecord(timed[0], st));
   }
   hipEvent_t* ev = timing ? timed.ev.data() : nullptr;
-  SortOut so;
-  CSH_TRY(msm_sort_stage<Fr>(p, pdig, scalars_dev, st, ar, &so, ev));
-  CSH_TRY(msm_bucket_stage<Cfg>(points, &p, &so, st, &ar, win_out_dev, ev));
-  if (timing) {
-    CSH_HIP(hipEventSynchronize(ev[5]));
-    for (int i = 0; i < 5; ++i) CSH_HIP(hipEventElapsedTime(&tl_msm_timing[i], ev[i], ev[i + 1]));
-    CSH_HIP(hipEventElapsedTime(&tl_msm_timing[5], ev[0], ev[5]));
-  }
-  return CSH_OK;
+  hipStream_t aux = timing ? nullptr : msm_fork_stream(p, st, syncs);
+  Events forks;
+  if (aux) CSH_TRY(forks.create(2, hipEventDisableTiming));
+  const SortFork fork{aux, aux ? forks[0] : nullptr, aux ? forks[1] : nullptr};
+  auto body = [&]() -> int {
+    SortOut so;
+    CSH_TRY(msm_sort_stage<Fr>(p, pdig, scalars_dev, st, ar, &so, ev, aux ? &fork : nullptr));
+    CSH_TRY(msm_bucket_stage<Cfg>(points, &p, &so, st, &ar, win_out_dev, ev, gate));
+    if (timing) {
+      CSH_HIP(hipEventSynchronize(ev[5]));
+      for (int i = 0; i < 5; ++i) CSH_HIP(hipEventElapsedTime(&tl_msm_timing[i], ev[i], ev[i + 1]));
+      CSH_HIP(hipEventElapsedTime(&tl_msm_timing[5], ev[0], ev[5]));
+    }
+    return CSH_OK;
+  };
+  const int rc = body();
+  if (rc != CSH_OK && aux) {
+    (void)hipStreamSynchronize(st);
+    (void)hipStreamSynchronize(aux);
+  }
+  return rc;
 }
 
 template <class Cfg>
@@ -942,12 +1004,26 @@
   Arena& wa = arena_for((hipStream_t)((uintptr_t)st ^ 0x2));
   CSH_TRY(wa.reserve(sizeof(XYZZ<Fq>) * MAX_WINDOWS));
   XYZZ<Fq>* win_dev = wa.take<XYZZ<Fq>>(MAX_WINDOWS);
+  void *pin_host = nullptr, *pin_dev = nullptr;
+  const size_t wins_bytes = sizeof(XYZZ<Fq>) * MAX_WINDOWS;
+  const bool pinned = pinned_for(st, wins_bytes + sizeof(uint32_t) * MAX_WINDOWS, &pin_host, &pin_dev);
+  Events counted;
+  GiantGate gate{};
+  const bool gated = pinned && (tune().msm_variant.load(std::memory_order_relaxed) & 256) == 0;
+  if (gated) {
+    CSH_TRY(counted.create(1, hipEventDisableTiming | hipEventReleaseToSystem));
+    gate = GiantGate{counted[0], reinterpret_cast<const volatile uint32_t*>(static_cast<char*>(pin_host) + wins_bytes),
+                     reinterpret_cast<uint32_t*>(static_cast<char*>(pin_dev) + wins_bytes)};
+  }
   MsmParams p;
-  CSH_TRY((msm_windows_dev<Cfg>(B, offset, n, scalars_dev, mont, st, win_dev, &p)));
-  void *pin_host = nullptr, *pin_dev = nullptr;
+  const int rc = msm_windows_dev<Cfg>(B, offset, n, scalars_dev, mont, st, win_dev, &p, gated ? &gate : nullptr, true);
+  if (rc != CSH_OK) {
+    if (gated) (void)hipStreamSynchronize(st);
+    return rc;
+  }
   std::vector<XYZZ<Fq>> pageable;
   XYZZ<Fq>* wins = nullptr;
-  if (pinned_for(st, sizeof(XYZZ<Fq>) * MAX_WINDOWS, &pin_host, &pin_dev)) {
+  if (pinned) {
     wins = reinterpret_cast<XYZZ<Fq>*>(pin_host);
   } else {
     pageable.resize(p.W);
@@ -978,7 +1054,7 @@
   uint32_t c = 0, W = 0, wide = 0;
   if (n > 0) {
     MsmParams p;
-    CSH_TRY((msm_windows_dev<Cfg>(B, offset, n, scalars_dev, mont, st, wins, &p)));
+    CSH_TRY((msm_windows_dev<Cfg>(B, offset, n, scalars_dev, mont, st, wins, &p, nullptr, sync)));
     c = (uint32_t)p.c;
     W = (uint32_t)p.W;
     wide = (uint32_t)p.wide;
@@ -1143,7 +1219,7 @@
   KW template int repack_bases_t<CFG>(Bases*, hipStream_t);                                                                     \
   KW template int msm_tail_selftest_t<CFG>(const void*, uint32_t, uint32_t, int, void*);                                        \
   KW template size_t msm_bucket_bytes<CFG>(const MsmParams*);                                                                   \
-  KW template int msm_bucket_stage<CFG>(const void*, const MsmParams*, const SortOut*, hipStream_t, Arena*, void*, hipEvent_t*);          \
+  KW template int msm_bucket_stage<CFG>(const void*, const MsmParams*, const SortOut*, hipStream_t, Arena*, void*, hipEvent_t*, const GiantGate*); \
   KW template int precompute_table_t<CFG>(Bases*, int, int, hipStream_t);                                                            \
   KW template void fold_windows_erased<CFG>(const void*, int, int, int, void*);
 
@@ -1166,9 +1242,9 @@
   int scalar_bits;
   size_t point_bytes;
   size_t xyzz_bytes;
-  int (*sort)(const MsmParams&, const MsmParams&, const uint64_t*, hipStream_t, Arena&, SortOut*, hipEvent_t*);
+  int (*sort)(const MsmParams&, const MsmParams&, const uint64_t*, hipStream_t, Arena&, SortOut*, hipEvent_t*, const SortFork*);
   size_t (*bucket_bytes)(const MsmParams*);
-  int (*bucket)(const void*, const MsmParams*, const SortOut*, hipStream_t, Arena*, void*, hipEvent_t*);
+  int (*bucket)(const void*, const MsmParams*, const SortOut*, hipStream_t, Arena*, void*, hipEvent_t*, const GiantGate*);
   void (*fold)(const void*, int, int, int, void*);
   int (*occ)();
 };
diff --git a/co-snarks_amd/csrc/msm_sort.hip b/co-snarks_amd/csrc/msm_sort.hip
--- a/co-snarks_amd/csrc/msm_sort.hip
+++ b/co-snarks_amd/csrc/msm_sort.hip
@@ -47,6 +47,7 @@
   }
 }
 
+template <bool WRITE_BACK>
 __global__ __launch_bounds__(256) void k_msm_colscan(MsmParams p, uint32_t* __restrict__ blkcnt, uint32_t* __restrict__ hist) {
   const uint32_t w = blockIdx.y;
   const uint32_t b = blockIdx.x * 256 + threadIdx.x;
@@ -59,7 +60,9 @@
     for (uint32_t j = 0; j < 8; ++j) t[j] = ch0 + j < p.CH ? col[(size_t)(ch0 + j) * p.NB] : 0u;
 #pragma unroll
     for (uint32_t j = 0; j < 8; ++j) {
-      if (ch0 + j < p.CH) col[(size_t)(ch0 + j) * p.NB] = acc;
+      if constexpr (WRITE_BACK) {
+        if (ch0 + j < p.CH) col[(size_t)(ch0 + j) * p.NB] = acc;
+      }
       acc += t[j];
     }
   }
@@ -133,20 +136,44 @@
 constexpr uint32_t PART_LB = 8;
 static_assert(PART_BUCKETS == 1u << PART_LB, "the record format's low key must hold a partition's bucket index");
 
-__global__ __launch_bounds__(256) void k_msm_part_offsets(MsmParams p, const uint32_t* __restrict__ start, uint32_t* part_cnt) {
+constexpr uint32_t MAXP = 128;
+
+constexpr uint32_t PO_REG = 32;
+__global__ __launch_bounds__(MAXP) void k_msm_part_offsets(MsmParams p, uint32_t* part_cnt) {
+  __shared__ uint32_t wsum[MAXP / 64];
   const uint32_t P = p.NB / PART_BUCKETS;
-  const uint32_t part = blockIdx.x * 256 + threadIdx.x, w = blockIdx.y;
-  if (part >= P) return;
-  uint32_t run = start[(size_t)w * (p.NB + 2) + (size_t)part * PART_BUCKETS + 1];
-  uint32_t* col = part_cnt + (size_t)w * p.CH * P + part;
-  for (uint32_t ch0 = 0; ch0 < p.CH; ch0 += 8) {
-    uint32_t c[8];
-#pragma unroll
-    for (uint32_t j = 0; j < 8; ++j) c[j] = ch0 + j < p.CH ? col[(size_t)(ch0 + j) * P] : 0u;
+  const uint32_t part = threadIdx.x, w = blockIdx.x;
+  const bool live = part < P;
+  uint32_t* col = part_cnt + (size_t)w * p.CH * P + (live ? part : 0);
+  uint32_t c[PO_REG];
+  uint32_t tot = 0;
+#pragma unroll
+  for (uint32_t j = 0; j < PO_REG; ++j) c[j] = live && j < p.CH ? col[(size_t)j * P] : 0u;
+#pragma unroll
+  for (uint32_t j = 0; j < PO_REG; ++j) tot += c[j];
+  for (uint32_t ch0 = PO_REG; ch0 < p.CH; ch0 += 8) {
+    uint32_t t[8];
+#pragma unroll
+    for (uint32_t j = 0; j < 8; ++j) t[j] = live && ch0 + j < p.CH ? col[(size_t)(ch0 + j) * P] : 0u;
+#pragma unroll
+    for (uint32_t j = 0; j < 8; ++j) tot += t[j];
+  }
+  uint32_t total;
+  uint32_t run = block_excl_scan<MAXP / 64>(tot, wsum, &total);
+  if (!live) return;
+#pragma unroll
+  for (uint32_t j = 0; j < PO_REG; ++j) {
+    if (j < p.CH) col[(size_t)j * P] = run;
+    run += c[j];
+  }
+  for (uint32_t ch0 = PO_REG; ch0 < p.CH; ch0 += 8) {
+    uint32_t t[8];
+#pragma unroll
+    for (uint32_t j = 0; j < 8; ++j) t[j] = ch0 + j < p.CH ? col[(size_t)(ch0 + j) * P] : 0u;
 #pragma unroll
     for (uint32_t j = 0; j < 8; ++j) {
       if (ch0 + j < p.CH) col[(size_t)(ch0 + j) * P] = run;
-      run += c[j];
+      run += t[j];
     }
   }
 }
@@ -161,7 +188,6 @@
 #endif
 constexpr int L1_EPT = 8;
 constexpr int L1_TILE = L1_EPT * SORT_BLK;
-constexpr uint32_t MAXP = 128;
 template <int REC>
 __global__ __launch_bounds__(SORT_BLK) CSH_L1_OCC void k_msm_scatter_l1(MsmParams p, const uint16_t* __restrict__ dig, const uint32_t* __restrict__ part_off,
                                                              void* __restrict__ inter) {
@@ -359,9 +385,8 @@
 }
 
 template <int REC>
-static void launch_two_level(const MsmParams& p, const SortBuffers& b, bool per_partition, hipStream_t st) {
+static void launch_level2(const MsmParams& p, const SortBuffers& b, bool per_partition, hipStream_t st) {
   const uint32_t nparts = p.NB / PART_BUCKETS;
-  hipLaunchKernelGGL(k_msm_scatter_l1<REC>, dim3(p.CH, p.W), dim3(SORT_BLK), 0, st, p, b.dig, b.part_cnt, (void*)b.inter);
   if (per_partition) {
     hipLaunchKernelGGL(k_msm_scatter_l2<REC>, dim3(nparts, p.W), dim3(SORT_BLK), 0, st, p, b.start, (const void*)b.inter, b.sorted);
   } else {
@@ -370,7 +395,18 @@
   }
 }
 
-int msm_sort_launch(const MsmParams& p, const SortBuffers& b, hipStream_t st, hipEvent_t* ev) {
+static int launch_bucket_scans(const MsmParams& p, const SortBuffers& b, bool chunk_prefixes, hipStream_t st, hipEvent_t* ev) {
+  const dim3 grid((p.NB + 255) / 256, p.W);
+  if (chunk_prefixes) hipLaunchKernelGGL(k_msm_colscan<true>, grid, dim3(256), 0, st, p, b.blkcnt, b.hist);
+  else hipLaunchKernelGGL(k_msm_colscan<false>, grid, dim3(256), 0, st, p, b.blkcnt, b.hist);
+  if (ev) CSH_HIP(hipEventRecord(ev[1], st));
+  const size_t scan_lds = sizeof(uint32_t) * ((size_t)p.NB + 2 + 16);
+  if (scan_lds > 48 * 1024) CSH_TRY(raise_lds_limit((const void*)k_msm_scan, 136 * 1024));
+  hipLaunchKernelGGL(k_msm_scan, dim3(p.W), dim3(1024), scan_lds, st, p, b.hist, b.start, b.nlanes);
+  return CSH_OK;
+}
+
+int msm_sort_launch(const MsmParams& p, const SortBuffers& b, hipStream_t st, hipEvent_t* ev, const SortFork* fork) {
   const SortPath path = msm_sort_path(p);
   const bool two_level = path.two_level;
   const size_t sort_lds = sizeof(uint32_t) * p.NB;
@@ -379,20 +415,28 @@
     CSH_TRY(raise_lds_limit((const void*)k_msm_scatter_lds, 128 * 1024));
   }
   hipLaunchKernelGGL(k_msm_hist_lds, dim3(p.CH, p.W), dim3(SORT_BLK), sort_lds, st, p, b.dig, b.blkcnt, two_level ? b.part_cnt : nullptr);
-  hipLaunchKernelGGL(k_msm_colscan, dim3((p.NB + 255) / 256, p.W), dim3(256), 0, st, p, b.blkcnt, b.hist);
-  if (ev) CSH_HIP(hipEventRecord(ev[1], st));
-  {
-    const size_t scan_lds = sizeof(uint32_t) * ((size_t)p.NB + 2 + 16);
-    if (scan_lds > 48 * 1024) CSH_TRY(raise_lds_limit((const void*)k_msm_scan, 136 * 1024));
-    hipLaunchKernelGGL(k_msm_scan, dim3(p.W), dim3(1024), scan_lds, st, p, b.hist, b.start, b.nlanes);
-  }
-  if (ev) CSH_HIP(hipEventRecord(ev[2], st));
-  if (two_level) {
-    hipLaunchKernelGGL(k_msm_part_offsets, dim3((p.NB / PART_BUCKETS + 255) / 256, p.W), dim3(256), 0, st, p, b.start, b.part_cnt);
-    path.rec4 ? launch_two_level<1>(p, b, path.per_partition, st) : launch_two_level<0>(p, b, path.per_partition, st);
+  if (!two_level) {
+    CSH_TRY(launch_bucket_scans(p, b, true, st, ev));
+    if (ev) CSH_HIP(hipEventRecord(ev[2], st));
+    hipLaunchKernelGGL(k_msm_scatter_lds, dim3(p.CH, p.W), dim3(SORT_BLK), sort_lds, st, p, b.dig, b.start, b.blkcnt, b.sorted);
+    if (ev) CSH_HIP(hipEventRecord(ev[3], st));
+    return CSH_OK;
+  }
+  const bool forked = fork && fork->aux && !ev;
+  if (forked) {
+    CSH_HIP(hipEventRecord(fork->forked, st));
+    CSH_HIP(hipStreamWaitEvent(fork->aux, fork->forked, 0));
+    CSH_TRY(launch_bucket_scans(p, b, path.per_partition, fork->aux, nullptr));
+    CSH_HIP(hipEventRecord(fork->joined, fork->aux));
   } else {
-    hipLaunchKernelGGL(k_msm_scatter_lds, dim3(p.CH, p.W), dim3(SORT_BLK), sort_lds, st, p, b.dig, b.start, b.blkcnt, b.sorted);
-  }
+    CSH_TRY(launch_bucket_scans(p, b, path.per_partition, st, ev));
+    if (ev) CSH_HIP(hipEventRecord(ev[2], st));
+  }
+  hipLaunchKernelGGL(k_msm_part_offsets, dim3(p.W), dim3(MAXP), 0, st, p, b.part_cnt);
+  if (path.rec4) hipLaunchKernelGGL(k_msm_scatter_l1<1>, dim3(p.CH, p.W), dim3(SORT_BLK), 0, st, p, b.dig, b.part_cnt, (void*)b.inter);
+  else hipLaunchKernelGGL(k_msm_scatter_l1<0>, dim3(p.CH, p.W), dim3(SORT_BLK), 0, st, p, b.dig, b.part_cnt, (void*)b.inter);
+  if (forked) CSH_HIP(hipStreamWaitEvent(st, fork->joined, 0));
+  path.rec4 ? launch_level2<1>(p, b, path.per_partition, st) : launch_level2<0>(p, b, path.per_partition, st);
   if (ev) CSH_HIP(hipEventRecord(ev[3], st));
   return CSH_OK;
 }
diff --git a/co-snarks_amd/csrc/msm_sort.hpp b/co-snarks_amd/csrc/msm_sort.hpp
--- a/co-snarks_amd/csrc/msm_sort.hpp
+++ b/co-snarks_amd/csrc/msm_sort.hpp
@@ -141,6 +141,10 @@
   bool per_partition;
 };
 SortPath msm_sort_path(const MsmParams& p);
-int msm_sort_launch(const MsmParams& p, const SortBuffers& b, hipStream_t st, hipEvent_t* ev);
+struct SortFork {
+  hipStream_t aux;
+  hipEvent_t forked, joined;
+};
+int msm_sort_launch(const MsmParams& p, const SortBuffers& b, hipStream_t st, hipEvent_t* ev, const SortFork* fork = nullptr);
 
 }
diff --git a/co-snarks_amd/csrc/selftest_dev.hip b/co-snarks_amd/csrc/selftest_dev.hip
--- a/co-snarks_amd/csrc/selftest_dev.hip
+++ b/co-snarks_amd/csrc/selftest_dev.hip
@@ -385,7 +385,7 @@
   CSH_HIP(hipMemset(ar.base, 0xFF, bytes));
   CSH_HIP(hipDeviceSynchronize());
   SortOut so{};
-  CSH_TRY(G->sort(p, pd, dsc.as<uint64_t>(), st, ar, &so, nullptr));
+  CSH_TRY(G->sort(p, pd, dsc.as<uint64_t>(), st, ar, &so, nullptr, nullptr));
   CSH_HIP(hipGetLastError());
   CSH_HIP(hipStreamSynchronize(st));
   CSH_HIP(hipMemcpy(start, so.start, nstart * sizeof(uint32_t), hipMemcpyDeviceToHost));
```

Result: no change. 657.4 million points/s (median of 2 runs) (-0.2%).
